# hanl2010/Binocular3DGS

Hardware: AMD Instinct MI355X
Metric: train iters/s (fwd+bwd), 1M Gaussians @ 800x600, 6 views/iter (higher is better)
Workload: dtype f32; 1 GPU; synth(P=1000000, seed=0) 800x600, 3 input + 3 binocular-shifted views per rank per iter, fwd+bwd+gradient sum+Adam; gaussians=1000000, width=800, height=600, views_per_rank=6, global_views=6, sh_degree=1, K=4, loss=synthetic, optimizer_in_step=True, densify_stats_in_step=True, optimizer=sharded, hip_graph=True, schedule=batched, binning_rounds=2, dp_tail_ranges=0

## Files before the change

binocular3dgs_amd/_lib.py:

```python
from __future__ import annotations

import ctypes as C
import os

_HERE = os.path.dirname(os.path.abspath(__file__))
LIB_PATH = os.environ.get("B3GS_LIB") or os.path.join(_HERE, "libb3gs_raster.so")

ABI_VERSION = 18
OK = 0
ERR_NAMES = {-1: "B3GS_ERR_ARG", -2: "B3GS_ERR_ALLOC", -3: "B3GS_ERR_HIP", -4: "B3GS_ERR_CAPACITY",
             -5: "B3GS_ERR_NO_DEVICE"}

c_float_p = C.c_void_p

ALLOC_FN = C.CFUNCTYPE(C.c_void_p, C.c_void_p, C.c_size_t)


class B3gsScene(C.Structure):
    _fields_ = [("P", C.c_int32), ("D", C.c_int32), ("M", C.c_int32), ("W", C.c_int32), ("H", C.c_int32),
                ("tan_fovx", C.c_float), ("tan_fovy", C.c_float), ("scale_modifier", C.c_float),
                ("prefiltered", C.c_int32), ("debug", C.c_int32),
                ("background", C.c_void_p), ("means3D", C.c_void_p), ("shs", C.c_void_p),
                ("colors_precomp", C.c_void_p), ("opacities", C.c_void_p), ("scales", C.c_void_p),
                ("rotations", C.c_void_p), ("cov3D_precomp", C.c_void_p), ("viewmatrix", C.c_void_p),
                ("projmatrix", C.c_void_p), ("campos", C.c_void_p)]


class B3gsRawParams(C.Structure):
    _fields_ = [("xyz", C.c_void_p), ("features_dc", C.c_void_p), ("features_rest", C.c_void_p),
                ("scaling", C.c_void_p), ("rotation", C.c_void_p), ("opacity", C.c_void_p)]


class B3gsRawGrads(C.Structure):
    _fields_ = B3gsRawParams._fields_ + [("touched_rows", C.c_void_p)]


class B3gsFusedView(C.Structure):
    _fields_ = [("view", C.POINTER(B3gsScene)), ("radii", C.c_void_p), ("geometry", C.c_void_p),
                ("scratch", C.c_void_p), ("dL_dmeans2D", C.c_void_p), ("densify_stats", C.c_int32)]


class B3gsBlendView(C.Structure):
    _fields_ = [("view", C.POINTER(B3gsScene)), ("geometry", C.c_void_p), ("binning", C.c_void_p),
                ("image", C.c_void_p), ("out_color", C.c_void_p), ("out_depth", C.c_void_p),
                ("out_alpha", C.c_void_p), ("dL_dcolor", C.c_void_p), ("dL_ddepth", C.c_void_p),
                ("dL_dalpha", C.c_void_p), ("scratch", C.c_void_p), ("binning_capacity", C.c_int64)]


class B3gsForwardView(C.Structure):
    _fields_ = [("view", C.POINTER(B3gsScene)), ("geometry", C.c_void_p), ("binning", C.c_void_p),
                ("binning_capacity", C.c_int64), ("image", C.c_void_p), ("out_color", C.c_void_p),
                ("out_depth", C.c_void_p), ("out_alpha", C.c_void_p), ("radii", C.c_void_p),
                ("device_num_rendered", C.c_void_p), ("depth_order_from", C.c_int32), ("seg1_fraction", C.c_float),
                ("high_water", C.c_void_p), ("overflow_flag", C.c_void_p), ("depth_key_bits", C.c_int32),
                ("fresh_image", C.c_int32), ("depth_order_hint", C.c_void_p), ("hint_mismatch", C.c_void_p),
                ("hint_trusted", C.c_int32), ("visible", C.c_void_p), ("reference_binning", C.c_int32)]


class B3gsLossIO(C.Structure):
    _fields_ = [("W", C.c_int32), ("H", C.c_int32), ("image", C.c_void_p), ("depth", C.c_void_p), ("alpha", C.c_void_p),
                ("gt_image", C.c_void_p), ("shifted_image", C.c_void_p), ("alpha_weight", C.c_void_p),
                ("focal_x", C.c_float), ("trans_dist", C.c_float), ("lambda_dssim", C.c_float),
                ("lambda_smooth", C.c_float), ("grad_scale", C.c_float), ("dL_dimage", C.c_void_p),
                ("dL_ddepth", C.c_void_p), ("dL_dalpha", C.c_void_p), ("dL_dshifted", C.c_void_p),
                ("parts", C.c_void_p), ("workspace", C.c_void_p), ("trans_dist_dev", C.c_void_p)]


class B3gsDensifyIO(C.Structure):
    _fields_ = [("P", C.c_int32), ("M", C.c_int32), ("param", C.c_void_p * 6), ("exp_avg", C.c_void_p * 6),
                ("exp_avg_sq", C.c_void_p * 6), ("xyz_gradient_accum", C.c_void_p), ("denom", C.c_void_p),
                ("grad_threshold", C.c_float), ("min_opacity", C.c_float), ("extent", C.c_float),
                ("percent_dense", C.c_float), ("max_screen_size", C.c_float)]


class B3gsAdamSegment(C.Structure):
    _fields_ = [("param", C.c_void_p), ("grad", C.c_void_p), ("exp_avg", C.c_void_p), ("exp_avg_sq", C.c_void_p),
                ("count", C.c_int64), ("lr", C.c_float), ("row_len", C.c_int32), ("first_row", C.c_int32),
                ("lr_dev", C.c_void_p)]


class B3gsDensifyStats(C.Structure):
    _fields_ = [("xyz_gradient_accum", C.c_void_p), ("denom", C.c_void_p), ("max_radii2D", C.c_void_p),
                ("skip_if_nonzero", C.c_void_p)]


class B3gsDebugViews(C.Structure):
    _fields_ = [("tiles_touched", C.c_void_p), ("depths", C.c_void_p), ("records", C.c_void_p),
                ("point_list", C.c_void_p), ("tile_ids", C.c_void_p), ("ranges", C.c_void_p),
                ("final_T", C.c_void_p), ("n_contrib", C.c_void_p), ("packed_idx_bits", C.c_int32),
                ("counts", C.c_void_p), ("point_list2", C.c_void_p), ("ranges2", C.c_void_p)]


class B3gsMetricView(C.Structure):
    _fields_ = [("image", C.c_void_p), ("gt", C.c_void_p), ("mask", C.c_void_p), ("mask_channels", C.c_int32),
                ("prepared_image", C.c_void_p), ("prepared_gt", C.c_void_p)]


class B3gsFrameView(C.Structure):
    _fields_ = [("rgb", C.c_void_p), ("depth", C.c_void_p), ("alpha", C.c_void_p), ("rgb_out", C.c_void_p),
                ("gray_out", C.c_void_p), ("cmap_out", C.c_void_p)]


class B3gsGtView(C.Structure):
    _fields_ = [("src", C.c_void_p), ("Hs", C.c_int32), ("Ws", C.c_int32), ("C", C.c_int32), ("tab_x", C.c_void_p),
                ("tab_y", C.c_void_p), ("ks_x", C.c_int32), ("ks_y", C.c_int32), ("image", C.c_void_p),
                ("alpha", C.c_void_p), ("bg_mask", C.c_void_p)]


class B3gsCloudGrow(C.Structure):
    _fields_ = ([(n, C.c_int32) for n in ("W", "H", "n_views", "ref", "src", "n_seeds", "n_samples", "n_start", "h_patch_size", "init")]
                + [(n, C.c_float) for n in ("fx", "fy", "cx", "cy", "alpha", "ssim_threshold")]
                + [(n, C.c_void_p) for n in ("images", "w2c", "window", "seed_idx", "noise", "points", "colors")]
                + [("capacity", C.c_int32)]
                + [(n, C.c_void_p) for n in ("length", "overflow", "grids", "workspace", "debug_ssim", "debug_mask")])


class B3gsSweepPair(C.Structure):
    _fields_ = ([(n, C.c_int32) for n in ("W", "H", "D", "stride", "radius")]
                + [(n, C.c_float) for n in ("near", "far", "inv_far", "step", "min_score", "margin", "min_var", "cyc_steps")]
                + [(n, C.c_void_p) for n in ("image_a", "image_b", "homographies", "proj", "kp_source", "kp_target", "score", "count",
                                             "node_invd", "node_score", "node_k", "workspace")])


class B3gsTsdfVolume(C.Structure):
    _fields_ = [("nx", C.c_int32), ("ny", C.c_int32), ("nz", C.c_int32), ("origin", C.c_float * 3), ("voxel", C.c_float),
                ("tsdf", C.c_void_p), ("weight", C.c_void_p), ("rgb", C.c_void_p)]


class B3gsTsdfView(C.Structure):
    _fields_ = [("depth", C.c_void_p), ("alpha", C.c_void_p), ("colour", C.c_void_p), ("rot", C.c_float * 9),
                ("trans", C.c_float * 3), ("fx", C.c_float), ("fy", C.c_float)]


class B3gsLpipsWeights(C.Structure):
    _fields_ = [("conv_w", C.c_void_p * 13), ("conv_b", C.c_void_p * 13), ("lin", C.c_void_p * 5), ("shift", C.c_float * 3),
                ("scale", C.c_float * 3)]


class B3gsKernelTimes(C.Structure):
    _fields_ = [("preprocess_ms", C.c_double), ("sort_ms", C.c_double), ("render_fwd_ms", C.c_double),
                ("render_bwd_ms", C.c_double), ("preprocess_bwd_ms", C.c_double), ("calls", C.c_int64)]


EXPORTS = ("b3gs_abi_version", "b3gs_last_error", "b3gs_set_timing", "b3gs_timing_collect", "b3gs_geometry_bytes", "b3gs_image_bytes",
           "b3gs_binning_bytes", "b3gs_forward", "b3gs_forward_capacity", "b3gs_backward", "b3gs_mark_visible",
           "b3gs_debug_views", "b3gs_forward_raw", "b3gs_backward_raw", "b3gs_backward_scratch_floats",
           "b3gs_backward_raw_accumulate", "b3gs_blend_forward_batch", "b3gs_blend_backward_batch",
           "b3gs_adam_step", "b3gs_forward_raw_batch", "b3gs_loss_workspace_floats", "b3gs_binocular_loss",
           "b3gs_densify_classify", "b3gs_densify_scatter", "b3gs_knn_workspace_bytes", "b3gs_knn_mean_dist2",
           "b3gs_backward_raw_accumulate_range", "b3gs_binocular_loss_batch",
           "b3gs_lossfn_workspace_floats", "b3gs_l1_loss_forward", "b3gs_l1_loss_backward", "b3gs_inverse_warp_forward",
           "b3gs_inverse_warp_backward", "b3gs_smooth_loss_forward", "b3gs_smooth_loss_backward", "b3gs_ssim_forward",
           "b3gs_ssim_backward", "b3gs_opacity_decay", "b3gs_add_densification_stats", "b3gs_adam_step_at", "b3gs_debug_activations",
           "b3gs_apply_staged_densify_stats",
           "b3gs_image_metrics_workspace_bytes", "b3gs_image_metrics_batch",
           "b3gs_frames_workspace_bytes", "b3gs_encode_frames_batch",
           "b3gs_gt_workspace_bytes", "b3gs_prepare_gt_batch",
           "b3gs_cloud_workspace_bytes", "b3gs_triangulate_matches", "b3gs_background_sheet", "b3gs_cloud_grow_round",
           "b3gs_sweep_workspace_bytes", "b3gs_sweep_match_pair",
           "b3gs_jpeg_workspace_bytes", "b3gs_jpeg_encode_batch",
           "b3gs_tsdf_integrate_batch", "b3gs_mesh_workspace_bytes", "b3gs_mesh_count", "b3gs_mesh_emit",
           "b3gs_mesh_components", "b3gs_mesh_clean_workspace_bytes", "b3gs_mesh_clean_count", "b3gs_mesh_clean_emit",
           "b3gs_mesh_sample_workspace_bytes", "b3gs_mesh_sample_count", "b3gs_mesh_sample_emit",
           "b3gs_nearest_workspace_bytes", "b3gs_nearest_grid", "b3gs_nearest_query",
           "b3gs_cloud_score_workspace_bytes", "b3gs_cloud_score",
           "b3gs_mesh_simplify_workspace_bytes", "b3gs_mesh_simplify_count", "b3gs_mesh_simplify_emit",
           "b3gs_mesh_raster_workspace_bytes", "b3gs_mesh_raster_batch", "b3gs_mesh_resolve_batch",
           "b3gs_mesh_texture_atlas_height", "b3gs_mesh_texture_accumulate_batch", "b3gs_mesh_texture_finalize",
           "b3gs_mesh_resolve_textured_batch",
           "b3gs_mesh_adjacency_workspace_bytes", "b3gs_mesh_adjacency_layout", "b3gs_mesh_adjacency_build", "b3gs_mesh_smooth",
           "b3gs_mesh_vertex_normals", "b3gs_mesh_resolve_shaded_batch",
           "b3gs_lpips_workspace_bytes", "b3gs_lpips_batch", "b3gs_lpips_features")

_lib = None


class B3gsError(RuntimeError):
    pass


def lib():
    global _lib
    if _lib is not None:
        return _lib
    if not os.path.exists(LIB_PATH):
        raise B3gsError(f"{LIB_PATH} not found: run `python -m binocular3dgs_amd.build` (hipcc, gfx950). "
                        "There is no CPU or PyTorch fallback for the rasterizer.")
    L = C.CDLL(LIB_PATH)
    L.b3gs_abi_version.restype = C.c_int
    L.b3gs_last_error.restype = C.c_char_p
    L.b3gs_set_timing.argtypes = [C.c_void_p]
    L.b3gs_set_timing.restype = None
    L.b3gs_timing_collect.restype = C.c_int
    L.b3gs_geometry_bytes.argtypes = [C.c_int32]
    L.b3gs_geometry_bytes.restype = C.c_size_t
    L.b3gs_image_bytes.argtypes = [C.c_int32, C.c_int32]
    L.b3gs_image_bytes.restype = C.c_size_t
    L.b3gs_binning_bytes.argtypes = [C.c_int32, C.c_int64]
    L.b3gs_binning_bytes.restype = C.c_size_t
    L.b3gs_forward.argtypes = [C.POINTER(B3gsScene), ALLOC_FN, C.c_void_p, ALLOC_FN, C.c_void_p, ALLOC_FN,
                               C.c_void_p, C.c_void_p, C.c_void_p, C.c_void_p, C.c_void_p,
                               C.POINTER(C.c_int32), C.c_void_p]
    L.b3gs_forward.restype = C.c_int
    L.b3gs_forward_capacity.argtypes = [C.POINTER(B3gsScene), C.c_void_p, C.c_void_p, C.c_int64, C.c_void_p,
                                        C.c_void_p, C.c_void_p, C.c_void_p, C.c_void_p, C.c_void_p, C.c_void_p]
    L.b3gs_forward_capacity.restype = C.c_int
    L.b3gs_backward.argtypes = [C.POINTER(B3gsScene), C.c_int32, C.c_void_p, C.c_void_p, C.c_void_p, C.c_void_p,
                                C.c_void_p, C.c_void_p, C.c_void_p] + [C.c_void_p] * 8 + [C.c_void_p]
    L.b3gs_backward.restype = C.c_int
    L.b3gs_forward_raw.argtypes = [C.POINTER(B3gsScene), C.POINTER(B3gsRawParams), C.c_void_p, C.c_void_p, C.c_int64,
                                   C.c_void_p, C.c_void_p, C.c_void_p, C.c_void_p, C.c_void_p, C.c_void_p, C.c_int,
                                   C.c_void_p]
    L.b3gs_forward_raw.restype = C.c_int
    for fn in (L.b3gs_blend_forward_batch, L.b3gs_blend_backward_batch):
        fn.argtypes = [C.c_int32, C.POINTER(B3gsBlendView), C.c_void_p]
        fn.restype = C.c_int
    L.b3gs_backward_scratch_floats.argtypes = [C.c_int32]
    L.b3gs_backward_scratch_floats.restype = C.c_size_t
    L.b3gs_backward_raw.argtypes = [C.POINTER(B3gsScene), C.POINTER(B3gsRawParams), C.c_void_p, C.c_void_p, C.c_void_p,
                                    C.c_void_p, C.c_void_p, C.c_void_p, C.c_void_p, C.c_void_p,
                                    C.POINTER(B3gsRawGrads), C.c_void_p, C.c_int, C.c_void_p]
    L.b3gs_backward_raw.restype = C.c_int
    L.b3gs_backward_raw_accumulate.argtypes = [C.c_int32, C.POINTER(B3gsFusedView), C.POINTER(B3gsRawParams),
                                               C.POINTER(B3gsRawGrads), C.c_int32, C.POINTER(B3gsDensifyStats),
                                               C.c_void_p]
    L.b3gs_backward_raw_accumulate.restype = C.c_int
    L.b3gs_backward_raw_accumulate_range.argtypes = [C.c_int32, C.POINTER(B3gsFusedView), C.POINTER(B3gsRawParams),
                                                     C.POINTER(B3gsRawGrads), C.c_int32, C.POINTER(B3gsDensifyStats),
                                                     C.c_int32, C.c_int32, C.c_void_p]
    L.b3gs_backward_raw_accumulate_range.restype = C.c_int
    L.b3gs_forward_raw_batch.argtypes = [C.c_int32, C.POINTER(B3gsForwardView), C.POINTER(B3gsRawParams), C.c_int,
                                         C.c_void_p]
    L.b3gs_forward_raw_batch.restype = C.c_int
    L.b3gs_loss_workspace_floats.argtypes = [C.c_int32, C.c_int32]
    L.b3gs_loss_workspace_floats.restype = C.c_size_t
    L.b3gs_binocular_loss.argtypes = [C.POINTER(B3gsLossIO), C.c_void_p]
    L.b3gs_binocular_loss.restype = C.c_int
    L.b3gs_binocular_loss_batch.argtypes = [C.c_int32, C.POINTER(B3gsLossIO), C.c_void_p]
    L.b3gs_binocular_loss_batch.restype = C.c_int
    L.b3gs_densify_classify.argtypes = [C.POINTER(B3gsDensifyIO), C.c_void_p, C.c_void_p]
    L.b3gs_densify_classify.restype = C.c_int
    L.b3gs_densify_scatter.argtypes = [C.POINTER(B3gsDensifyIO), C.c_void_p, C.c_void_p, C.c_void_p, C.c_void_p, C.c_int32,
                                       C.c_int32, C.c_int32, C.c_void_p, C.POINTER(C.c_void_p), C.POINTER(C.c_void_p),
                                       C.POINTER(C.c_void_p), C.c_void_p]
    L.b3gs_densify_scatter.restype = C.c_int
    L.b3gs_knn_workspace_bytes.argtypes = [C.c_int32]
    L.b3gs_knn_workspace_bytes.restype = C.c_size_t
    L.b3gs_knn_mean_dist2.argtypes = [C.c_int32, C.c_void_p, C.c_void_p, C.c_void_p, C.c_void_p]
    L.b3gs_knn_mean_dist2.restype = C.c_int
    L.b3gs_adam_step.argtypes = [C.c_int32, C.POINTER(B3gsAdamSegment), C.c_void_p, C.c_float, C.c_float, C.c_float,
                                 C.c_float, C.c_int32, C.c_int32, C.c_int32, C.c_void_p, C.c_void_p, C.c_void_p]
    L.b3gs_adam_step.restype = C.c_int
    V, I32, I64, F = C.c_void_p, C.c_int32, C.c_int64, C.c_float
    L.b3gs_lossfn_workspace_floats.argtypes = [I64, I32, I32]
    L.b3gs_lossfn_workspace_floats.restype = C.c_size_t
    L.b3gs_l1_loss_forward.argtypes = [V, V, V, I64, I32, I64, V, V, V]
    L.b3gs_l1_loss_backward.argtypes = [V, V, V, I64, I32, I64, V, V, V, V, V]
    L.b3gs_inverse_warp_forward.argtypes = [V, V, I32, I32, I32, I32, V, V, V]
    L.b3gs_inverse_warp_backward.argtypes = [V, V, V, I32, I32, I32, I32, V, V, V]
    L.b3gs_smooth_loss_forward.argtypes = [V, V, I32, I32, I32, I32, V, V, V]
    L.b3gs_smooth_loss_backward.argtypes = [V, V, I32, I32, I32, I32, V, V, V, V]
    L.b3gs_ssim_forward.argtypes = [V, V, I32, I32, I32, I32, I32, V, I32, V, V, V]
    L.b3gs_ssim_backward.argtypes = [V, V, V, I32, I32, I32, I32, I32, V, V, V, V]
    L.b3gs_opacity_decay.argtypes = [V, I64, F, V]
    L.b3gs_add_densification_stats.argtypes = [I64, V, I64, V, V, V, V]
    L.b3gs_adam_step_at.argtypes = [I32, C.POINTER(B3gsAdamSegment), I32, F, F, F, V]
    for fn in (L.b3gs_l1_loss_forward, L.b3gs_l1_loss_backward, L.b3gs_inverse_warp_forward, L.b3gs_inverse_warp_backward,
               L.b3gs_smooth_loss_forward, L.b3gs_smooth_loss_backward, L.b3gs_ssim_forward, L.b3gs_ssim_backward,
               L.b3gs_opacity_decay, L.b3gs_add_densification_stats, L.b3gs_adam_step_at):
        fn.restype = C.c_int
    L.b3gs_apply_staged_densify_stats.argtypes = [I64] + [V] * 9
    L.b3gs_apply_staged_densify_stats.restype = C.c_int
    L.b3gs_debug_activations.argtypes = [I32, C.POINTER(B3gsRawParams), V, V, V, V]
    L.b3gs_debug_activations.restype = C.c_int
    L.b3gs_image_metrics_workspace_bytes.argtypes = [I32, I32, I32, I32]
    L.b3gs_image_metrics_workspace_bytes.restype = C.c_size_t
    L.b3gs_image_metrics_batch.argtypes = [I32, C.POINTER(B3gsMetricView), I32, I32, I32, I32, V, V, V]
    L.b3gs_image_metrics_batch.restype = C.c_int
    L.b3gs_frames_workspace_bytes.argtypes = [I32, I32, I32]
    L.b3gs_frames_workspace_bytes.restype = C.c_size_t
    L.b3gs_encode_frames_batch.argtypes = [I32, C.POINTER(B3gsFrameView), I32, I32, C.c_double, V, V, V, V]
    L.b3gs_encode_frames_batch.restype = C.c_int
    L.b3gs_gt_workspace_bytes.argtypes = [I32, C.POINTER(B3gsGtView), I32, I32]
    L.b3gs_gt_workspace_bytes.restype = C.c_size_t
    L.b3gs_prepare_gt_batch.argtypes = [I32, C.POINTER(B3gsGtView), I32, I32, I32, C.c_float, V, V]
    L.b3gs_prepare_gt_batch.restype = C.c_int
    L.b3gs_cloud_workspace_bytes.argtypes = [I64]
    L.b3gs_cloud_workspace_bytes.restype = C.c_size_t
    L.b3gs_triangulate_matches.argtypes = [I32] + [V] * 8 + [I32, I32, F, V, V, V, V, V]
    L.b3gs_triangulate_matches.restype = C.c_int
    L.b3gs_background_sheet.argtypes = [V, I32, I32, V, V, F, V, V, V, V, V]
    L.b3gs_background_sheet.restype = C.c_int
    L.b3gs_cloud_grow_round.argtypes = [C.POINTER(B3gsCloudGrow), V]
    L.b3gs_cloud_grow_round.restype = C.c_int
    L.b3gs_sweep_workspace_bytes.argtypes = [I32, I32, I32, I32]
    L.b3gs_sweep_workspace_bytes.restype = C.c_size_t
    L.b3gs_sweep_match_pair.argtypes = [C.POINTER(B3gsSweepPair), V]
    L.b3gs_sweep_match_pair.restype = C.c_int
    L.b3gs_jpeg_workspace_bytes.argtypes = [I32, I32, I32]
    L.b3gs_jpeg_workspace_bytes.restype = C.c_size_t
    L.b3gs_jpeg_encode_batch.argtypes = [I32, C.POINTER(C.c_void_p), I32, I32, V, V, I64, V, V, V]
    L.b3gs_jpeg_encode_batch.restype = C.c_int
    L.b3gs_tsdf_integrate_batch.argtypes = [C.POINTER(B3gsTsdfVolume), I32, C.POINTER(B3gsTsdfView), I32, I32, F, F, F, V]
    L.b3gs_tsdf_integrate_batch.restype = C.c_int
    L.b3gs_mesh_workspace_bytes.argtypes = [I32, I32, I32]
    L.b3gs_mesh_workspace_bytes.restype = C.c_size_t
    L.b3gs_mesh_count.argtypes = [C.POINTER(B3gsTsdfVolume), F, V, V]
    L.b3gs_mesh_count.restype = C.c_int
    L.b3gs_mesh_emit.argtypes = [C.POINTER(B3gsTsdfVolume), V, I64, I64, V, V, V, V]
    L.b3gs_mesh_emit.restype = C.c_int
    L.b3gs_mesh_components.argtypes = [I32, I64, V, V, V, V]
    L.b3gs_mesh_components.restype = C.c_int
    L.b3gs_mesh_clean_workspace_bytes.argtypes = [I64, I64]
    L.b3gs_mesh_clean_workspace_bytes.restype = C.c_size_t
    L.b3gs_mesh_clean_count.argtypes = [I32, I64, V, V, V, V, V, V]
    L.b3gs_mesh_clean_count.restype = C.c_int
    L.b3gs_mesh_clean_emit.argtypes = [I32, I64, V, V, V, V, V, V, V, I64, I64, V, V, V, V]
    L.b3gs_mesh_clean_emit.restype = C.c_int
    L.b3gs_mesh_sample_workspace_bytes.argtypes = [I64]
    L.b3gs_mesh_sample_workspace_bytes.restype = C.c_size_t
    L.b3gs_mesh_sample_count.argtypes = [I32, I64, V, V, F, V, V]
    L.b3gs_mesh_sample_count.restype = C.c_int
    L.b3gs_mesh_sample_emit.argtypes = [I32, I64, V, V, F, V, I64, V, V]
    L.b3gs_mesh_sample_emit.restype = C.c_int
    L.b3gs_nearest_workspace_bytes.argtypes = [I64]
    L.b3gs_nearest_workspace_bytes.restype = C.c_size_t
    L.b3gs_nearest_grid.argtypes = [I64, V, F, V, V]
    L.b3gs_nearest_grid.restype = C.c_int
    L.b3gs_nearest_query.argtypes = [I64, V, I64, F, V, V, V]
    L.b3gs_nearest_query.restype = C.c_int
    L.b3gs_cloud_score_workspace_bytes.argtypes = [I64]
    L.b3gs_cloud_score_workspace_bytes.restype = C.c_size_t
    L.b3gs_cloud_score.argtypes = [I64, V, V, F, V, V, V]
    L.b3gs_cloud_score.restype = C.c_int
    L.b3gs_mesh_simplify_workspace_bytes.argtypes = [I64, I64]
    L.b3gs_mesh_simplify_workspace_bytes.restype = C.c_size_t
    L.b3gs_mesh_simplify_count.argtypes = [I32, I64, V, V, F, V, V]
    L.b3gs_mesh_simplify_count.restype = C.c_int
    L.b3gs_mesh_simplify_emit.argtypes = [I32, I64, V, V, V, F, I32, V, I64, I64, V, V, V, V]
    L.b3gs_mesh_simplify_emit.restype = C.c_int
    L.b3gs_mesh_raster_workspace_bytes.argtypes = [I32, I64, I64, I32, I32]
    L.b3gs_mesh_raster_workspace_bytes.restype = C.c_size_t
    L.b3gs_mesh_raster_batch.argtypes = [I32, V, I32, I32, I32, I64, V, V, I32, I32, I32, V, V, V]
    L.b3gs_mesh_raster_batch.restype = C.c_int
    L.b3gs_mesh_resolve_batch.argtypes = [I32, V, I32, I32, I32, I64, V, V, V, V, V, I32, V, V, V, V, V, V]
    L.b3gs_mesh_resolve_batch.restype = C.c_int
    L.b3gs_mesh_texture_atlas_height.argtypes = [I64, I32, I32]
    L.b3gs_mesh_texture_atlas_height.restype = I32
    L.b3gs_mesh_texture_accumulate_batch.argtypes = [I32, V, I32, I32, I32, I64, V, V, I32, I32, I32, V, V, V, C.c_float, I32, V, V, V]
    L.b3gs_mesh_texture_accumulate_batch.restype = C.c_int
    L.b3gs_mesh_texture_finalize.argtypes = [I32, I64, V, V, I32, I32, I32, V, V, V, V]
    L.b3gs_mesh_texture_finalize.restype = C.c_int
    L.b3gs_mesh_resolve_textured_batch.argtypes = [I32, V, I32, I32, I32, I64, V, V, V, V, V, I32, I32, I32, V, V, V, V, V, V]
    L.b3gs_mesh_resolve_textured_batch.restype = C.c_int
    L.b3gs_mesh_adjacency_workspace_bytes.argtypes = [I64, I64]
    L.b3gs_mesh_adjacency_workspace_bytes.restype = C.c_size_t
    L.b3gs_mesh_adjacency_layout.argtypes = [I64, I64, C.POINTER(C.c_size_t)]
    L.b3gs_mesh_adjacency_layout.restype = C.c_int
    L.b3gs_mesh_adjacency_build.argtypes = [I32, I64, V, V, V, V]
    L.b3gs_mesh_adjacency_build.restype = C.c_int
    L.b3gs_mesh_smooth.argtypes = [I32, I64, V, V, I32, C.c_double, C.c_double, I32, V, V]
    L.b3gs_mesh_smooth.restype = C.c_int
    L.b3gs_mesh_vertex_normals.argtypes = [I32, I64, V, V, V, V, V]
    L.b3gs_mesh_vertex_normals.restype = C.c_int
    L.b3gs_mesh_resolve_shaded_batch.argtypes = [I32, V, I32, I32, I32, I64, V, V, V, V, I32, V, V, V, V, V, V]
    L.b3gs_mesh_resolve_shaded_batch.restype = C.c_int
    L.b3gs_lpips_workspace_bytes.argtypes = [I32, I32, I32]
    L.b3gs_lpips_workspace_bytes.restype = C.c_size_t
    L.b3gs_lpips_batch.argtypes = [I32, V, V, I32, I32, C.POINTER(B3gsLpipsWeights), I32, V, V, V]
    L.b3gs_lpips_batch.restype = C.c_int
    L.b3gs_lpips_features.argtypes = [I32, V, I32, I32, C.POINTER(B3gsLpipsWeights), I32, C.POINTER(C.c_void_p), V, V]
    L.b3gs_lpips_features.restype = C.c_int
    L.b3gs_mark_visible.argtypes = [C.c_int32, C.c_void_p, C.c_void_p, C.c_void_p, C.c_void_p, C.c_void_p]
    L.b3gs_mark_visible.restype = C.c_int
    L.b3gs_debug_views.argtypes = [C.c_int32, C.c_int32, C.c_int32, C.c_int64, C.c_void_p, C.c_void_p, C.c_void_p,
                                   C.POINTER(B3gsDebugViews)]
    L.b3gs_debug_views.restype = C.c_int
    if L.b3gs_abi_version() != ABI_VERSION:
        raise B3gsError(f"libb3gs_raster.so ABI {L.b3gs_abi_version()} != binding {ABI_VERSION}: rebuild")
    _lib = L
    return L


# ... 5 lines not shown
```

binocular3dgs_amd/csrc/api.hip:

```cpp
#include "b3gs_internal.h"

#include <cstdio>
#include <cstdlib>
#include <cstring>
#include <mutex>

namespace {

thread_local char g_err[512] = "";
B3gsKernelTimes* g_timing = nullptr;
std::mutex g_timing_mu;

int fail(int code, const char* fmt, const char* detail) {
  snprintf(g_err, sizeof(g_err), fmt, detail);
  return code;
}

#define HIP_TRY(expr)                                                                   \
  do {                                                                                  \
    hipError_t e_ = (expr);                                                             \
    if (e_ != hipSuccess) return fail(B3GS_ERR_HIP, #expr ": %s", hipGetErrorString(e_)); \
  } while (0)

int check_scene(const B3gsScene* sc) {
  if (!sc) return fail(B3GS_ERR_ARG, "%s", "scene is NULL");
  if (sc->P < 0 || sc->W <= 0 || sc->H <= 0) return fail(B3GS_ERR_ARG, "%s", "bad P/W/H");
  if (sc->P >= (1 << 24)) return fail(B3GS_ERR_ARG, "%s", "P must be below 2^24 (24-bit row offsets in the blend backward)");
  if (sc->D < 0 || sc->D > 3) return fail(B3GS_ERR_ARG, "%s", "SH degree must be 0..3");
  if ((sc->shs == nullptr) == (sc->colors_precomp == nullptr))
    return fail(B3GS_ERR_ARG, "%s", "provide exactly one of shs / colors_precomp");
  const bool has_sr = sc->scales != nullptr && sc->rotations != nullptr;
  if (has_sr == (sc->cov3D_precomp != nullptr))
    return fail(B3GS_ERR_ARG, "%s", "provide exactly one of (scales, rotations) / cov3D_precomp");
  if (sc->shs && sc->M < (sc->D + 1) * (sc->D + 1)) return fail(B3GS_ERR_ARG, "%s", "M too small for SH degree");
  if (((sc->W + B3GS_TILE - 1) / B3GS_TILE) > 65535 || ((sc->H + B3GS_TILE - 1) / B3GS_TILE) > 65535)
    return fail(B3GS_ERR_ARG, "%s", "image too large for the packed tile rect");
  if (!sc->background || !sc->viewmatrix || !sc->projmatrix || !sc->campos || (sc->P > 0 && (!sc->means3D || !sc->opacities)))
    return fail(B3GS_ERR_ARG, "%s", "NULL required tensor");
  return B3GS_OK;
}

SceneX wrap(const B3gsScene* sc) {
  SceneX x;
  x.sc = *sc;
  x.raw = B3gsRawParams{nullptr, nullptr, nullptr, nullptr, nullptr, nullptr};
  x.raw_mode = 0;
  x.tight = 0;
  return x;
}

int check_raw(const B3gsScene* sc, const B3gsRawParams* rp) {
  if (!sc || !rp) return fail(B3GS_ERR_ARG, "%s", "scene / raw params NULL");
  if (sc->P < 0 || sc->W <= 0 || sc->H <= 0) return fail(B3GS_ERR_ARG, "%s", "bad P/W/H");
  if (sc->P >= (1 << 24)) return fail(B3GS_ERR_ARG, "%s", "P must be below 2^24 (24-bit row offsets in the blend backward)");
  if (sc->D < 0 || sc->D > 3 || sc->M < (sc->D + 1) * (sc->D + 1)) return fail(B3GS_ERR_ARG, "%s", "bad SH degree / M");
  if (((sc->W + B3GS_TILE - 1) / B3GS_TILE) > 65535 || ((sc->H + B3GS_TILE - 1) / B3GS_TILE) > 65535)
    return fail(B3GS_ERR_ARG, "%s", "image too large for the packed tile rect");
  if (!sc->background || !sc->viewmatrix || !sc->projmatrix || !sc->campos) return fail(B3GS_ERR_ARG, "%s", "NULL camera tensor");
  if (sc->P > 0 && (!rp->xyz || !rp->features_dc || (sc->M > 1 && !rp->features_rest) || !rp->scaling || !rp->rotation ||
                    !rp->opacity))
    return fail(B3GS_ERR_ARG, "%s", "NULL raw parameter tensor");
  return B3GS_OK;
}

void blend_forward_one(const B3gsScene& sc, const GeomView& g, const BinView& b, const ImgView& im, float* out_color,
                       float* out_depth, float* out_alpha, hipStream_t s) {
  BlendBatch batch;
  batch.n = 1;
  batch.order = nullptr;
  batch.order_buf = nullptr;
  batch.cls_size = 0;
  batch.v[0] = b3gs_blend_view(sc, g, b, im);
  batch.v[0].out_color = out_color;
  batch.v[0].out_depth = out_depth;
  batch.v[0].out_alpha = out_alpha;
  b3gs_launch_blend_forward(batch, s);
}

BlendView blend_backward_view(const B3gsScene& sc, const GeomView& g, const BinView& b, const ImgView& im,
                              const float* dL_dcolor, const float* dL_ddepth, const float* dL_dalpha, float* m2d,
                              float* col, float* op, float* cov, uint32_t m2d_stride, uint32_t col_stride,
                              uint32_t op_stride, uint32_t cov_stride) {
  BlendView v = b3gs_blend_view(sc, g, b, im);
  v.dL_dcolor = dL_dcolor;
  v.dL_ddepth = dL_ddepth;
  v.dL_dalpha = dL_dalpha;
  v.dL_dmeans2D = m2d;
  v.dL_dcolors = col;
  v.dL_dopacity = op;
  v.dL_dcov3D = cov;
  v.m2d_stride = m2d_stride;
  v.col_stride = col_stride;
  v.op_stride = op_stride;
  v.cov_stride = cov_stride;
  return v;
}

struct PendingStage {
  hipEvent_t a, b;
  int slot;
};
PendingStage g_pending[4096];
int g_npending = 0;

struct StageTimer {
  hipStream_t s;
  hipEvent_t prev = nullptr;
  bool on;
  explicit StageTimer(hipStream_t st) : s(st), on(g_timing != nullptr) {}
  void mark(int slot) {
    if (!on) return;
    hipEvent_t e;
    (void)hipEventCreate(&e);
    (void)hipEventRecord(e, s);
    std::lock_guard<std::mutex> lk(g_timing_mu);
    if (slot >= 0 && prev && g_npending < 4096) {
      g_pending[g_npending++] = PendingStage{prev, e, slot};
    }
    prev = e;
  }
};

int debug_sync(const B3gsScene* sc, hipStream_t s, const char* what) {
  if (!sc->debug) return B3GS_OK;
  hipError_t e = hipStreamSynchronize(s);
  if (e == hipSuccess) e = hipGetLastError();
  if (e != hipSuccess) {
    snprintf(g_err, sizeof(g_err), "after %s: %s", what, hipGetErrorString(e));
    return B3GS_ERR_HIP;
  }
  return B3GS_OK;
}

}

int b3gs_fail(int code, const char* what, const char* detail) {
  snprintf(g_err, sizeof(g_err), "%s%s%s", what ? what : "", (what && detail) ? ": " : "", detail ? detail : "");
  return code;
}

int b3gs_launch_status(const char* what) {
  const hipError_t e = hipGetLastError();
  return e == hipSuccess ? B3GS_OK : b3gs_fail(B3GS_ERR_HIP, what, hipGetErrorString(e));
}

extern "C" {

int b3gs_abi_version(void) { return B3GS_ABI_VERSION; }
const char* b3gs_last_error(void) { return g_err; }
void b3gs_set_timing(B3gsKernelTimes* sink) { g_timing = sink; }

int b3gs_timing_collect(void) {
  std::lock_guard<std::mutex> lk(g_timing_mu);
// ... 268 lines not shown
  if (phases & 2) {
    b3gs_launch_blend_forward(bb, s);
    tm.mark(2);
    if (K1) {
      b3gs_launch_round2_batch(P, nviews, jobs, s);
      tm.mark(1);
      for (int k = 0; k < nviews; k++) bb.v[k].round = 1;
      b3gs_launch_blend_forward(bb, s);
      tm.mark(2);
    }
  }
  HIP_TRY(hipGetLastError());
  return B3GS_OK;
}

size_t b3gs_backward_scratch_floats(int32_t P) { return (size_t)B3GS_SCRATCH_ROW * (size_t)(P > 0 ? P : 0); }

int b3gs_backward_raw(const B3gsScene* view, const B3gsRawParams* params, const int32_t* radii, const char* geometry,
                      const char* binning, const char* image, const float* dL_dcolor, const float* dL_ddepth,
                      const float* dL_dalpha, float* scratch, const B3gsRawGrads* grads, float* dL_dmeans2D,
                      int phases, b3gs_stream_t stream) {
  int rc = check_raw(view, params);
  if (rc) return rc;
  if (view->P == 0) return B3GS_OK;
  if (!radii || !geometry || !binning || !image || !dL_dcolor || !scratch || !grads || !grads->xyz ||
      !grads->features_dc || (view->M > 1 && !grads->features_rest) || !grads->scaling || !grads->rotation ||
      !grads->opacity)
    return fail(B3GS_ERR_ARG, "%s", "NULL required tensor in backward_raw");
  hipStream_t s = (hipStream_t)stream;
  SceneX sx;
  sx.sc = *view;
  sx.raw = *params;
  sx.raw_mode = 1;
  sx.tight = 0;
  GeomView g;
  ImgView im;
  BinView b;
  b3gs_geom_view(const_cast<char*>(geometry), view->P, &g);
  b3gs_img_view(const_cast<char*>(image), view->W, view->H, &im);
  b3gs_bin_view(const_cast<char*>(binning), view->P, 1, &b);
  const size_t P = (size_t)view->P;
  (void)P;
  StageTimer tm(s);
  tm.mark(-1);
  if (phases & 1) {
    BlendBatch batch;
    batch.n = 1;
    batch.order = nullptr;
    batch.order_buf = im.order;
    batch.v[0] = blend_backward_view(sx.sc, g, b, im, dL_dcolor, dL_ddepth, dL_dalpha, scratch + 4, scratch + 6,
                                     scratch + 9, scratch, B3GS_SCRATCH_ROW, B3GS_SCRATCH_ROW, B3GS_SCRATCH_ROW,
                                     B3GS_SCRATCH_ROW);
    b3gs_launch_blend_backward(batch, s);
    tm.mark(3);
  }
  if (phases & 2) {
    if (!(phases & 1)) tm.mark(-1);
    b3gs_launch_preprocess_backward(sx, g, radii, nullptr, nullptr, nullptr, nullptr, scratch, nullptr, nullptr, nullptr,
                                    grads, dL_dmeans2D, s);
    tm.mark(4);
  }
  HIP_TRY(hipGetLastError());
  return B3GS_OK;
}

int b3gs_backward(const B3gsScene* sc, int32_t num_rendered, const int32_t* radii, const char* geometry,
                  const char* binning, const char* image, const float* dL_dcolor, const float* dL_ddepth,
                  const float* dL_dalpha, float* dL_dmeans2D, float* dL_dcolors, float* dL_dopacity,
                  float* dL_dmeans3D, float* dL_dcov3D, float* dL_dsh, float* dL_dscales, float* dL_drotations,
                  b3gs_stream_t stream) {
  int rc = check_scene(sc);
  if (rc) return rc;
  if (sc->P == 0) return B3GS_OK;
  if (!radii || !geometry || !image || !dL_dcolor || !dL_dmeans2D || !dL_dcolors || !dL_dopacity || !dL_dmeans3D ||
      !dL_dcov3D)
    return fail(B3GS_ERR_ARG, "%s", "NULL required tensor in backward");
  if (sc->shs && !dL_dsh) return fail(B3GS_ERR_ARG, "%s", "dL_dsh required when shs given");
  if (sc->scales && (!dL_dscales || !dL_drotations)) return fail(B3GS_ERR_ARG, "%s", "dL_dscales/dL_drotations required");
  if (num_rendered != 0 && !binning) return fail(B3GS_ERR_ARG, "%s", "binning buffer is NULL");
  hipStream_t s = (hipStream_t)stream;
  GeomView g;
  ImgView im;
  BinView b;
  b3gs_geom_view(const_cast<char*>(geometry), sc->P, &g);
  b3gs_img_view(const_cast<char*>(image), sc->W, sc->H, &im);
  b3gs_bin_view(const_cast<char*>(binning), sc->P, num_rendered < 0 ? 1 : num_rendered, &b);

  const size_t P = (size_t)sc->P;
  StageTimer tm(s);
  tm.mark(-1);
  float* rows = g.bwd_rows;
  HIP_TRY(hipMemsetAsync(rows, 0, P * B3GS_SCRATCH_ROW * sizeof(float), s));
  if (num_rendered != 0) {
    BlendBatch batch;
    batch.n = 1;
    batch.order = nullptr;
    batch.order_buf = im.order;
    batch.v[0] = blend_backward_view(*sc, g, b, im, dL_dcolor, dL_ddepth, dL_dalpha, rows + 4, rows + 6, rows + 9, rows,
                                     B3GS_SCRATCH_ROW, B3GS_SCRATCH_ROW, B3GS_SCRATCH_ROW, B3GS_SCRATCH_ROW);
    b3gs_launch_blend_backward(batch, s);
  }
  if ((rc = debug_sync(sc, s, "render backward"))) return rc;
  tm.mark(3);
  b3gs_launch_preprocess_backward(wrap(sc), g, radii, dL_dmeans2D, dL_dcolors, dL_dopacity, dL_dmeans3D, dL_dcov3D,
                                  dL_dsh, dL_dscales, dL_drotations, nullptr, nullptr, s);
  if ((rc = debug_sync(sc, s, "preprocess backward"))) return rc;
  tm.mark(4);
  HIP_TRY(hipGetLastError());
  return B3GS_OK;
}

static int batch_views_ok(int32_t nviews, const B3gsBlendView* views) {
  if (nviews <= 0 || nviews > B3GS_MAX_FUSED_VIEWS || !views)
    return fail(B3GS_ERR_ARG, "%s", "bad view count (1..8) or NULL view table");
  for (int k = 0; k < nviews; k++)
    if (!views[k].view || !views[k].geometry || !views[k].binning || !views[k].image || views[k].view->W <= 0 ||
        views[k].view->H <= 0 || !views[k].view->background)
      return fail(B3GS_ERR_ARG, "%s", "NULL state buffer in a batched view");
  return B3GS_OK;
}

int b3gs_blend_forward_batch(int32_t nviews, const B3gsBlendView* views, b3gs_stream_t stream) {
  int rc = batch_views_ok(nviews, views);
  if (rc) return rc;
  hipStream_t s = (hipStream_t)stream;
  BlendBatch batch;
  batch.n = nviews;
  batch.order = nullptr;
  batch.order_buf = nullptr;
  batch.cls_size = 0;
  for (int k = 0; k < nviews; k++) {
    const B3gsBlendView& bv = views[k];
    if (!bv.out_color || !bv.out_depth || !bv.out_alpha) return fail(B3GS_ERR_ARG, "%s", "NULL output image");
    GeomView g;
    ImgView im;
    BinView b;
    b3gs_geom_view(const_cast<char*>(bv.geometry), bv.view->P, &g);
    b3gs_img_view(const_cast<char*>(bv.image), bv.view->W, bv.view->H, &im);
    b3gs_bin_view(const_cast<char*>(bv.binning), bv.view->P, bv.binning_capacity > 0 ? bv.binning_capacity : 1, &b);
    batch.v[k] = b3gs_blend_view(*bv.view, g, b, im);
    batch.v[k].round = 2;
    batch.v[k].out_color = bv.out_color;
    batch.v[k].out_depth = bv.out_depth;
    batch.v[k].out_alpha = bv.out_alpha;
  }
  StageTimer tm(s);
  tm.mark(-1);
  b3gs_launch_blend_forward(batch, s);
  tm.mark(2);
  HIP_TRY(hipGetLastError());
  return B3GS_OK;
}

int b3gs_blend_backward_batch(int32_t nviews, const B3gsBlendView* views, b3gs_stream_t stream) {
  int rc = batch_views_ok(nviews, views);
  if (rc) return rc;
  hipStream_t s = (hipStream_t)stream;
  BlendBatch batch;
  batch.n = nviews;
  batch.order = nullptr;
  batch.order_buf = nullptr;
  batch.cls_size = 0;
  for (int k = 0; k < nviews; k++) {
    const B3gsBlendView& bv = views[k];
    if (!bv.dL_dcolor || !bv.scratch) return fail(B3GS_ERR_ARG, "%s", "NULL dL_dcolor / scratch");
    GeomView g;
    ImgView im;
    BinView b;
    b3gs_geom_view(const_cast<char*>(bv.geometry), bv.view->P, &g);
    b3gs_img_view(const_cast<char*>(bv.image), bv.view->W, bv.view->H, &im);
    if (k == 0) batch.order_buf = im.order;
    b3gs_bin_view(const_cast<char*>(bv.binning), bv.view->P, bv.binning_capacity > 0 ? bv.binning_capacity : 1, &b);
    batch.v[k] = blend_backward_view(*bv.view, g, b, im, bv.dL_dcolor, bv.dL_ddepth, bv.dL_dalpha, bv.scratch + 4,
                                     bv.scratch + 6, bv.scratch + 9, bv.scratch, B3GS_SCRATCH_ROW, B3GS_SCRATCH_ROW,
                                     B3GS_SCRATCH_ROW, B3GS_SCRATCH_ROW);
  }
  StageTimer tm(s);
  tm.mark(-1);
  b3gs_launch_blend_backward(batch, s);
  tm.mark(3);
  HIP_TRY(hipGetLastError());
  return B3GS_OK;
}

int b3gs_backward_raw_accumulate(int32_t nviews, const B3gsFusedView* views, const B3gsRawParams* params,
                                 const B3gsRawGrads* grads, int32_t overwrite, const B3gsDensifyStats* stats,
                                 b3gs_stream_t stream) {
  const int32_t P = (nviews > 0 && views && views[0].view) ? views[0].view->P : 0;
  return b3gs_backward_raw_accumulate_range(nviews, views, params, grads, overwrite, stats, 0, P, stream);
}

int b3gs_backward_raw_accumulate_range(int32_t nviews, const B3gsFusedView* views, const B3gsRawParams* params,
                                       const B3gsRawGrads* grads, int32_t overwrite, const B3gsDensifyStats* stats,
                                       int32_t first, int32_t count, b3gs_stream_t stream) {
  if (nviews <= 0 || nviews > B3GS_MAX_FUSED_VIEWS || !views || !params || !grads)
    return fail(B3GS_ERR_ARG, "%s", "bad view count / NULL argument (at most 8 views per call)");
  const B3gsScene* v0 = views[0].view;
  int rc = check_raw(v0, params);
  if (rc) return rc;
  if (v0->P == 0 || count == 0) return B3GS_OK;
  if (first < 0 || count < 0 || (int64_t)first + count > v0->P) return fail(B3GS_ERR_ARG, "%s", "bad Gaussian range");
  if (grads->touched_rows && overwrite && (first & 63))
    return fail(B3GS_ERR_ARG, "%s", "sparse-row gradients (touched_rows) need a range that starts at a multiple of 64");
  if (!grads->xyz || !grads->features_dc || (v0->M > 1 && !grads->features_rest) || !grads->scaling ||
      !grads->rotation || !grads->opacity)
    return fail(B3GS_ERR_ARG, "%s", "NULL gradient buffer");
  B3gsViewRef refs[B3GS_MAX_FUSED_VIEWS];
  uint32_t *list = nullptr, *counts = nullptr;
  static const bool no_staged = getenv("B3GS_NO_STAGED") != nullptr;
  for (int k = 0; k < nviews; k++) {
    const B3gsFusedView& fv = views[k];
    if (!fv.view || !fv.radii || !fv.geometry || !fv.scratch) return fail(B3GS_ERR_ARG, "%s", "NULL view state");
    if (fv.view->P != v0->P || fv.view->M != v0->M || fv.view->D != v0->D || fv.view->scale_modifier != v0->scale_modifier)
      return fail(B3GS_ERR_ARG, "%s", "views of one call must share P, M, D and scale_modifier");
    GeomView g;
    b3gs_geom_view(const_cast<char*>(fv.geometry), v0->P, &g);
    if (k == 0) { list = g.skey[1]; counts = g.skey[0]; }
    refs[k] = B3gsViewRef{fv.view->W, fv.view->H, fv.view->tan_fovx, fv.view->tan_fovy, fv.view->viewmatrix,
                          fv.view->projmatrix, fv.view->campos, fv.radii, reinterpret_cast<const float*>(g.rec), fv.scratch, fv.dL_dmeans2D,
                          fv.densify_stats, no_staged ? nullptr : g.staged, g.header + B3GS_GEOM_EPOCH};
  }
  if (stats && (!stats->xyz_gradient_accum || !stats->denom || !stats->max_radii2D))
    return fail(B3GS_ERR_ARG, "%s", "densify stats need all three arrays");
  hipStream_t s = (hipStream_t)stream;
  StageTimer tm(s);
  tm.mark(-1);
  b3gs_launch_accumulate_views(*v0, *params, nviews, refs, *grads, overwrite, stats, first, count, list, counts, s);
  tm.mark(4);
  HIP_TRY(hipGetLastError());
  return B3GS_OK;
}

int b3gs_mark_visible(int32_t P, const float* means3D, const float* viewmatrix, const float* projmatrix,
                      uint8_t* present, b3gs_stream_t stream) {
  (void)projmatrix;
  if (P < 0 || (P > 0 && (!means3D || !viewmatrix || !present))) return fail(B3GS_ERR_ARG, "%s", "bad arguments");
  b3gs_launch_mark_visible(P, means3D, viewmatrix, present, (hipStream_t)stream);
  HIP_TRY(hipGetLastError());
  return B3GS_OK;
}

int b3gs_debug_views(int32_t P, int32_t W, int32_t H, int64_t num_rendered, const char* geometry, const char* binning,
                     const char* image, B3gsDebugViews* out) {
  if (!out || !geometry || !image) return fail(B3GS_ERR_ARG, "%s", "NULL argument");
  GeomView g;
  ImgView im;
  BinView b;
  b3gs_geom_view(const_cast<char*>(geometry), P, &g);
  b3gs_img_view(const_cast<char*>(image), W, H, &im);
  memset(out, 0, sizeof(*out));
  out->tiles_touched = g.tiles_touched;
  out->depths = reinterpret_cast<const float*>(g.depth_key);
  out->records = reinterpret_cast<const float*>(g.rec);
  if (binning) {
    b3gs_bin_view(const_cast<char*>(binning), P, num_rendered, &b);
    out->point_list = b.val[0];
    out->packed_idx_bits = b3gs_packed_idx_bits(P, W, H);
    out->tile_ids = out->packed_idx_bits >= 0 ? nullptr : b.key[0];
  }
  out->ranges = reinterpret_cast<const uint32_t*>(im.ranges);
  out->ranges2 = reinterpret_cast<const uint32_t*>(im.ranges2);
  out->counts = g.header;
  if (binning) out->point_list2 = b.val[0];
  out->final_T = im.final_T;
  out->n_contrib = im.n_contrib;
  return B3GS_OK;
}

}
```

binocular3dgs_amd/csrc/preprocess.hip:

```cpp
#include "b3gs_internal.h"

namespace {

constexpr float SH_C0 = 0.28209479177387814f;
constexpr float SH_C1 = 0.4886025119029199f;
__constant__ float SH_C2[5] = {1.0925484305920792f, -1.0925484305920792f, 0.31539156525252005f,
                               -1.0925484305920792f, 0.5462742152960396f};
__constant__ float SH_C3[7] = {-0.5900435899266435f, 2.890611442640554f, -0.4570457994644658f,
                               0.3731763325901154f,  -0.4570457994644658f, 1.445305721320277f,
                               -0.5900435899266435f};

struct Mat16 {
  float m[16];
};

__device__ __forceinline__ Mat16 load_mat(const float* __restrict__ p) {
  Mat16 r;
#pragma unroll
  for (int i = 0; i < 16; i++) r.m[i] = p[i];
  return r;
}
typedef const float __attribute__((address_space(4))) cfloat_k;
__device__ __forceinline__ cfloat_k* uniform_ptr(const float* p) { return (cfloat_k*)(uintptr_t)p; }
__device__ __forceinline__ Mat16 load_mat_uniform(const float* p) {
  cfloat_k* q = uniform_ptr(p);
  Mat16 r;
#pragma unroll
  for (int i = 0; i < 16; i++) r.m[i] = q[i];
  return r;
}

__device__ __forceinline__ void quat_to_R(float r, float x, float y, float z, float R[9]) {
  R[0] = 1.f - 2.f * (y * y + z * z);
  R[1] = 2.f * (x * y - r * z);
  R[2] = 2.f * (x * z + r * y);
  R[3] = 2.f * (x * y + r * z);
  R[4] = 1.f - 2.f * (x * x + z * z);
  R[5] = 2.f * (y * z - r * x);
  R[6] = 2.f * (x * z - r * y);
  R[7] = 2.f * (y * z + r * x);
  R[8] = 1.f - 2.f * (x * x + y * y);
}

template <bool RAW>
__device__ __forceinline__ void load_scale_rot(const SceneX& sx_, int i, float s[3], float q[4], float* inv_norm) {
  if (RAW) {
    const float* ls = sx_.raw.scaling + 3 * (size_t)i;
    s[0] = expf(ls[0]); s[1] = expf(ls[1]); s[2] = expf(ls[2]);
    const float4 r = reinterpret_cast<const float4*>(sx_.raw.rotation)[i];
    const float n = sqrtf((r.x * r.x + r.y * r.y) + (r.z * r.z + r.w * r.w));
    const float den = fmaxf(n, 1e-12f);
    q[0] = r.x / den; q[1] = r.y / den; q[2] = r.z / den; q[3] = r.w / den;
    *inv_norm = 1.0f / den;
  } else {
    const float* ps = sx_.sc.scales + 3 * (size_t)i;
    s[0] = ps[0]; s[1] = ps[1]; s[2] = ps[2];
    const float4 r = reinterpret_cast<const float4*>(sx_.sc.rotations)[i];
    q[0] = r.x; q[1] = r.y; q[2] = r.z; q[3] = r.w;
    *inv_norm = 1.0f;
  }
}
template <bool RAW>
__device__ __forceinline__ float load_opacity(const SceneX& sx_, int i) {
  if (RAW) return 1.0f / (1.0f + expf(-sx_.raw.opacity[i]));
  return sx_.sc.opacities[i];
}
struct ShView {
  const float* dc;
  const float* rest;
  __device__ __forceinline__ float operator()(int k, int ch) const { return k == 0 ? dc[ch] : rest[3 * (k - 1) + ch]; }
};
struct ShLds {
  const float* lo;
  const float* rest;
  __device__ __forceinline__ float operator()(int k, int ch) const { return k < 4 ? lo[(3 * k + ch) * 256] : rest[3 * (k - 1) + ch]; }
};
template <bool RAW>
__device__ __forceinline__ ShView sh_view(const SceneX& sx_, int i) {
  ShView v;
  if (RAW) {
    v.dc = sx_.raw.features_dc + 3 * (size_t)i;
    v.rest = sx_.raw.features_rest + (size_t)3 * (sx_.sc.M - 1) * i;
  } else {
    v.dc = sx_.sc.shs + (size_t)3 * sx_.sc.M * i;
    v.rest = v.dc + 3;
  }
  return v;
}

template <bool RAW>
__device__ __forceinline__ void cov3d_of(const SceneX& sx_, int i, float c6[6]) {
  const B3gsScene& sc = sx_.sc;
  if (!RAW && sc.cov3D_precomp) {
#pragma unroll
    for (int k = 0; k < 6; k++) c6[k] = sc.cov3D_precomp[6 * (size_t)i + k];
    return;
  }
  float s[3], q[4], inv_norm;
  load_scale_rot<RAW>(sx_, i, s, q, &inv_norm);
  float R[9], L[9];
  quat_to_R(q[0], q[1], q[2], q[3], R);
  float sx = sc.scale_modifier * s[0], sy = sc.scale_modifier * s[1], sz = sc.scale_modifier * s[2];
#pragma unroll
  for (int r = 0; r < 3; r++) {
    L[3 * r + 0] = R[3 * r + 0] * sx;
    L[3 * r + 1] = R[3 * r + 1] * sy;
    L[3 * r + 2] = R[3 * r + 2] * sz;
  }
#define LL(a, b) ((L[3 * a] * L[3 * b] + L[3 * a + 1] * L[3 * b + 1]) + L[3 * a + 2] * L[3 * b + 2])
  c6[0] = LL(0, 0);
  c6[1] = LL(0, 1);
  c6[2] = LL(0, 2);
  c6[3] = LL(1, 1);
  c6[4] = LL(1, 2);
  c6[5] = LL(2, 2);
#undef LL
}

struct Ewa {
  float T0[3], T1[3];
  float a, b, c;
  float tx, ty, tz;
  float xmul, ymul;
};

__device__ __forceinline__ Ewa ewa_project(const float pv[3], float fx, float fy, float tanfovx, float tanfovy,
                                           const float c6[6], const Mat16& vm) {
  Ewa e;
  float limx = 1.3f * tanfovx, limy = 1.3f * tanfovy;
  float txtz = pv[0] / pv[2], tytz = pv[1] / pv[2];
  e.xmul = (txtz < -limx || txtz > limx) ? 0.f : 1.f;
  e.ymul = (tytz < -limy || tytz > limy) ? 0.f : 1.f;
  e.tx = fminf(limx, fmaxf(-limx, txtz)) * pv[2];
  e.ty = fminf(limy, fmaxf(-limy, tytz)) * pv[2];
  e.tz = pv[2];
  float J00 = fx / e.tz, J02 = -(fx * e.tx) / (e.tz * e.tz);
  float J11 = fy / e.tz, J12 = -(fy * e.ty) / (e.tz * e.tz);
#pragma unroll
  for (int j = 0; j < 3; j++) {
    e.T0[j] = J00 * vm.m[4 * j + 0] + J02 * vm.m[4 * j + 2];
    e.T1[j] = J11 * vm.m[4 * j + 1] + J12 * vm.m[4 * j + 2];
  }
  float S00 = c6[0], S01 = c6[1], S02 = c6[2], S11 = c6[3], S12 = c6[4], S22 = c6[5];
  float v0x = (S00 * e.T0[0] + S01 * e.T0[1]) + S02 * e.T0[2];
  float v0y = (S01 * e.T0[0] + S11 * e.T0[1]) + S12 * e.T0[2];
  float v0z = (S02 * e.T0[0] + S12 * e.T0[1]) + S22 * e.T0[2];
  float v1x = (S00 * e.T1[0] + S01 * e.T1[1]) + S02 * e.T1[2];
  float v1y = (S01 * e.T1[0] + S11 * e.T1[1]) + S12 * e.T1[2];
  float v1z = (S02 * e.T1[0] + S12 * e.T1[1]) + S22 * e.T1[2];
  e.a = (e.T0[0] * v0x + e.T0[1] * v0y) + e.T0[2] * v0z;
  e.b = (e.T0[0] * v1x + e.T0[1] * v1y) + e.T0[2] * v1z;
  e.c = (e.T1[0] * v1x + e.T1[1] * v1y) + e.T1[2] * v1z;
  return e;
// ... 408 lines not shown
      gdir[0] += rx * gl;
      gdir[1] += ry * gl;
      gdir[2] += rz * gl;
    }
    float dot = gdir[0] * x + gdir[1] * y + gdir[2] * z;
    dmean[0] += (gdir[0] - x * dot) * inv;
    dmean[1] += (gdir[1] - y * dot) * inv;
    dmean[2] += (gdir[2] - z * dot) * inv;
  }

  if (do_sr) {
    load_scale_rot<RAW>(sx_, i, o.sraw, o.q, &o.inv_norm);
    const float r = o.q[0], x = o.q[1], y = o.q[2], z = o.q[3];
    float R[9];
    quat_to_R(r, x, y, z, R);
    const float sv[3] = {sc.scale_modifier * o.sraw[0], sc.scale_modifier * o.sraw[1], sc.scale_modifier * o.sraw[2]};
    const float G[9] = {dS[0], 0.5f * dS[1], 0.5f * dS[2], 0.5f * dS[1], dS[3], 0.5f * dS[4], 0.5f * dS[2], 0.5f * dS[4], dS[5]};
    float dR[9];
#pragma unroll
    for (int bcol = 0; bcol < 3; bcol++) {
      float ds = 0.f;
#pragma unroll
      for (int arow = 0; arow < 3; arow++) {
        float dLab = 2.f * sv[bcol] * (G[3 * arow] * R[bcol] + G[3 * arow + 1] * R[3 + bcol] + G[3 * arow + 2] * R[6 + bcol]);
        ds += dLab * R[3 * arow + bcol];
        dR[3 * arow + bcol] = dLab * sv[bcol];
      }
      o.dscale[bcol] = ds * sc.scale_modifier;
    }
    o.dq.x = 2.f * (-z * dR[1] + y * dR[2] + z * dR[3] - x * dR[5] - y * dR[6] + x * dR[7]);
    o.dq.y = 2.f * (y * dR[1] + z * dR[2] + y * dR[3] - 2.f * x * dR[4] - r * dR[5] + z * dR[6] + r * dR[7] - 2.f * x * dR[8]);
    o.dq.z = 2.f * (-2.f * y * dR[0] + x * dR[1] + r * dR[2] + x * dR[3] + z * dR[5] - r * dR[6] + z * dR[7] - 2.f * y * dR[8]);
    o.dq.w = 2.f * (-2.f * z * dR[0] - r * dR[1] + x * dR[2] + r * dR[3] - 2.f * z * dR[4] + y * dR[5] + x * dR[6] + y * dR[7]);
  }
}

__device__ __forceinline__ void raw_chain(const GaussGrad& gg, float dscaling[3], float4& drot) {
  dscaling[0] = gg.dscale[0] * gg.sraw[0];
  dscaling[1] = gg.dscale[1] * gg.sraw[1];
  dscaling[2] = gg.dscale[2] * gg.sraw[2];
  const float qd = ((gg.q[0] * gg.dq.x + gg.q[1] * gg.dq.y) + gg.q[2] * gg.dq.z) + gg.q[3] * gg.dq.w;
  drot.x = (gg.dq.x - gg.q[0] * qd) * gg.inv_norm;
  drot.y = (gg.dq.y - gg.q[1] * qd) * gg.inv_norm;
  drot.z = (gg.dq.z - gg.q[2] * qd) * gg.inv_norm;
  drot.w = (gg.dq.w - gg.q[3] * qd) * gg.inv_norm;
}

template <bool RAW>
__global__ void __launch_bounds__(256)
    preprocess_bwd_kernel(SceneX sx_, GeomView g, const int32_t* __restrict__ radii, float* __restrict__ dL_dmeans2D,
                          float* __restrict__ dL_dcolors, float* __restrict__ dL_dopacity,
                          float* __restrict__ dL_dmeans3D, float* __restrict__ dL_dcov3D, float* __restrict__ dL_dsh,
                          float* __restrict__ dL_dscales, float* __restrict__ dL_drots, B3gsRawGrads rg,
                          float* __restrict__ m2d_out) {
  const B3gsScene& sc = sx_.sc;
  const int i = blockIdx.x * blockDim.x + threadIdx.x;
  if (i >= sc.P) return;
  const size_t i3 = 3 * (size_t)i;
  if (radii[i] <= 0) {
    if (RAW) {
      if (m2d_out) { m2d_out[i3] = 0.f; m2d_out[i3 + 1] = 0.f; m2d_out[i3 + 2] = 0.f; }
      return;
    }
#pragma unroll
    for (int k = 0; k < 3; k++) { dL_dmeans2D[i3 + k] = 0.f; dL_dcolors[i3 + k] = 0.f; dL_dmeans3D[i3 + k] = 0.f; }
#pragma unroll
    for (int k = 0; k < 6; k++) dL_dcov3D[6 * (size_t)i + k] = 0.f;
    dL_dopacity[i] = 0.f;
    if (dL_dsh) for (int k = 0; k < 3 * sc.M; k++) dL_dsh[(size_t)3 * sc.M * i + k] = 0.f;
    if (dL_dscales) { dL_dscales[i3] = 0.f; dL_dscales[i3 + 1] = 0.f; dL_dscales[i3 + 2] = 0.f; }
    if (dL_drots) reinterpret_cast<float4*>(dL_drots)[i] = make_float4(0.f, 0.f, 0.f, 0.f);
    return;
  }
  const Mat16 vm = load_mat_uniform(sc.viewmatrix);
  const Mat16 pm = load_mat_uniform(sc.projmatrix);

  PixSums in;
  if (RAW) {
    bool touched;
    in = load_scratch_row(dL_dcov3D, i, &touched);
    if (m2d_out) { m2d_out[i3] = in.g2x; m2d_out[i3 + 1] = in.g2y; m2d_out[i3 + 2] = 0.f; }
  } else {
    const float2* row = reinterpret_cast<const float2*>(g.bwd_rows) + 5 * (size_t)i;
    const float2 r0 = row[0], r1 = row[1], r2 = row[2], r3 = row[3], r4 = row[4];
    in.gxx = r0.x; in.gxy = r0.y; in.gyy = r1.x; in.gdepth = r1.y;
    in.g2x = r2.x; in.g2y = r2.y;
    in.gcol[0] = r3.x; in.gcol[1] = r3.y; in.gcol[2] = r4.x;
    in.gop = r4.y;
    dL_dmeans2D[i3] = in.g2x; dL_dmeans2D[i3 + 1] = in.g2y; dL_dmeans2D[i3 + 2] = 0.f;
    dL_dcolors[i3] = in.gcol[0]; dL_dcolors[i3 + 1] = in.gcol[1]; dL_dcolors[i3 + 2] = in.gcol[2];
    dL_dopacity[i] = in.gop;
  }
  {
    const uint32_t any = ((__float_as_uint(in.gxx) | __float_as_uint(in.gxy)) | (__float_as_uint(in.gyy) | __float_as_uint(in.gdepth))) |
                         ((__float_as_uint(in.g2x) | __float_as_uint(in.g2y)) | (__float_as_uint(in.gcol[0]) | __float_as_uint(in.gcol[1]))) |
                         (__float_as_uint(in.gcol[2]) | __float_as_uint(in.gop));
    if (any == 0u) {
      if (RAW) return;
#pragma unroll
      for (int k = 0; k < 3; k++) dL_dmeans3D[i3 + k] = 0.f;
#pragma unroll
      for (int k = 0; k < 6; k++) dL_dcov3D[6 * (size_t)i + k] = 0.f;
      if (dL_dsh) for (int k = 0; k < 3 * sc.M; k++) dL_dsh[(size_t)3 * sc.M * i + k] = 0.f;
      if (dL_dscales) { dL_dscales[i3] = 0.f; dL_dscales[i3 + 1] = 0.f; dL_dscales[i3 + 2] = 0.f; }
      if (dL_drots) reinterpret_cast<float4*>(dL_drots)[i] = make_float4(0.f, 0.f, 0.f, 0.f);
      return;
    }
  }

  GaussGrad gg;
  const uint32_t cb = __float_as_uint(reinterpret_cast<const float*>(g.rec + 4 * (size_t)i + 3)[0]);
  if (RAW) {
    ShAddMem sink{rg.features_dc + i3, rg.features_rest + (size_t)3 * (sc.M - 1) * i};
    gaussian_backward<true>(sx_, vm, pm, i, cb, in, true, true, gg, sink);
    rg.xyz[i3] += gg.dmean[0];
    rg.xyz[i3 + 1] += gg.dmean[1];
    rg.xyz[i3 + 2] += gg.dmean[2];
    const float op = load_opacity<true>(sx_, i);
    rg.opacity[i] += in.gop * op * (1.0f - op);
    float dsc[3];
    float4 drot;
    raw_chain(gg, dsc, drot);
    rg.scaling[i3] += dsc[0];
    rg.scaling[i3 + 1] += dsc[1];
    rg.scaling[i3 + 2] += dsc[2];
    float4* dst = reinterpret_cast<float4*>(rg.rotation) + i;
    float4 cur = *dst;
    cur.x += drot.x; cur.y += drot.y; cur.z += drot.z; cur.w += drot.w;
    *dst = cur;
  } else {
    const bool do_sh = !sc.colors_precomp && dL_dsh;
    const bool do_sr = !sc.cov3D_precomp && dL_dscales && dL_drots;
    float* dsh = do_sh ? dL_dsh + (size_t)3 * sc.M * i : nullptr;
    if (do_sh) {
      const int nb = (sc.D + 1) * (sc.D + 1);
      for (int k = nb; k < sc.M; k++) { dsh[3 * k] = 0.f; dsh[3 * k + 1] = 0.f; dsh[3 * k + 2] = 0.f; }
    }
    ShStore sink{dsh, dsh ? dsh + 3 : nullptr};
    gaussian_backward<false>(sx_, vm, pm, i, cb, in, do_sh, do_sr, gg, sink);
#pragma unroll
    for (int k = 0; k < 6; k++) dL_dcov3D[6 * (size_t)i + k] = gg.dS[k];
    dL_dmeans3D[i3] = gg.dmean[0];
    dL_dmeans3D[i3 + 1] = gg.dmean[1];
    dL_dmeans3D[i3 + 2] = gg.dmean[2];
    if (do_sr) {
      dL_dscales[i3] = gg.dscale[0];
      dL_dscales[i3 + 1] = gg.dscale[1];
      dL_dscales[i3 + 2] = gg.dscale[2];
      reinterpret_cast<float4*>(dL_drots)[i] = gg.dq;
    }
  }
}

struct MultiViews {
  int n;
  B3gsViewRef v[B3GS_MAX_FUSED_VIEWS];
};

#ifndef B3GS_ACC_WAVES
#define B3GS_ACC_WAVES 3
#endif
template <int ACC_PER_THREAD>
__global__ void __launch_bounds__(256, ACC_PER_THREAD >= 4 ? 4 : 8)
    accumulate_scan_kernel(B3gsScene base, MultiViews mv, B3gsRawGrads rg, int overwrite, int first, int count,
                           B3gsDensifyStats ds, uint32_t* __restrict__ g_list, uint32_t* __restrict__ g_count) {
  constexpr int ACC_BLOCK = 256 * ACC_PER_THREAD;
  __shared__ uint32_t s_list[ACC_BLOCK];
  __shared__ uint32_t s_count;
  if (threadIdx.x == 0) s_count = 0;
  __syncthreads();
  const int blk_first = first + (int)blockIdx.x * ACC_BLOCK;
  const int end = first + count;
  const unsigned lane = threadIdx.x & 63u;
  const unsigned long long lt = lane == 0 ? 0ull : (~0ull >> (64 - lane));
  const int nrest = 3 * (base.M - 1);
  const bool skip_stats = ds.skip_if_nonzero && *ds.skip_if_nonzero != 0;
  unsigned long long epochs = 0ull;
#pragma unroll
  for (int v = 0; v < B3GS_MAX_FUSED_VIEWS; v++)
    if (v < mv.n && mv.v[v].staged) epochs |= (unsigned long long)(*mv.v[v].epoch & 0xFFu) << (8 * v);

  uint32_t vis_j[ACC_PER_THREAD], stg_j[ACC_PER_THREAD];
  int rad_j[ACC_PER_THREAD];
  float cnt_j[ACC_PER_THREAD], acc_j[ACC_PER_THREAD], den_j[ACC_PER_THREAD], mxr_j[ACC_PER_THREAD];
  const bool do_stats = ds.denom && !skip_stats;
#pragma unroll
  for (int j = 0; j < ACC_PER_THREAD; j++) {
    const int i = blk_first + j * 256 + (int)threadIdx.x;
    const bool valid = i < end;
    const int ic = valid ? i : end - 1;
    uint32_t vis = 0u, stg = 0u;
    int st_rad = 0;
    float st_cnt = 0.f;
#pragma unroll
    for (int v = 0; v < B3GS_MAX_FUSED_VIEWS; v++) {
      if (v < mv.n) {
        const B3gsViewRef& vr = mv.v[v];
        const int rad = vr.radii[ic];
        const uint8_t ep = (uint8_t)(epochs >> (8 * v));
        const uint8_t mk = vr.staged ? vr.staged[ic] : ep;
        if (rad > 0) {
          vis |= 1u << v;
          if (vr.densify_stats) {
            st_cnt += 1.0f;
            st_rad = max(st_rad, rad);
          }
        }
        if (mk == ep) stg |= 1u << v;
      }
    }
    vis_j[j] = valid ? vis : 0u, stg_j[j] = stg, rad_j[j] = st_rad, cnt_j[j] = valid ? st_cnt : 0.f;
    acc_j[j] = do_stats ? ds.xyz_gradient_accum[ic] : 0.f;
    den_j[j] = do_stats ? ds.denom[ic] : 0.f;
    mxr_j[j] = do_stats ? ds.max_radii2D[ic] : 0.f;
  }
#pragma unroll
  for (int j = 0; j < ACC_PER_THREAD; j++) {
    const int li = j * 256 + (int)threadIdx.x;
    const int i = blk_first + li;
    uint32_t mask = 0;
    if (i < end) {
      const size_t i3 = 3 * (size_t)i;
      float st_norm = 0.f;
      const float st_cnt = cnt_j[j];
      const int st_rad = rad_j[j];
      const uint32_t vis = vis_j[j], stg = stg_j[j];
      for (int v = 0; v < mv.n; v++) {
        const B3gsViewRef& vr = mv.v[v];
        float* m2d = vr.dL_dmeans2D;
        if (!((vis >> v) & 1u)) {
          if (m2d) { m2d[i3] = 0.f; m2d[i3 + 1] = 0.f; m2d[i3 + 2] = 0.f; }
          continue;
        }
        float2 r0 = make_float2(0.f, 0.f), r1 = r0, r2 = r0, r3 = r0, r4 = r0;
        if ((stg >> v) & 1u) {
          const float2* row = reinterpret_cast<const float2*>(vr.scratch) + 5 * (size_t)i;
          r0 = row[0], r1 = row[1], r2 = row[2], r3 = row[3], r4 = row[4];
        }
        const uint32_t any = ((__float_as_uint(r0.x) | __float_as_uint(r0.y)) | (__float_as_uint(r1.x) | __float_as_uint(r1.y))) |
                             ((__float_as_uint(r2.x) | __float_as_uint(r2.y)) | (__float_as_uint(r3.x) | __float_as_uint(r3.y))) |
                             (__float_as_uint(r4.x) | __float_as_uint(r4.y));
        if (any) mask |= 1u << v;
        if (m2d) { m2d[i3] = r2.x; m2d[i3 + 1] = r2.y; m2d[i3 + 2] = 0.f; }
        if (vr.densify_stats) st_norm += sqrtf(r2.x * r2.x + r2.y * r2.y);
      }
      if (do_stats && st_cnt > 0.f) {
        ds.xyz_gradient_accum[i] = acc_j[j] + st_norm;
        ds.denom[i] = den_j[j] + st_cnt;
        ds.max_radii2D[i] = fmaxf(mxr_j[j], (float)st_rad);
      }
      if (mask == 0u && overwrite && !rg.touched_rows) {
        rg.xyz[i3] = 0.f; rg.xyz[i3 + 1] = 0.f; rg.xyz[i3 + 2] = 0.f;
        rg.scaling[i3] = 0.f; rg.scaling[i3 + 1] = 0.f; rg.scaling[i3 + 2] = 0.f;
        reinterpret_cast<float4*>(rg.rotation)[i] = make_float4(0.f, 0.f, 0.f, 0.f);
        rg.opacity[i] = 0.f;
        rg.features_dc[i3] = 0.f; rg.features_dc[i3 + 1] = 0.f; rg.features_dc[i3 + 2] = 0.f;
        float* rest = rg.features_rest + (size_t)nrest * i;
        for (int k = 0; k < nrest; k++) rest[k] = 0.f;
      }
    }
    const unsigned long long b = __ballot(mask != 0u);
    if (overwrite && rg.touched_rows && lane == 0 && blk_first + j * 256 + (int)(threadIdx.x & ~63u) < end)
      rg.touched_rows[(size_t)(blk_first + j * 256 + (int)(threadIdx.x & ~63u)) >> 6] = b;
    if (b) {
      const int leader = __builtin_ctzll(b);
      uint32_t at = 0;
      if ((int)lane == leader) at = atomicAdd(&s_count, (uint32_t)__builtin_popcountll(b));
      at = (uint32_t)__shfl((int)at, leader, 64);
      if (mask != 0u) s_list[at + (uint32_t)__builtin_popcountll(b & lt)] = (uint32_t)li | (mask << 16);
    }
  }
  __syncthreads();
  const uint32_t n_list = s_count;
  for (uint32_t e = threadIdx.x; e < n_list; e += 256) g_list[(size_t)blockIdx.x * ACC_BLOCK + e] = s_list[e];
  if (threadIdx.x == 0) g_count[blockIdx.x] = n_list;
}

template <int REG>
struct ShPairReg {
  float acc[3 * REG];
  float* rest;
  __device__ __forceinline__ void put(int k, int ch, float v) {
    if (k < REG) acc[3 * k + ch] += v;
    else unsafeAtomicAdd(rest + 3 * (k - 1) + ch, v);
  }
};

constexpr int CH_GROUP = 256;
constexpr int CH_ROW = 25;
template <int ACC_PER_THREAD>
__global__ void __launch_bounds__(256, B3GS_ACC_WAVES)
    accumulate_chain_kernel(B3gsScene base, B3gsRawParams raw, MultiViews mv, B3gsRawGrads rg, int overwrite, int first,
                            const uint32_t* __restrict__ g_list, const uint32_t* __restrict__ g_count) {
  constexpr int ACC_BLOCK = 256 * ACC_PER_THREAD;
  __shared__ float s_acc[CH_GROUP][CH_ROW];
  __shared__ uint8_t s_idx[B3GS_MAX_FUSED_VIEWS][CH_GROUP];
  __shared__ uint32_t s_wcnt[B3GS_MAX_FUSED_VIEWS][4];
  __shared__ uint32_t s_chunk[B3GS_MAX_FUSED_VIEWS * 4];
  __shared__ uint32_t s_nchunk;
  const uint32_t nblk = gridDim.x / (uint32_t)ACC_PER_THREAD;
  const uint32_t blk = blockIdx.x % nblk, part = blockIdx.x / nblk;
  const int blk_first = first + (int)blk * ACC_BLOCK;
  const int nrest = 3 * (base.M - 1);
  const uint32_t* __restrict__ s_list = g_list + (size_t)blk * ACC_BLOCK;
  const uint32_t n_list = min(g_count[blk], (part + 1u) * (uint32_t)CH_GROUP);
  const unsigned lane = threadIdx.x & 63u, w = threadIdx.x >> 6;
  const unsigned long long lt = lane == 0 ? 0ull : (~0ull >> (64 - lane));
  SceneX sx_;
  sx_.sc = base;
  sx_.raw = raw;
  sx_.raw_mode = 1;
  sx_.tight = 0;
#pragma unroll 1
  for (uint32_t e0 = part * (uint32_t)CH_GROUP; e0 < n_list; e0 += CH_GROUP) {
    const uint32_t e = e0 + threadIdx.x;
    const uint32_t ent = e < n_list ? s_list[e] : 0u;
    const uint32_t mask = ent >> 16;
    const int i = blk_first + (int)(ent & 0xFFFFu);
    const size_t i3 = 3 * (size_t)i;
#pragma unroll
    for (int k = 0; k < 23; k++) s_acc[threadIdx.x][k] = 0.f;
    if (mask != 0u && overwrite && base.M > 4) {
      float* rest = rg.features_rest + (size_t)nrest * i;
      for (int k = 9; k < nrest; k++) rest[k] = 0.f;
    }
    uint32_t rank[B3GS_MAX_FUSED_VIEWS];
#pragma unroll
    for (int v = 0; v < B3GS_MAX_FUSED_VIEWS; v++) {
      rank[v] = 0;
      if (v < mv.n) {
        const unsigned long long b = __ballot((mask >> v) & 1u);
        rank[v] = (uint32_t)__builtin_popcountll(b & lt);
        if (lane == 0) s_wcnt[v][w] = (uint32_t)__builtin_popcountll(b);
      }
    }
    __syncthreads();
#pragma unroll
    for (int v = 0; v < B3GS_MAX_FUSED_VIEWS; v++)
      if (v < mv.n && ((mask >> v) & 1u)) {
        uint32_t base_w = 0;
        for (unsigned k = 0; k < w; k++) base_w += s_wcnt[v][k];
        s_idx[v][base_w + rank[v]] = (uint8_t)threadIdx.x;
      }
    if (threadIdx.x == 0) {
      uint32_t nc = 0;
      for (int v = 0; v < mv.n; v++) {
        const uint32_t tot = (s_wcnt[v][0] + s_wcnt[v][1]) + (s_wcnt[v][2] + s_wcnt[v][3]);
        for (uint32_t p0 = 0; p0 < tot; p0 += 64u) s_chunk[nc++] = (uint32_t)v | (p0 << 8) | (min(64u, tot - p0) << 20);
      }
      s_nchunk = nc;
    }
    __syncthreads();
    const uint32_t nchunk = s_nchunk;
#pragma unroll 1
    for (uint32_t c = w; c < nchunk; c += 4u) {
      const uint32_t cd = __builtin_amdgcn_readfirstlane(s_chunk[c]);
      const int v = (int)(cd & 0xFFu);
      const uint32_t p0 = (cd >> 8) & 0xFFFu, np = cd >> 20;
      if (lane >= np) continue;
      const uint32_t t2 = s_idx[v][p0 + lane];
      const int i2 = blk_first + (int)(s_list[e0 + t2] & 0xFFFFu);
      const B3gsViewRef& vr = mv.v[v];
      sx_.sc.W = vr.W; sx_.sc.H = vr.H;
      sx_.sc.tan_fovx = vr.tan_fovx; sx_.sc.tan_fovy = vr.tan_fovy;
      sx_.sc.viewmatrix = vr.viewmatrix; sx_.sc.projmatrix = vr.projmatrix; sx_.sc.campos = vr.campos;
      const Mat16 vm = load_mat_uniform(vr.viewmatrix);
      const Mat16 pm = load_mat_uniform(vr.projmatrix);
      const PixSums in = load_scratch_row(vr.scratch, i2);
      ShPairReg<4> sink;
#pragma unroll
      for (int k = 0; k < 12; k++) sink.acc[k] = 0.f;
      sink.rest = rg.features_rest + (size_t)nrest * i2;
      GaussGrad gg;
      gaussian_backward<true>(sx_, vm, pm, i2, __float_as_uint(vr.rec_words[16 * (size_t)i2 + 12]), in, true, true, gg, sink);
      float dsc[3];
      float4 dr;
      raw_chain(gg, dsc, dr);
      float* row = s_acc[t2];
      atomicAdd(row + 0, gg.dmean[0]); atomicAdd(row + 1, gg.dmean[1]); atomicAdd(row + 2, gg.dmean[2]);
      atomicAdd(row + 3, dsc[0]); atomicAdd(row + 4, dsc[1]); atomicAdd(row + 5, dsc[2]);
      atomicAdd(row + 6, dr.x); atomicAdd(row + 7, dr.y); atomicAdd(row + 8, dr.z); atomicAdd(row + 9, dr.w);
      atomicAdd(row + 10, in.gop);
#pragma unroll
      for (int k = 0; k < 12; k++) atomicAdd(row + 11 + k, sink.acc[k]);
    }
    __syncthreads();
    if (mask != 0u) {
      const float* row = s_acc[threadIdx.x];
      const float op = load_opacity<true>(sx_, i);
      const float dop = row[10] * op * (1.0f - op);
      const int nreg = base.M < 4 ? base.M : 4;
      float4* rot_dst = reinterpret_cast<float4*>(rg.rotation) + i;
      float* dc = rg.features_dc + i3;
      float* rest = rg.features_rest + (size_t)nrest * i;
      if (overwrite) {
        rg.xyz[i3] = row[0]; rg.xyz[i3 + 1] = row[1]; rg.xyz[i3 + 2] = row[2];
        rg.scaling[i3] = row[3]; rg.scaling[i3 + 1] = row[4]; rg.scaling[i3 + 2] = row[5];
        *rot_dst = make_float4(row[6], row[7], row[8], row[9]);
        rg.opacity[i] = dop;
#pragma unroll
        for (int ch = 0; ch < 3; ch++) dc[ch] = row[11 + ch];
#pragma unroll
        for (int k = 1; k < 4; k++)
          if (k < nreg) { rest[3 * (k - 1)] = row[11 + 3 * k]; rest[3 * (k - 1) + 1] = row[12 + 3 * k]; rest[3 * (k - 1) + 2] = row[13 + 3 * k]; }
      } else {
        rg.xyz[i3] += row[0]; rg.xyz[i3 + 1] += row[1]; rg.xyz[i3 + 2] += row[2];
        rg.scaling[i3] += row[3]; rg.scaling[i3 + 1] += row[4]; rg.scaling[i3 + 2] += row[5];
        float4 cur = *rot_dst;
        cur.x += row[6]; cur.y += row[7]; cur.z += row[8]; cur.w += row[9];
        *rot_dst = cur;
        rg.opacity[i] += dop;
#pragma unroll
        for (int ch = 0; ch < 3; ch++) dc[ch] += row[11 + ch];
#pragma unroll
        for (int k = 1; k < 4; k++)
          if (k < nreg) { rest[3 * (k - 1)] += row[11 + 3 * k]; rest[3 * (k - 1) + 1] += row[12 + 3 * k]; rest[3 * (k - 1) + 2] += row[13 + 3 * k]; }
      }
    }
  }
}

__global__ void mark_visible_kernel(int P, const float* __restrict__ means3D, const float* __restrict__ viewmatrix,
                                    uint8_t* __restrict__ present) {
  const int i = blockIdx.x * blockDim.x + threadIdx.x;
  if (i >= P) return;
  const float x = means3D[3 * (size_t)i], y = means3D[3 * (size_t)i + 1], z = means3D[3 * (size_t)i + 2];
  float vz = ((viewmatrix[2] * x + viewmatrix[6] * y) + viewmatrix[10] * z) + viewmatrix[14];
  present[i] = vz > B3GS_NEAR ? 1 : 0;
}

}

PreOut b3gs_pre_out(const B3gsScene& sc, const GeomView& g, const ImgView& im, int32_t* radii) {
  PreOut o;
  o.rec = g.rec;
  o.depth_key = g.depth_key;
  o.tiles_touched = g.tiles_touched;
  o.rect = g.rect;
  o.rect_stride = 1;
  o.rect_role = 0;
  o.radii = radii;
  o.ranges = im.ranges;
  o.ranges2 = im.ranges2;
  o.open_rows = im.open_rows;
  o.span_flag = nullptr;
  o.pred_rows = nullptr;
  o.pflag = g.pflag;
  o.nrowwords = ((sc.H + B3GS_TILE - 1) / B3GS_TILE) * (((sc.W + B3GS_TILE - 1) / B3GS_TILE + 63) / 64);
  o.ntiles = ((sc.W + B3GS_TILE - 1) / B3GS_TILE) * ((sc.H + B3GS_TILE - 1) / B3GS_TILE);
  return o;
}

void b3gs_launch_preprocess(const PreBatch& pb, hipStream_t s) {
  int work = pb.sc[0].P;
  for (int v = 0; v < pb.n; v++) work = pb.out[v].ntiles > work ? pb.out[v].ntiles : work;
  if (pb.n <= 0 || work <= 0) return;
  const dim3 grid((work + 255) / 256);
  if (pb.raw_mode) hipLaunchKernelGGL(preprocess_fwd_kernel<true>, grid, dim3(256), 0, s, pb);
  else hipLaunchKernelGGL(preprocess_fwd_kernel<false>, grid, dim3(256), 0, s, pb);
}

void b3gs_launch_preprocess_backward(const SceneX& sx, const GeomView& g, const int32_t* radii, float* dL_dmeans2D,
                                     float* dL_dcolors, float* dL_dopacity, float* dL_dmeans3D, float* dL_dcov3D,
                                     float* dL_dsh, float* dL_dscales, float* dL_drotations, const B3gsRawGrads* rg,
                                     float* m2d_out, hipStream_t s) {
  if (sx.sc.P <= 0) return;
  const dim3 grid((sx.sc.P + 255) / 256);
  B3gsRawGrads none = {nullptr, nullptr, nullptr, nullptr, nullptr, nullptr};
  if (sx.raw_mode)
    hipLaunchKernelGGL(preprocess_bwd_kernel<true>, grid, dim3(256), 0, s, sx, g, radii, dL_dmeans2D, dL_dcolors,
                       dL_dopacity, dL_dmeans3D, dL_dcov3D, dL_dsh, dL_dscales, dL_drotations, *rg, m2d_out);
  else
    hipLaunchKernelGGL(preprocess_bwd_kernel<false>, grid, dim3(256), 0, s, sx, g, radii, dL_dmeans2D, dL_dcolors,
                       dL_dopacity, dL_dmeans3D, dL_dcov3D, dL_dsh, dL_dscales, dL_drotations, none, m2d_out);
}

void b3gs_launch_accumulate_views(const B3gsScene& base, const B3gsRawParams& raw, int nviews, const B3gsViewRef* views,
                                  const B3gsRawGrads& rg, int overwrite, const B3gsDensifyStats* stats, int first, int count,
                                  uint32_t* list, uint32_t* counts, hipStream_t s) {
  if (base.P <= 0 || nviews <= 0 || count <= 0) return;
  MultiViews mv;
  mv.n = nviews;
  for (int v = 0; v < nviews; v++) mv.v[v] = views[v];
  const B3gsDensifyStats ds = stats ? *stats : B3gsDensifyStats{nullptr, nullptr, nullptr, nullptr};
  static const int force = getenv("B3GS_ACC_PER_THREAD") ? atoi(getenv("B3GS_ACC_PER_THREAD")) : 0;
  const bool big = force ? force >= 4 : count >= (1 << 18) + (1 << 17);
  if (force == 2) {
    const dim3 grid((count + 511) / 512);
    hipLaunchKernelGGL(accumulate_scan_kernel<2>, grid, dim3(256), 0, s, base, mv, rg, overwrite, first, count, ds, list, counts);
    hipLaunchKernelGGL(accumulate_chain_kernel<2>, dim3(grid.x * 2), dim3(256), 0, s, base, raw, mv, rg, overwrite, first, list, counts);
  } else if (big) {
    const dim3 grid((count + 1023) / 1024);
    hipLaunchKernelGGL(accumulate_scan_kernel<4>, grid, dim3(256), 0, s, base, mv, rg, overwrite, first, count, ds, list, counts);
    hipLaunchKernelGGL(accumulate_chain_kernel<4>, dim3(grid.x * 4), dim3(256), 0, s, base, raw, mv, rg, overwrite, first, list, counts);
  } else {
    const dim3 grid((count + 255) / 256);
    hipLaunchKernelGGL(accumulate_scan_kernel<1>, grid, dim3(256), 0, s, base, mv, rg, overwrite, first, count, ds, list, counts);
    hipLaunchKernelGGL(accumulate_chain_kernel<1>, grid, dim3(256), 0, s, base, raw, mv, rg, overwrite, first, list, counts);
  }
}

void b3gs_launch_mark_visible(int32_t P, const float* means3D, const float* viewmatrix, uint8_t* present,
                              hipStream_t s) {
  if (P <= 0) return;
  hipLaunchKernelGGL(mark_visible_kernel, dim3((P + 255) / 256), dim3(256), 0, s, P, means3D, viewmatrix, present);
}


namespace {
__global__ void __launch_bounds__(256) debug_activations_kernel(SceneX sx_, float* __restrict__ scales, float* __restrict__ rot,
                                                                float* __restrict__ opacity) {
  const int i = blockIdx.x * 256 + threadIdx.x;
  if (i >= sx_.sc.P) return;
  float s[3], q[4], inv;
  load_scale_rot<true>(sx_, i, s, q, &inv);
  for (int k = 0; k < 3; k++) scales[3 * (size_t)i + k] = s[k];
  for (int k = 0; k < 4; k++) rot[4 * (size_t)i + k] = q[k];
  opacity[i] = load_opacity<true>(sx_, i);
}
}

extern "C" int b3gs_debug_activations(int32_t P, const B3gsRawParams* raw, float* scales, float* rotations, float* opacity,
                                      b3gs_stream_t stream) {
  if (P < 0 || !raw || (P > 0 && (!raw->scaling || !raw->rotation || !raw->opacity || !scales || !rotations || !opacity)))
    return b3gs_fail(B3GS_ERR_ARG, "b3gs_debug_activations", "NULL pointer or negative count");
  if (P == 0) return B3GS_OK;
  SceneX sx_{};
  sx_.sc.P = P;
  sx_.raw = *raw;
  sx_.raw_mode = 1;
  hipLaunchKernelGGL(debug_activations_kernel, dim3((P + 255) / 256), dim3(256), 0, (hipStream_t)stream, sx_, scales, rotations, opacity);
  return b3gs_launch_status("b3gs_debug_activations");
}
```

binocular3dgs_amd/csrc/render.hip:

```cpp
#include "b3gs_internal.h"
#include <cstdlib>
#include <cstring>

namespace {

typedef unsigned long long u64;

__device__ __forceinline__ unsigned lane_id() {
  return __builtin_amdgcn_mbcnt_hi(~0u, __builtin_amdgcn_mbcnt_lo(~0u, 0u));
}
__device__ __forceinline__ void clear_bit(u64& m, int j) {
#ifdef B3GS_NO_BITSET0
  m &= ~(1ull << j);
#else
  asm("s_bitset0_b64 %0, %1" : "+s"(m) : "s"(j));
#endif
}
__device__ __forceinline__ u64 uniform_u64(u64 v) {
  uint32_t lo = __builtin_amdgcn_readfirstlane((uint32_t)v);
  uint32_t hi = __builtin_amdgcn_readfirstlane((uint32_t)(v >> 32));
  return ((u64)hi << 32) | lo;
}

constexpr uint32_t B3GS_ORDER_MAGIC = 0xB365A0D1u;
__device__ __forceinline__ int tile_of_block(int bid, int ntiles) {
  const int per = (ntiles + 7) >> 3;
  return (bid & 7) * per + (bid >> 3);
}

__device__ __forceinline__ BlendView select_view(const BlendBatch& batch, int bid) {
  BlendView v = batch.v[0];
#pragma unroll
  for (int k = 1; k < B3GS_MAX_FUSED_VIEWS; k++)
    if (k < batch.n && bid >= batch.v[k].block_base) v = batch.v[k];
  return v;
}

template <int CTRL, int ROW_MASK>
__device__ __forceinline__ float dpp_add(float v) {
  int t = __builtin_amdgcn_update_dpp(0, __float_as_int(v), CTRL, ROW_MASK, 0xF, false);
  return v + __int_as_float(t);
}
template <int CHUNK>
struct TileShared {
  float4 A[CHUNK];
  float4 B[CHUNK];
  float4 C[CHUNK];
  u64 mask[4][CHUNK / 64];
};

struct TileList {
  const uint32_t* list1;
  const uint32_t* list2;
  uint32_t first1, first2, len1, total;
};
__device__ __forceinline__ TileList tile_list(const BlendView& bv, int tile, bool with_segment2) {
  uint2 r1 = bv.ranges[tile];
  if (r1.y <= r1.x) r1 = make_uint2(0u, 0u);
  uint2 r2 = with_segment2 ? bv.ranges2[tile] : make_uint2(0u, 0u);
  if (r2.y <= r2.x) r2 = make_uint2(0u, 0u);
  TileList t;
  t.list1 = bv.point_list;
  t.list2 = bv.point_list2;
  t.first1 = r1.x;
  t.first2 = r2.x;
  t.len1 = r1.y - r1.x;
  t.total = t.len1 + (r2.y - r2.x);
  return t;
}

template <int CHUNK>
__device__ __forceinline__ int stage_chunk(TileShared<CHUNK>& sh, const TileList& tl, uint32_t idx_mask,
                                           const float4* __restrict__ rec, uint32_t q0, float tile_px, float tile_py) {
  const unsigned tid = threadIdx.x;
  const uint32_t q = q0 + tid;
  int id = -1;
  uint32_t hits = 0u;
  if (CHUNK < 256 && tid >= (unsigned)CHUNK) return id;
  if (q < tl.total) {
    const uint32_t word = q < tl.len1 ? tl.list1[tl.first1 + q] : tl.list2[tl.first2 + (q - tl.len1)];
    id = (int)(word & idx_mask);
    const float4* r = rec + 4 * (size_t)id;
    const float4 r0 = r[0], r1 = r[1], r2 = r[2];
    sh.A[tid] = r0;
    sh.B[tid] = r1;
    sh.C[tid] = make_float4(r2.x, r2.y, __int_as_float(id), 0.f);
    const float lx = r0.x - r2.z - tile_px, hx = r0.x + r2.z - tile_px;
    const float ly = r0.y - r2.w - tile_py, hy = r0.y + r2.w - tile_py;
    const bool xl = (lx <= 7.0f) && (hx >= 0.0f), xr = (lx <= 15.0f) && (hx >= 8.0f);
    const bool yt = (ly <= 7.0f) && (hy >= 0.0f), yb = (ly <= 15.0f) && (hy >= 8.0f);
    hits = (uint32_t)(xl && yt) | ((uint32_t)(xr && yt) << 1) | ((uint32_t)(xl && yb) << 2) | ((uint32_t)(xr && yb) << 3);
    if (hits) {
      const float cxx = r0.z, cxy = r0.w, cyy = r1.x;
      const float tau = __logf(255.0f * r1.y) * 1.0005f + 2e-3f;
      const float icx = __builtin_amdgcn_rcpf(cxx), icy = __builtin_amdgcn_rcpf(cyy);
      const float ox = tile_px - r0.x, oy = tile_py - r0.y;
#pragma unroll 1
      for (int qd = 0; qd < 4; qd++) {
        if (!((hits >> qd) & 1u)) continue;
        const float ax = ox + (float)((qd & 1) * 8), bx = ax + 7.0f;
        const float ay = oy + (float)((qd >> 1) * 8), by = ay + 7.0f;
        const bool inside = (ax <= 0.0f) && (bx >= 0.0f) && (ay <= 0.0f) && (by >= 0.0f);
        float fmin = 3.0e38f;
#pragma unroll
        for (int e = 0; e < 2; e++) {
          const float dx = e ? bx : ax;
          const float dy = fminf(fmaxf(-cxy * dx * icy, ay), by);
          fmin = fminf(fmin, 0.5f * (cxx * dx * dx + cyy * dy * dy) + cxy * dx * dy);
          const float ey = e ? by : ay;
          const float ex = fminf(fmaxf(-cxy * ey * icx, ax), bx);
          fmin = fminf(fmin, 0.5f * (cxx * ex * ex + cyy * ey * ey) + cxy * ex * ey);
        }
        if (!(inside || !(fmin > tau))) hits &= ~(1u << qd);
      }
    }
  }
  const unsigned w = tid >> 6;
#pragma unroll
  for (int qd = 0; qd < 4; qd++) {
    const u64 m = __ballot((hits >> qd) & 1u);
    if ((tid & 63) == 0) sh.mask[qd][w] = m;
  }
  return id;
}

__device__ __forceinline__ float blend_power(const float4& A, float cyy, float dx, float dy) {
  const float q = __builtin_fmaf(cyy * dy, dy, (A.z * dx) * dx);
  return __builtin_fmaf(-A.w * dx, dy, -0.5f * q);
}

#if defined(B3GS_FWD_SENS_SALU)
#define B3GS_FWD_SENS asm volatile("s_add_u32 s2, s2, 1\n s_add_u32 s2, s2, 1\n s_add_u32 s2, s2, 1\n s_add_u32 s2, s2, 1" ::: "s2", "scc")
#elif defined(B3GS_FWD_SENS_VALU)
#define B3GS_FWD_SENS asm volatile("v_add_u32 v60, v60, 1\n v_add_u32 v61, v61, 1\n v_add_u32 v62, v62, 1\n v_add_u32 v63, v63, 1" ::: "v60", "v61", "v62", "v63")
#else
#define B3GS_FWD_SENS do { } while (0)
#endif
#ifndef B3GS_FWD_CHECK_EVERY
#define B3GS_FWD_CHECK_EVERY 4
#endif
template <int CHUNK, bool TRACE>
__device__ __forceinline__ void render_fwd_tile(const BlendView bv, int bid, unsigned slot, TileShared<CHUNK>& sh,
                                                uint32_t (&s_work)[4], unsigned long long* __restrict__ trace) {
  const unsigned long long t_start = TRACE ? __builtin_readcyclecounter() : 0ull;
  const unsigned long long r_start = TRACE ? __builtin_amdgcn_s_memrealtime() : 0ull;
  unsigned n_iter = 0, n_chunks = 0;
  const int W = bv.W, H = bv.H, grid_x = bv.grid_x, ntiles = bv.ntiles;
  const float4* __restrict__ rec = bv.rec;
  const float* __restrict__ bg = bv.bg;
  float* __restrict__ final_T = bv.final_T;
  uint32_t* __restrict__ n_contrib = bv.n_contrib;
  float* __restrict__ out_color = bv.out_color;
  float* __restrict__ out_depth = bv.out_depth;
// ... 307 lines not shown
      "ds_write_addtid_b32 %9 offset:2448"                                                       \
      :                                                                                          \
      : "v"(p[0]), "v"(p[1]), "v"(p[2]), "v"(p[3]), "v"(p[4]), "v"(p[5]), "v"(p[6]), "v"(p[7]),  \
        "v"(p[8]), "v"(p[9]), "s"(red_m0)                                                        \
      : "memory")


template <int CHUNK, bool TRACE>
__global__ void __launch_bounds__(256, B3GS_BWD_WAVES)
    render_bwd_tile_kernel(BlendBatch batch, unsigned long long* __restrict__ trace) {
  __shared__ TileSharedBwd<CHUNK> sh;
  __shared__ uint32_t s_max_last[4];
  const unsigned long long t_start = TRACE ? __builtin_readcyclecounter() : 0ull;
  const unsigned long long r_start = TRACE ? __builtin_amdgcn_s_memrealtime() : 0ull;
  unsigned n_iter = 0, n_live = 0, n_lanes = 0, n_half = 0, n_pair = 0, prev_half = 0, n_pair_last_ = 0;
  const int bid = batch.order ? 8 * (int)batch.order[(blockIdx.x & 7u) * (unsigned)batch.cls_size + (blockIdx.x >> 3)] + (int)(blockIdx.x & 7u)
                              : (int)blockIdx.x;
  const BlendView bv = select_view(batch, bid);
  const int W = bv.W, H = bv.H, grid_x = bv.grid_x, ntiles = bv.ntiles;
  const float4* __restrict__ rec = bv.rec;
  const float* __restrict__ bg = bv.bg;
  const float* __restrict__ final_T = bv.final_T;
  const uint32_t* __restrict__ n_contrib = bv.n_contrib;
  const float* __restrict__ dL_dcolor = bv.dL_dcolor;
  const float* __restrict__ dL_ddepth = bv.dL_ddepth;
  const float* __restrict__ dL_dalpha_img = bv.dL_dalpha;
  float* __restrict__ dL_dmeans2D = bv.dL_dmeans2D;
  float* __restrict__ dL_dcolors = bv.dL_dcolors;
  float* __restrict__ dL_dopacity = bv.dL_dopacity;
  float* __restrict__ dL_dcov3D = bv.dL_dcov3D;
  const unsigned cov_stride = bv.cov_stride;
  const int tile = tile_of_block(bid - bv.block_base, ntiles);
  if (tile >= ntiles) return;
  const int tile_x = tile % grid_x, tile_y = tile / grid_x;
  const unsigned tid = threadIdx.x, lane = tid & 63, w = tid >> 6;
  const int ipx = tile_x * B3GS_TILE + (int)((w & 1) * 8 + (lane & 7));
  const int ipy = tile_y * B3GS_TILE + (int)((w >> 1) * 8 + (lane >> 3));
  const bool inside = ipx < W && ipy < H;
  const TileList tl = tile_list(bv, tile, true);

  BwdPixel px;
  px.fpx = (float)ipx;
  px.fpy = (float)ipy;
  px.half_w = 0.5f * (float)W;
  px.half_h = 0.5f * (float)H;
  px.last = 0;
  px.T_final = 0.f;
  px.dCr = px.dCg = px.dCb = px.dD = px.dA = 0.f;
  if (inside) {
    const size_t pix = (size_t)ipy * W + ipx, hw = (size_t)H * W;
    px.last = n_contrib[pix];
    px.T_final = final_T[pix];
    px.dCr = dL_dcolor[pix];
    px.dCg = dL_dcolor[hw + pix];
    px.dCb = dL_dcolor[2 * hw + pix];
    if (dL_ddepth) px.dD = dL_ddepth[pix];
    if (dL_dalpha_img) px.dA = dL_dalpha_img[pix];
  }
  px.bg_dot = (bg[0] * px.dCr + bg[1] * px.dCg) + bg[2] * px.dCb;
  px.T = px.T_final;
  px.Bw = 0.f;

  {
    uint32_t m = px.last;
#pragma unroll
    for (int d = 32; d >= 1; d >>= 1) m = max(m, (uint32_t)__shfl_xor((int)m, d, 64));
    if (lane == 0) s_max_last[w] = m;
  }
  __syncthreads();
  const uint32_t max_last = max(max(s_max_last[0], s_max_last[1]), max(s_max_last[2], s_max_last[3]));
  if (max_last == 0) return;
  const uint32_t wave_last = __builtin_amdgcn_readfirstlane(s_max_last[w]);
  if (wave_last > 400) __builtin_amdgcn_s_setprio(3);
  else if (wave_last > 330) __builtin_amdgcn_s_setprio(2);
  else if (wave_last > 260) __builtin_amdgcn_s_setprio(1);

  const unsigned rk = lane >> 2, rpart = lane & 3;
  float* red_base;
  unsigned red_stride;
  if (rk < 2) { red_base = dL_dmeans2D + rk; red_stride = bv.m2d_stride; }
  else if (rk < 5) { red_base = dL_dcov3D + (rk - 2); red_stride = cov_stride; }
  else if (rk == 5) { red_base = dL_dopacity; red_stride = bv.op_stride; }
  else if (rk < 9) { red_base = dL_dcolors + (rk - 6); red_stride = bv.col_stride; }
  else { red_base = dL_dcov3D + 3; red_stride = cov_stride; }
  const bool red_writer = (rk < 10u) && (rpart == 0);
  float* const red = sh.red[w];
  static_assert(RED_STRIDE * 4 == 272, "row offsets of the ds_write_addtid_b32 block");
  const uint32_t red_m0 = __builtin_amdgcn_readfirstlane((uint32_t)(uintptr_t)(__attribute__((address_space(3))) float*)red);
  const float4* const red_rd = reinterpret_cast<const float4*>(red + (rk < 10 ? rk : 0) * RED_STRIDE + rpart * 16);

  float4 q0, q1, q2, q3;
  uint32_t pend_g = 0;
  bool pending = false;
  for (int c = (int)((max_last - 1) / CHUNK); c >= 0; c--) {
    stage_chunk(sh.f, tl, bv.idx_mask, rec, (uint32_t)(c * CHUNK), (float)(tile_x * B3GS_TILE), (float)(tile_y * B3GS_TILE));
    __syncthreads();
#pragma unroll 1
    for (int pw = CHUNK / 64 - 1; pw >= 0; pw--) {
      const uint32_t base = (uint32_t)(c * CHUNK + pw * 64);
      if (base >= wave_last) continue;
      u64 m = uniform_u64(sh.f.mask[w][pw]);
      const uint32_t lim = wave_last - base;
      if (lim < 64) m &= (1ull << lim) - 1ull;
      if (m == 0) continue;
      const float4* const sA = sh.f.A + pw * 64;
      const float4* const sB = sh.f.B + pw * 64;
      const float4* const sC = sh.f.C + pw * 64;
#if B3GS_BWD_PREFETCH
      int j = 63 - __builtin_clzll(m);
      clear_bit(m, j);
      float4 A0 = sA[j], B0 = sB[j], C0 = sC[j], A1, B1, C1;
      while (true) {
        bool more = m != 0;
        int jn = more ? 63 - __builtin_clzll(m) : j;
        clear_bit(m, jn);
        A1 = sA[jn]; B1 = sB[jn]; C1 = sC[jn];
        B3GS_BWD_CANDIDATE(A0, B0, C0, j);
        if (!more) break;
        j = jn;
        more = m != 0;
        jn = more ? 63 - __builtin_clzll(m) : j;
        clear_bit(m, jn);
        A0 = sA[jn]; B0 = sB[jn]; C0 = sC[jn];
        B3GS_BWD_CANDIDATE(A1, B1, C1, j);
        if (!more) break;
        j = jn;
      }
#else
      while (m) {
        const int j = 63 - __builtin_clzll(m);
        clear_bit(m, j);
        const float4 A0 = sA[j], B0 = sB[j], C0 = sC[j];
        B3GS_BWD_CANDIDATE(A0, B0, C0, j);
      }
#endif
    }
    __syncthreads();
  }
  if (pending) B3GS_RETIRE_PENDING();
  if (TRACE && lane == 0) {
    unsigned long long* t = trace + 4 * ((size_t)blockIdx.x * 4 + w);
    t[0] = __builtin_readcyclecounter() - t_start;
    t[1] = (r_start << 32) | (__builtin_amdgcn_s_memrealtime() & 0xFFFFFFFFull);
    t[2] = (unsigned long long)n_iter | ((unsigned long long)(n_half & 0xFFFFu) << 32) | ((unsigned long long)(n_pair & 0xFFFFu) << 48);
    t[3] = (unsigned long long)n_live | ((unsigned long long)n_lanes << 32);
  }
}

template <int SC>
struct WaveSharedBwd {
  float4 A[SC], B[SC], C[SC];
  float red[10 * RED_STRIDE];
};
template <bool TRACE, int SC, bool REGS, bool ROWS>
__global__ void __launch_bounds__(64, REGS ? B3GS_BWD_QWAVES : B3GS_BWD_WAVES)
    render_bwd_kernel(BlendBatch batch, unsigned long long* __restrict__ trace) {
  __shared__ WaveSharedBwd<REGS ? 1 : SC> sh;
  const unsigned long long t_start = TRACE ? __builtin_readcyclecounter() : 0ull;
  const unsigned long long r_start = TRACE ? __builtin_amdgcn_s_memrealtime() : 0ull;
  unsigned n_iter = 0, n_live = 0, n_lanes = 0, n_half = 0, n_pair = 0, prev_half = 0, n_pair_last_ = 0;
#ifdef B3GS_BWD_QUAD_LINEAR
  const unsigned w = blockIdx.x & 3u, blk = blockIdx.x >> 2;
#else
  const unsigned w = (blockIdx.x >> 3) & 3u, blk = ((blockIdx.x >> 5) << 3) | (blockIdx.x & 7u);
#endif
  const int bid = batch.order ? 8 * (int)batch.order[(blk & 7u) * (unsigned)batch.cls_size + (blk >> 3)] + (int)(blk & 7u) : (int)blk;
  const BlendView bv = select_view(batch, bid);
  const int W = bv.W, H = bv.H, grid_x = bv.grid_x, ntiles = bv.ntiles;
  const float4* __restrict__ rec = bv.rec;
  const float* __restrict__ bg = bv.bg;
  float* __restrict__ dL_dmeans2D = bv.dL_dmeans2D;
  float* __restrict__ dL_dcolors = bv.dL_dcolors;
  float* __restrict__ dL_dopacity = bv.dL_dopacity;
  float* __restrict__ dL_dcov3D = bv.dL_dcov3D;
  const unsigned cov_stride = bv.cov_stride;
  const int tile = tile_of_block(bid - bv.block_base, ntiles);
  if (tile >= ntiles) return;
  const int tile_x = tile % grid_x, tile_y = tile / grid_x;
  const unsigned lane = threadIdx.x;
  const int ipx = tile_x * B3GS_TILE + (int)((w & 1) * 8 + (lane & 7));
  const int ipy = tile_y * B3GS_TILE + (int)((w >> 1) * 8 + (lane >> 3));
  const bool inside = ipx < W && ipy < H;
  const TileList tl = tile_list(bv, tile, true);

  BwdPixel px;
  px.fpx = (float)ipx;
  px.fpy = (float)ipy;
  px.half_w = 0.5f * (float)W;
  px.half_h = 0.5f * (float)H;
  px.last = 0;
  px.T_final = 0.f;
  px.dCr = px.dCg = px.dCb = px.dD = px.dA = 0.f;
  if (inside) {
    const size_t pix = (size_t)ipy * W + ipx, hw = (size_t)H * W;
    px.last = bv.n_contrib[pix];
    px.T_final = bv.final_T[pix];
    px.dCr = bv.dL_dcolor[pix];
    px.dCg = bv.dL_dcolor[hw + pix];
    px.dCb = bv.dL_dcolor[2 * hw + pix];
    if (bv.dL_ddepth) px.dD = bv.dL_ddepth[pix];
    if (bv.dL_dalpha) px.dA = bv.dL_dalpha[pix];
  }
  px.bg_dot = (bg[0] * px.dCr + bg[1] * px.dCg) + bg[2] * px.dCb;
  px.T = px.T_final;
  px.Bw = 0.f;
  uint32_t wave_last = px.last;
#pragma unroll
  for (int d = 32; d >= 1; d >>= 1) wave_last = max(wave_last, (uint32_t)__shfl_xor((int)wave_last, d, 64));
  wave_last = __builtin_amdgcn_readfirstlane(wave_last);
  if (wave_last == 0) {
    if (TRACE && lane == 0) {
      unsigned long long* t = trace + 4 * ((size_t)blk * 4 + w);
      t[0] = 0ull;
      t[1] = (r_start << 32) | (r_start & 0xFFFFFFFFull);
      t[2] = 0ull;
      t[3] = 0ull;
    }
    return;
  }
  if (wave_last > 400) __builtin_amdgcn_s_setprio(3);
  else if (wave_last > 330) __builtin_amdgcn_s_setprio(2);
  else if (wave_last > 260) __builtin_amdgcn_s_setprio(1);

  const unsigned rk = lane >> 2, rpart = lane & 3;
  float* red_base;
  unsigned red_stride;
  if (rk < 2) { red_base = dL_dmeans2D + rk; red_stride = bv.m2d_stride; }
  else if (rk < 5) { red_base = dL_dcov3D + (rk - 2); red_stride = cov_stride; }
  else if (rk == 5) { red_base = dL_dopacity; red_stride = bv.op_stride; }
  else if (rk < 9) { red_base = dL_dcolors + (rk - 6); red_stride = bv.col_stride; }
  else { red_base = dL_dcov3D + 3; red_stride = cov_stride; }
  const bool red_writer = (rk < 10u) && (rpart == 0);
  const uint32_t red_col4 = 4u * (rk < 2 ? 4u + rk : (rk < 5 ? rk - 2u : (rk == 5 ? 9u : (rk < 9 ? rk : 3u))));
  const uint32_t row_bytes = 4u * cov_stride;
  char* const row0 = reinterpret_cast<char*>(dL_dcov3D);
#undef B3GS_RED_ADDR
#define B3GS_RED_ADDR(g) (ROWS ? reinterpret_cast<float*>(row0 + ((g) * row_bytes + red_col4)) : red_base + __umul24((g), red_stride))
  float* const red = sh.red;
  const uint32_t red_m0 = __builtin_amdgcn_readfirstlane((uint32_t)(uintptr_t)(__attribute__((address_space(3))) float*)red);
  const float4* const red_rd = reinterpret_cast<const float4*>(red + (rk < 10 ? rk : 0) * RED_STRIDE + rpart * 16);
  float4 q0, q1, q2, q3;
  uint32_t pend_g = 0;
  bool pending = false;

  const float qx0 = (float)((w & 1) * 8), qy0 = (float)((w >> 1) * 8);
  const float tile_px = (float)(tile_x * B3GS_TILE), tile_py = (float)(tile_y * B3GS_TILE);
  for (int c = (int)((wave_last - 1) / (uint32_t)SC); c >= 0; c--) {
    const uint32_t base = (uint32_t)c * (uint32_t)SC;
    const uint32_t q = base + lane;
    bool hit = false;
    float4 r0 = make_float4(0.f, 0.f, 0.f, 0.f), r1 = r0, r2 = r0;
    int id = 0;
    if ((SC == 64 || lane < (unsigned)SC) && q < tl.total && q < wave_last) {
      const uint32_t word = q < tl.len1 ? tl.list1[tl.first1 + q] : tl.list2[tl.first2 + (q - tl.len1)];
      id = (int)(word & bv.idx_mask);
      const float4* r = rec + 4 * (size_t)id;
      r0 = r[0]; r1 = r[1]; r2 = r[2];
      if (!REGS) {
        sh.A[lane] = r0;
        sh.B[lane] = r1;
        sh.C[lane] = make_float4(r2.x, r2.y, __int_as_float(id), 0.f);
      }
      const float ax = (tile_px + qx0) - r0.x, bx = ax + 7.0f;
      const float ay = (tile_py + qy0) - r0.y, by = ay + 7.0f;
      hit = (ax <= r2.z) && (bx >= -r2.z) && (ay <= r2.w) && (by >= -r2.w);
      if (hit) {
        const float cxx = r0.z, cxy = r0.w, cyy = r1.x;
        const float tau = __logf(255.0f * r1.y) * 1.0005f + 2e-3f;
        const float icx = __builtin_amdgcn_rcpf(cxx), icy = __builtin_amdgcn_rcpf(cyy);
        const bool in_rect = (ax <= 0.0f) && (bx >= 0.0f) && (ay <= 0.0f) && (by >= 0.0f);
        float fmin = 3.0e38f;
#pragma unroll
        for (int e = 0; e < 2; e++) {
          const float dx = e ? bx : ax;
          const float dy = fminf(fmaxf(-cxy * dx * icy, ay), by);
          fmin = fminf(fmin, 0.5f * (cxx * dx * dx + cyy * dy * dy) + cxy * dx * dy);
          const float ey = e ? by : ay;
          const float ex = fminf(fmaxf(-cxy * ey * icx, ax), bx);
          fmin = fminf(fmin, 0.5f * (cxx * ex * ex + cyy * ey * ey) + cxy * ex * ey);
        }
        hit = in_rect || !(fmin > tau);
      }
    }
    u64 m = __ballot(hit);
    __builtin_amdgcn_fence(__ATOMIC_RELEASE, "wavefront");
    __builtin_amdgcn_wave_barrier();
    __builtin_amdgcn_fence(__ATOMIC_ACQUIRE, "wavefront");
    if (REGS) {
      typedef const float __attribute__((address_space(4))) cfloat_k;
      while (m) {
        const int j = 63 - __builtin_clzll(m);
        clear_bit(m, j);
        const int idj = __builtin_amdgcn_readlane(id, j);
        cfloat_k* rs = (cfloat_k*)(uintptr_t)(rec + 4 * (size_t)idj);
        const float4 A0 = make_float4(rs[0], rs[1], rs[2], rs[3]);
        const float4 B0 = make_float4(rs[4], rs[5], rs[6], rs[7]);
        const float4 C0 = make_float4(rs[8], rs[9], __int_as_float(idj), 0.f);
        B3GS_BWD_CANDIDATE(A0, B0, C0, j);
      }
    } else if (m != 0) {
      const float4* const sA = sh.A;
      const float4* const sB = sh.B;
      const float4* const sC = sh.C;
      int j = 63 - __builtin_clzll(m);
      clear_bit(m, j);
      float4 A0 = sA[j], B0 = sB[j], C0 = sC[j], A1, B1, C1;
      while (true) {
        bool more = m != 0;
        int jn = more ? 63 - __builtin_clzll(m) : j;
        clear_bit(m, jn);
        A1 = sA[jn]; B1 = sB[jn]; C1 = sC[jn];
        B3GS_BWD_CANDIDATE(A0, B0, C0, j);
        if (!more) break;
        j = jn;
        more = m != 0;
        jn = more ? 63 - __builtin_clzll(m) : j;
        clear_bit(m, jn);
        A0 = sA[jn]; B0 = sB[jn]; C0 = sC[jn];
        B3GS_BWD_CANDIDATE(A1, B1, C1, j);
        if (!more) break;
        j = jn;
      }
    }
    __builtin_amdgcn_fence(__ATOMIC_RELEASE, "wavefront");
    __builtin_amdgcn_wave_barrier();
  }
  if (pending) B3GS_RETIRE_PENDING();
  if (TRACE && lane == 0) {
    unsigned long long* t = trace + 4 * ((size_t)blk * 4 + w);
    t[0] = __builtin_readcyclecounter() - t_start;
    t[1] = (r_start << 32) | (__builtin_amdgcn_s_memrealtime() & 0xFFFFFFFFull);
    t[2] = (unsigned long long)n_iter | ((unsigned long long)(n_half & 0xFFFFu) << 32) | ((unsigned long long)(n_pair & 0xFFFFu) << 48);
    t[3] = (unsigned long long)n_live | ((unsigned long long)n_lanes << 32);
  }
}
#undef B3GS_BWD_CANDIDATE
#undef B3GS_ROW_WRITES
#undef B3GS_RETIRE_PENDING
#undef B3GS_RED_ADDR

#ifndef B3GS_FWD_CHUNK
#define B3GS_FWD_CHUNK 256
#endif
constexpr int FWD_CHUNK = B3GS_FWD_CHUNK;
unsigned long long* g_bwd_trace = nullptr;
size_t g_bwd_trace_words = 0;
unsigned long long* trace_buffer(int nblocks) {
  if (g_bwd_trace && g_bwd_trace_words < (size_t)nblocks * 16) {
    (void)hipFree(g_bwd_trace);
    g_bwd_trace = nullptr;
  }
  if (!g_bwd_trace) {
    (void)hipMalloc((void**)&g_bwd_trace, (size_t)nblocks * 16 * sizeof(unsigned long long));
    g_bwd_trace_words = (size_t)nblocks * 16;
  }
  return g_bwd_trace;
}
constexpr int BWD_CHUNK = 64;

}

namespace {
int blocks_of(const BlendView& v) { return ((v.ntiles + 7) / 8) * 8; }
}

namespace {
bool order_fits(const BlendBatch& batch, int total, uint32_t* sig_off, uint32_t* sig) {
  const size_t words = (size_t)B3GS_MAX_FUSED_VIEWS * (size_t)(batch.v[0].ntiles + 8);
  *sig_off = (uint32_t)(words - 2);
  *sig = (uint32_t)total * 16u + (uint32_t)batch.n;
  return (size_t)total <= words - 2;
}
}

void b3gs_launch_blend_forward(BlendBatch batch, hipStream_t s) {
  int total = 0;
  for (int k = 0; k < batch.n; k++) {
    batch.v[k].block_base = total;
    total += blocks_of(batch.v[k]);
  }
  if (total <= 0) return;
  static const bool lpt = getenv("B3GS_NO_LPT") == nullptr && getenv("B3GS_NO_FWD_LPT") == nullptr;
  batch.order = nullptr;
  batch.cls_size = total / 8;
  if (lpt && batch.order_buf && order_fits(batch, total, &batch.sig_off, &batch.sig)) batch.order = batch.order_buf;
  if (batch.v[0].round == 1) {
    batch.order = nullptr;
    hipLaunchKernelGGL((render_fwd_repair_kernel<FWD_CHUNK>), dim3(total < REBLEND_GRID ? total : REBLEND_GRID), dim3(256), 0, s,
                       batch, total);
    return;
  }
  static const bool fwd_trace = getenv("B3GS_FWD_TRACE") != nullptr;
  if (fwd_trace)
    hipLaunchKernelGGL((render_fwd_kernel<FWD_CHUNK, true>), dim3(total), dim3(256), 0, s, batch, trace_buffer(total));
  else
    hipLaunchKernelGGL((render_fwd_kernel<FWD_CHUNK, false>), dim3(total), dim3(256), 0, s, batch, nullptr);
}

namespace {
constexpr int ORDER_CACHE = 4096;
__global__ void __launch_bounds__(256) blend_order_kernel(BlendBatch batch, uint32_t* __restrict__ order, int cls_size,
                                                          int view_groups) {
  __shared__ uint32_t hist[256], cursor[256], s_max[4], tmp[8];
  const int c = (int)blockIdx.x;
  const unsigned lane = threadIdx.x & 63u, w = threadIdx.x >> 6;
  const uint32_t levels = 256u / (uint32_t)view_groups;
  auto work_of = [&](int q) -> uint32_t {
    const int bid = 8 * q + c;
    int k = 0;
    for (int j = 1; j < batch.n; j++) k = bid >= batch.v[j].block_base ? j : k;
    const BlendView bv = select_view(batch, bid);
    const int tile = tile_of_block(bid - bv.block_base, bv.ntiles);
    const uint32_t wk = tile < bv.ntiles ? min(bv.tile_work[tile], 0xFFFFFFu) : 0u;
    return wk | ((uint32_t)(k * view_groups / batch.n) << 24);
  };
  __shared__ uint32_t s_work[ORDER_CACHE];
  for (int q = (int)threadIdx.x; q < cls_size && q < ORDER_CACHE; q += 256) s_work[q] = work_of(q);
  __syncthreads();
  auto work_at = [&](int q) -> uint32_t { return q < ORDER_CACHE ? s_work[q] : work_of(q); };
  uint32_t m = 0;
  for (int q = (int)threadIdx.x; q < cls_size; q += 256) m = max(m, work_at(q) & 0xFFFFFFu);
#pragma unroll
  for (int d = 32; d >= 1; d >>= 1) m = max(m, (uint32_t)__shfl_xor((int)m, d, 64));
  if (lane == 0) s_max[w] = m;
  hist[threadIdx.x] = 0;
  __syncthreads();
  const float scale = (float)(levels - 1u) / (float)max(max(max(s_max[0], s_max[1]), max(s_max[2], s_max[3])), 1u);
  auto bucket_of = [&](uint32_t wk) -> uint32_t {
    return (wk >> 24) * levels + (levels - 1u) - (uint32_t)((float)(wk & 0xFFFFFFu) * scale);
  };
  for (int q = (int)threadIdx.x; q < cls_size; q += 256) atomicAdd(&hist[bucket_of(work_at(q))], 1u);
  __syncthreads();
  {
    const uint32_t v = hist[threadIdx.x];
    uint32_t inc = v;
#pragma unroll
    for (int d = 1; d < 64; d <<= 1) {
      const uint32_t o = (uint32_t)__shfl_up((int)inc, d, 64);
      if (lane >= (unsigned)d) inc += o;
    }
    if (lane == 63) tmp[w] = inc;
    __syncthreads();
    uint32_t base = 0;
    for (unsigned k = 0; k < w; k++) base += tmp[k];
    cursor[threadIdx.x] = base + inc - v;
  }
  __syncthreads();
  for (int q = (int)threadIdx.x; q < cls_size; q += 256) {
    const uint32_t b = bucket_of(work_at(q));
    order[(size_t)c * cls_size + atomicAdd(&cursor[b], 1u)] = (uint32_t)q;
  }
  if (c == 0 && threadIdx.x == 0) {
    order[batch.sig_off] = B3GS_ORDER_MAGIC;
    order[batch.sig_off + 1] = batch.sig;
  }
}
}

void b3gs_launch_blend_backward(BlendBatch batch, hipStream_t s) {
  int total = 0;
  for (int k = 0; k < batch.n; k++) {
    batch.v[k].block_base = total;
    total += blocks_of(batch.v[k]);
  }
  if (total <= 0) return;
  static const bool lpt = getenv("B3GS_NO_LPT") == nullptr;
  uint32_t* order = batch.order_buf;
  batch.order = nullptr;
  batch.cls_size = total / 8;
  if (lpt && order && order_fits(batch, total, &batch.sig_off, &batch.sig)) {
    static const int groups_env = getenv("B3GS_BWD_VIEW_GROUPS") ? atoi(getenv("B3GS_BWD_VIEW_GROUPS")) : 0;
    const int want = groups_env > 0 ? groups_env : (batch.n + 2) / 3;
    const int groups = want < 1 ? 1 : (want > batch.n ? batch.n : want);
    hipLaunchKernelGGL(blend_order_kernel, dim3(8), dim3(256), 0, s, batch, order, batch.cls_size, groups);
    batch.order = order;
  }
  static const bool bwd_trace = getenv("B3GS_BWD_TRACE") != nullptr;
  unsigned long long* trace = bwd_trace ? trace_buffer(total) : nullptr;
  static const int bwd_chunk = getenv("B3GS_BWD_CHUNK") ? atoi(getenv("B3GS_BWD_CHUNK")) : BWD_CHUNK;
  static const char* which = getenv("B3GS_BWD_KERNEL");
  const bool tile_wg = which && !strcmp(which, "tile"), wave_lds = which && !strcmp(which, "wave");
  if (!tile_wg) {
    bool rows = true;
    for (int k = 0; k < batch.n; k++) {
      const BlendView& v = batch.v[k];
      rows = rows && v.m2d_stride == v.cov_stride && v.col_stride == v.cov_stride && v.op_stride == v.cov_stride &&
             v.dL_dmeans2D == v.dL_dcov3D + 4 && v.dL_dcolors == v.dL_dcov3D + 6 && v.dL_dopacity == v.dL_dcov3D + 9 &&
             (uint64_t)v.cov_stride * 4u * (uint64_t)(v.idx_mask == 0xFFFFFFFFu ? 0x7FFFFFFFu : v.idx_mask) < 0xFFFFFFFFull;
    }
    if (trace) hipLaunchKernelGGL((render_bwd_kernel<true, 64, true, false>), dim3(total * 4), dim3(64), 0, s, batch, trace);
    else if (wave_lds) hipLaunchKernelGGL((render_bwd_kernel<false, 64, false, false>), dim3(total * 4), dim3(64), 0, s, batch, trace);
    else if (rows) hipLaunchKernelGGL((render_bwd_kernel<false, 64, true, true>), dim3(total * 4), dim3(64), 0, s, batch, trace);
    else hipLaunchKernelGGL((render_bwd_kernel<false, 64, true, false>), dim3(total * 4), dim3(64), 0, s, batch, trace);
    return;
  }
  if (trace) hipLaunchKernelGGL((render_bwd_tile_kernel<64, true>), dim3(total), dim3(256), 0, s, batch, trace);
  else if (bwd_chunk == 256) hipLaunchKernelGGL((render_bwd_tile_kernel<256, false>), dim3(total), dim3(256), 0, s, batch, trace);
  else if (bwd_chunk == 128) hipLaunchKernelGGL((render_bwd_tile_kernel<128, false>), dim3(total), dim3(256), 0, s, batch, trace);
  else hipLaunchKernelGGL((render_bwd_tile_kernel<64, false>), dim3(total), dim3(256), 0, s, batch, trace);
}

BlendView b3gs_blend_view(const B3gsScene& sc, const GeomView& g, const BinView& b, const ImgView& im) {
  BlendView v;
  memset(&v, 0, sizeof(v));
  v.W = sc.W;
  v.H = sc.H;
  v.grid_x = (sc.W + B3GS_TILE - 1) / B3GS_TILE;
  v.ntiles = v.grid_x * ((sc.H + B3GS_TILE - 1) / B3GS_TILE);
  v.ranges = im.ranges;
  v.point_list = b.val[0];
  v.ranges2 = im.ranges2;
  v.point_list2 = b.val[0];
  v.tile_work = im.tile_work;
  v.open_rows = nullptr;
  v.pred_rows = nullptr;
  v.pred_next = nullptr;
  v.z_clear = nullptr;
  v.z_base = 0u;
  v.open_count = im.header + 3;
  v.row_words = (v.grid_x + 63) / 64;
  v.round = 0;
  const int idx_bits = b3gs_packed_idx_bits(sc.P, sc.W, sc.H);
  v.idx_mask = (idx_bits < 0 || idx_bits >= 32) ? 0xFFFFFFFFu : ((1u << idx_bits) - 1u);
  v.rec = g.rec;
  static const bool no_staged = getenv("B3GS_NO_STAGED") != nullptr;
  v.staged = no_staged ? nullptr : g.staged;
  v.epoch = g.header + B3GS_GEOM_EPOCH;
  v.bg = sc.background;
  v.final_T = im.final_T;
  v.n_contrib = im.n_contrib;
  return v;
}

extern "C" size_t b3gs_debug_bwd_trace(unsigned long long* host, size_t max_words) {
  if (!g_bwd_trace) return 0;
  (void)hipDeviceSynchronize();
  size_t n = g_bwd_trace_words < max_words ? g_bwd_trace_words : max_words;
  (void)hipMemcpy(host, g_bwd_trace, n * sizeof(unsigned long long), hipMemcpyDeviceToHost);
  return n;
}
```

binocular3dgs_amd/fused.py:

```python
from __future__ import annotations

import ctypes as C
import math
from typing import List, Optional, Sequence

import torch

from . import _lib

MAX_BATCH = 8


class _Slot:
    def __init__(self, P, W, H, capacity, dev, want_means2D, scratch_floats, stream, n_dev):
        L = _lib.lib()
        u8 = dict(dtype=torch.uint8, device=dev)
        self.geom = torch.empty(L.b3gs_geometry_bytes(P), **u8)
        self.binning = torch.empty(L.b3gs_binning_bytes(P, capacity), **u8)
        self.img = torch.zeros(L.b3gs_image_bytes(W, H), **u8)
        self.capacity = capacity
        f = dict(dtype=torch.float32, device=dev)
        self.color = torch.empty((3, H, W), **f)
        self.depth = torch.empty((1, H, W), **f)
        self.alpha = torch.empty((1, H, W), **f)
        self.radii = torch.zeros((P,), dtype=torch.int32, device=dev)
        self.n_dev = n_dev
        self.means2D_grad = torch.zeros((P, 3), **f) if want_means2D else None
        self.scratch = torch.zeros(max(scratch_floats, 1), **f)
        self.stream = stream


class _ViewOutputs(dict):

    def __missing__(self, key):
        if key == "visibility_filter":
            self[key] = self["radii"] > 0
            return self[key]
        raise KeyError(key)


class _RasterizeBatch(torch.autograd.Function):

    @staticmethod
    def forward(ctx, xyz, f_dc, f_rest, scaling, rotation, opacity, owner, specs):
        owner._forward_batch(specs)
        ctx.owner, ctx.specs = owner, specs
        ctx.set_materialize_grads(False)
        outs = []
        for sp in specs:
            s = owner.slots[sp["slot"]]
            ctx.mark_non_differentiable(s.radii)
            outs += [s.color, s.radii, s.depth, s.alpha]
        return tuple(outs)

    @staticmethod
    def backward(ctx, *grads):
        per_view = [(grads[4 * k], grads[4 * k + 2], grads[4 * k + 3]) for k in range(len(ctx.specs))]
        ctx.owner._backward_batch(ctx.specs, per_view)
        return (None,) * 8


class FusedRasterizer:
    def __init__(self, model, width: int, height: int, num_slots: int = 2, binning_capacity: Optional[int] = None,
                 want_means2D: bool = True, concurrent: bool = True, schedule: Optional[str] = None,
                 seg1_fraction="auto", reference_binning: bool = False):
        self.model = model
        self.reference_binning = bool(reference_binning)
        self.W, self.H = int(width), int(height)
        p = model.get_xyz
        if not p.is_cuda:
            raise _lib.B3gsError("FusedRasterizer needs the model on an MI355X (HIP) device")
        self.dev = p.device
        self.P = p.shape[0]
        self.K = model._features_dc.shape[1] + model._features_rest.shape[1]
        self.capacity = int(binning_capacity) if binning_capacity else max(4_000_000, 12 * self.P)
        self.schedule = schedule or ("batched" if concurrent else "serial")
        assert self.schedule in ("batched", "groups", "streams", "serial")
        self.concurrent = self.schedule == "streams"
        self._want_m2d = want_means2D
        self.two_round_min_instances = 2_000_000
        self.two_round_max_miss_rate = 0.3
        self.two_round_disabled = None
        self._seg1_auto = seg1_fraction == "auto"
        self.seg1_fraction = 0.0 if self._seg1_auto else float(seg1_fraction)
        self._n_all = torch.zeros((num_slots,), dtype=torch.int32, device=self.dev)
        self.high_water = torch.zeros((num_slots,), dtype=torch.int32, device=self.dev)
        self.overflow_flag = torch.zeros((1,), dtype=torch.int32, device=self.dev)
        self.depth_key_bits = 27
        self.slots: List[_Slot] = [self._new_slot(torch.cuda.Stream(self.dev), k) for k in range(num_slots)]
        self._deferred = None
        self._params = _lib.B3gsRawParams()
        self._grads = _lib.B3gsRawGrads()

    def _new_slot(self, stream, index):
        L = _lib.lib()
        return _Slot(self.P, self.W, self.H, self.capacity, self.dev, self._want_m2d,
                     L.b3gs_backward_scratch_floats(self.P), stream, self._n_all[index:index + 1])

    def _scene(self, sp) -> _lib.B3gsScene:
        cam, m = sp["cam"], self.model
        return _lib.B3gsScene(self.P, int(m.active_sh_degree), int(self.K), self.W, self.H,
                              math.tan(cam.FoVx * 0.5), math.tan(cam.FoVy * 0.5), float(sp["scaling_modifier"]), 0,
                              int(bool(sp["debug"])), sp["bg"].data_ptr(), None, None, None, None, None, None, None,
                              cam.world_view_transform.data_ptr(), cam.full_proj_transform.data_ptr(),
                              cam.camera_center.data_ptr())

    def _bind_params(self):
        m, rp = self.model, self._params
        rp.xyz, rp.features_dc = m._xyz.data_ptr(), m._features_dc.data_ptr()
        rp.features_rest = m._features_rest.data_ptr() if m._features_rest.numel() else None
        rp.scaling, rp.rotation, rp.opacity = m._scaling.data_ptr(), m._rotation.data_ptr(), m._opacity.data_ptr()
        return rp

    def _bind_grads(self):
        m, gr = self.model, self._grads
        for name, p in (("xyz", m._xyz), ("features_dc", m._features_dc), ("features_rest", m._features_rest),
                        ("scaling", m._scaling), ("rotation", m._rotation), ("opacity", m._opacity)):
            if p.grad is None:
                p.grad = torch.zeros_like(p)
            setattr(gr, name, p.grad.data_ptr() if p.numel() else None)
        return gr

    def _blend_table(self, specs, scenes, grads=None):
        arr = (_lib.B3gsBlendView * len(specs))()
        keep = []
        for k, (sp, sc) in enumerate(zip(specs, scenes)):
            s = self.slots[sp["slot"]]
            arr[k].view = C.pointer(sc)
            arr[k].geometry, arr[k].binning, arr[k].image = s.geom.data_ptr(), s.binning.data_ptr(), s.img.data_ptr()
            arr[k].out_color, arr[k].out_depth, arr[k].out_alpha = s.color.data_ptr(), s.depth.data_ptr(), s.alpha.data_ptr()
            arr[k].binning_capacity = s.capacity
            if grads is not None:
                gc, gd, ga = grads[k]
                if gc is None:
                    gc = torch.zeros((3, self.H, self.W), dtype=torch.float32, device=self.dev)
                gc = gc.contiguous()
                gd = None if gd is None else gd.contiguous()
                ga = None if ga is None else ga.contiguous()
                keep += [gc, gd, ga]
                arr[k].dL_dcolor = gc.data_ptr()
                arr[k].dL_ddepth = None if gd is None else gd.data_ptr()
                arr[k].dL_dalpha = None if ga is None else ga.data_ptr()
                arr[k].scratch = s.scratch.data_ptr()
        return arr, keep

    def _forward_batch(self, specs):
        self._forward_batch_launch(specs)
        if self.schedule not in ("batched", "groups"):
            torch.maximum(self.high_water, self._n_all, out=self.high_water)
            self.overflow_flag.bitwise_or_((self._n_all > self.capacity).any().to(torch.int32))

    def _forward_batch_launch(self, specs):
        L = _lib.lib()
        main = torch.cuda.current_stream(self.dev)
        scenes = [self._scene(sp) for sp in specs]
        rp = self._bind_params()
        if self.schedule in ("batched", "groups"):
            if self.schedule == "groups" and len(specs) > 2:
                per = min(MAX_BATCH - MAX_BATCH % 2, max(2, 2 * (-(-len(specs) // (2 * getattr(self, "groups", 2))))))
                bounds = list(range(0, len(specs), per))
            else:
                per, bounds = MAX_BATCH, list(range(0, len(specs), MAX_BATCH))
            streams = [main] + [self.slots[k].stream for k in range(1, len(bounds))] if len(bounds) > 1 and self.schedule == "groups" else None
            for gi, c0 in enumerate(bounds):
                chunk = specs[c0:c0 + per]
                st = main
                if streams is not None:
                    st = streams[gi]
                    if st is not main:
                        st.wait_stream(main)
                arr = (_lib.B3gsForwardView * len(chunk))()
                for k, sp in enumerate(chunk):
                    s = self.slots[sp["slot"]]
                    arr[k].view = C.pointer(scenes[c0 + k])
                    arr[k].geometry, arr[k].binning, arr[k].image = s.geom.data_ptr(), s.binning.data_ptr(), s.img.data_ptr()
                    arr[k].binning_capacity = s.capacity
                    arr[k].out_color, arr[k].out_depth, arr[k].out_alpha = (s.color.data_ptr(), s.depth.data_ptr(),
                                                                            s.alpha.data_ptr())
                    arr[k].radii, arr[k].device_num_rendered = s.radii.data_ptr(), s.n_dev.data_ptr()
                    donor = getattr(sp["cam"], "same_depth_as", None)
                    arr[k].depth_order_from = -1
                    arr[k].seg1_fraction = self.seg1_fraction
                    arr[k].reference_binning = int(self.reference_binning)
                    arr[k].high_water = self.high_water[sp["slot"]:sp["slot"] + 1].data_ptr()
                    arr[k].overflow_flag = self.overflow_flag.data_ptr()
                    arr[k].depth_key_bits = sp.get("key_bits", self.depth_key_bits)
                    for j in range(k):
                        if donor is not None and chunk[j]["cam"] is donor and arr[j].depth_order_from == -1:
                            arr[k].depth_order_from = j
                            arr[k].hint_trusted = 1 if j == k - 1 else 0
                rc = L.b3gs_forward_raw_batch(len(chunk), arr, C.byref(rp), 3, st.cuda_stream)
                _lib.check(rc, "b3gs_forward_raw_batch")
            if streams is not None:
                for st in streams[1:]:
                    main.wait_stream(st)
            return
        if self.concurrent:
            for sp, sc in zip(specs, scenes):
                s = self.slots[sp["slot"]]
                s.stream.wait_stream(main)
                rc = L.b3gs_forward_raw(C.byref(sc), C.byref(rp), s.geom.data_ptr(), s.binning.data_ptr(), s.capacity,
                                        s.img.data_ptr(), s.color.data_ptr(), s.depth.data_ptr(), s.alpha.data_ptr(),
                                        s.radii.data_ptr(), s.n_dev.data_ptr(), 3, s.stream.cuda_stream)
                _lib.check(rc, "b3gs_forward_raw")
            for sp in specs:
                main.wait_stream(self.slots[sp["slot"]].stream)
            return
        for sp, sc in zip(specs, scenes):
            s = self.slots[sp["slot"]]
            rc = L.b3gs_forward_raw(C.byref(sc), C.byref(rp), s.geom.data_ptr(), s.binning.data_ptr(), s.capacity,
                                    s.img.data_ptr(), None, None, None, s.radii.data_ptr(), s.n_dev.data_ptr(), 1,
                                    main.cuda_stream)
            _lib.check(rc, "b3gs_forward_raw(phase 1)")
        for c0 in range(0, len(specs), MAX_BATCH):
            arr, _ = self._blend_table(specs[c0:c0 + MAX_BATCH], scenes[c0:c0 + MAX_BATCH])
            _lib.check(L.b3gs_blend_forward_batch(len(arr), arr, main.cuda_stream), "b3gs_blend_forward_batch")

    def _backward_batch(self, specs, grads):
        L = _lib.lib()
        stream = torch.cuda.current_stream(self.dev)
        scenes = [self._scene(sp) for sp in specs]
        for c0 in range(0, len(specs), MAX_BATCH):
            arr, keep = self._blend_table(specs[c0:c0 + MAX_BATCH], scenes[c0:c0 + MAX_BATCH], grads[c0:c0 + MAX_BATCH])
            _lib.check(L.b3gs_blend_backward_batch(len(arr), arr, stream.cuda_stream), "b3gs_blend_backward_batch")
            del keep
        pend = list(zip(specs, scenes))
        if self._deferred is not None:
            self._deferred += pend
        else:
            self._accumulate(pend, overwrite=False)

    def _accumulate(self, pend, overwrite: bool, grads=None, first: int = 0, count: Optional[int] = None,
                    touched_rows: Optional[torch.Tensor] = None, stats_target=None):
        L, m = _lib.lib(), self.model
        gr = grads if grads is not None else self._bind_grads()
        if touched_rows is not None:
            if not overwrite or len(pend) > MAX_BATCH:
                raise _lib.B3gsError("sparse gradient rows need overwrite mode and at most 8 views (one accumulate call)")
            assert touched_rows.dtype == torch.int64 and touched_rows.numel() >= (self.P + 63) // 64
        if grads is None or touched_rows is not None:
            gr.touched_rows = None if touched_rows is None else touched_rows.data_ptr()
        count = self.P - first if count is None else count
        stats = None
        if getattr(m, "denom", None) is not None and m.denom.numel() == self.P:
            ta, td, tr = stats_target if stats_target is not None else (m.xyz_gradient_accum, m.denom, m.max_radii2D)
            stats = _lib.B3gsDensifyStats(ta.data_ptr(), td.data_ptr(), tr.data_ptr(), self.overflow_flag.data_ptr())
        stream = torch.cuda.current_stream(self.dev).cuda_stream
        for c0 in range(0, len(pend), MAX_BATCH):
            chunk = pend[c0:c0 + MAX_BATCH]
            arr = (_lib.B3gsFusedView * len(chunk))()
            for k, (sp, sc) in enumerate(chunk):
                sl = self.slots[sp["slot"]]
                arr[k].view = C.pointer(sc)
                arr[k].radii, arr[k].geometry = sl.radii.data_ptr(), sl.geom.data_ptr()
                arr[k].scratch = sl.scratch.data_ptr()
                arr[k].dL_dmeans2D = None if sl.means2D_grad is None else sl.means2D_grad.data_ptr()
                arr[k].densify_stats = int(bool(sp["densify_stats"]) and stats is not None)
            rc = L.b3gs_backward_raw_accumulate_range(len(chunk), arr, C.byref(self._bind_params()), C.byref(gr),
                                                      int(bool(overwrite) and c0 == 0),
                                                      None if stats is None else C.byref(stats), first, count, stream)
            _lib.check(rc, "b3gs_backward_raw_accumulate_range")

    def render(self, viewpoint_camera, bg_color: torch.Tensor, slot: int = 0, scaling_modifier: float = 1.0,
               debug: bool = False) -> dict:
        return self.render_batch([(viewpoint_camera, slot)], bg_color, scaling_modifier, debug)[0]

    def render_batch(self, views: Sequence, bg_color: torch.Tensor, scaling_modifier: float = 1.0,
                     debug: bool = False, _span_checked: bool = False) -> List[dict]:
        m = self.model
        key_bits = self.depth_key_bits if (torch.is_grad_enabled() or _span_checked) else 0
        specs = tuple({"cam": v[0], "slot": int(v[1]), "densify_stats": bool(v[2]) if len(v) > 2 else False,
                       "bg": bg_color, "scaling_modifier": scaling_modifier, "debug": debug, "key_bits": key_bits}
                      for v in views)
        assert len({sp["slot"] for sp in specs}) == len(specs), "each view of a batch needs its own slot"
        flat = _RasterizeBatch.apply(m._xyz, m._features_dc, m._features_rest, m._scaling, m._rotation, m._opacity,
                                     self, specs)
        out = []
        for k, sp in enumerate(specs):
            color, radii, depth, alpha = flat[4 * k:4 * k + 4]
            out.append(_ViewOutputs({"render": color, "viewspace_points_grad": self.slots[sp["slot"]].means2D_grad,
                                     "radii": radii, "rendered_depth": depth, "rendered_alpha": alpha}))
        return out

    def begin_deferred(self):
        self._deferred = []

    def take_deferred(self):
        pend, self._deferred = self._deferred, None
        return pend

    def accumulate_range(self, pend, grads, first: int, count: int, overwrite: bool = True, stats_target=None):
        self._accumulate(pend, overwrite, grads, first, count, stats_target=stats_target)

    def finish_views(self, pend, overwrite: bool = True):
        if not pend:
            if overwrite:
                for p in self.model.parameters():
                    if p.grad is not None:
                        p.grad.zero_()
            return
        self._accumulate(pend, overwrite)

    def finish_deferred(self, overwrite: bool = True, touched_rows: Optional[torch.Tensor] = None):
        pend, self._deferred = self._deferred, None
        if not pend:
            if overwrite:
                for p in self.model.parameters():
                    if p.grad is not None:
                        p.grad.zero_()
                if touched_rows is not None:
                    touched_rows.fill_(-1)
            return
        self._accumulate(pend, overwrite, touched_rows=touched_rows)

    def resize(self):
        self.P = self.model.get_xyz.shape[0]
        self.capacity = max(self.capacity, 12 * self.P)
        for i in range(len(self.slots)):
            self.slots[i] = self._new_slot(self.slots[i].stream, i)
        self.high_water.zero_()
        self.overflow_flag.zero_()

    def num_rendered(self):
        torch.cuda.synchronize(self.dev)
        return [int(s.n_dev.item()) for s in self.slots]

    def overflowed(self) -> bool:
        return any(n > self.capacity for n in self.num_rendered())

    def grow(self, factor: float = 1.5, need: Optional[int] = None):
        need = max(self.num_rendered() + [self.capacity, int(need or 0)])
        self.capacity = int(need * factor)
        for i in range(len(self.slots)):
            self.slots[i] = self._new_slot(self.slots[i].stream, i)
        self.high_water.zero_()

    def check_overflow(self) -> int:
        hw = int(self.high_water.max().item())
        flag = int(self.overflow_flag.item())
        self.high_water.zero_()
        timed_out = self._check_repair_status()
        if hw <= self.capacity and not flag and not timed_out:
            return 0
        self.overflow_flag.zero_()
        if flag & 8:
            raise _lib.B3gsError("B3GS_ERR_ARG: a view was rendered from the depth order of the camera it names as "
                                 "`same_depth_as`, but its depth keys differ (the z rows of the two view matrices are not the "
                                 "same bits); the steps since the last check were dropped on the device")
        if flag & 2:
            self.depth_key_bits = 0
        if (flag & 4) or timed_out:
            self.seg1_fraction = 0.0
            self._seg1_auto = False
            self.two_round_disabled = "grid-barrier time-out of the second binning round"
        if hw > self.capacity or (flag & 1):
            self.grow(need=hw)
        return max(hw, 1)

    def repair_rate(self, reset: bool = False):
        w = self.slots[0].img[:48].view(torch.int32)
        missed, total = int(w[10].item()), int(w[11].item())
        if reset:
            w[10:12] = 0
        return missed, total

    def _check_repair_status(self):
        if self.seg1_fraction <= 0.0 or not self.slots:
            return False
        if self._seg1_auto and not torch.cuda.is_current_stream_capturing():
            missed, total = self.repair_rate(reset=True)
            if total >= 8 and missed > self.two_round_max_miss_rate * total:
                self.seg1_fraction = 0.0
                self.two_round_disabled = (missed, total)
        st = int(self.slots[0].img[:48].view(torch.int32)[9].item())
        if st:
            self.slots[0].img[:48].view(torch.int32)[9] = 0
        return bool(st)

    def fit_capacity(self, views: Sequence, bg_color: torch.Tensor, margin: float = 1.3) -> int:
        frac, self.seg1_fraction = self.seg1_fraction, 0.0
        with torch.no_grad():
            self.render_batch([(v[0], v[1]) for v in views], bg_color, _span_checked=True)
        need = max(self.num_rendered())
        self.high_water.zero_()
        if int(self.overflow_flag.item()) & 2:
            self.depth_key_bits = 0
        self.overflow_flag.zero_()
        if need * margin > self.capacity:
            self.grow(factor=margin, need=need)
        self.seg1_fraction = (0.0 if (need < self.two_round_min_instances or self.two_round_disabled)
                              else min(0.125, max(0.02, 0.75e6 / need))) if self._seg1_auto else frac
        if self.seg1_fraction > 0.0:
            with torch.no_grad():
                self.render_batch([(v[0], v[1]) for v in views], bg_color, _span_checked=True)
            self.high_water.zero_()
        return self.capacity
```

binocular3dgs_amd/step.py:

```python
from __future__ import annotations

from typing import Callable, List, Optional, Sequence, Tuple

import torch
import torch.distributed as dist

from .render import PipelineParams, render


def _dist_on(group=None) -> bool:
    return dist.is_available() and dist.is_initialized()


class FlatGradSlab:

    def __init__(self, params: Sequence[torch.nn.Parameter], padded_numel: int = 0):
        self.params = list(params)
        self.force_collective = False
        total = sum(p.numel() for p in self.params)
        self.numel = total
        dev = self.params[0].device
        self.flat = torch.zeros(max(total, int(padded_numel)), dtype=torch.float32, device=dev)
        off = 0
        self.views: List[torch.Tensor] = []
# ... 421 lines not shown
            return self._reduce_and_update_pipelined()
        self._agree_on_overflow()
        if self._pending_views is not None:
            self.slab.rebind()
            self.fused.finish_views(self._pending_views, overwrite=True)
        mask, self._row_mask = self._row_mask, None
        if isinstance(self.optimizer, ShardedAdam):
            self.slab.rebind()
            return self.optimizer.step(self.slab, average=self.average, row_mask=mask)
        assert mask is None or isinstance(self.optimizer, FusedAdam)
        self.slab.all_reduce(self.average, self.group)
        if self.optimizer is not None:
            self.slab.rebind()
            if mask is not None:
                self.optimizer.step(row_mask=mask)
            else:
                self.optimizer.step()

    def _agree_on_overflow(self, group=None):
        group = group if group is not None else self.group
        if self.fused is not None and _dist_on() and dist.get_world_size(group) > 1:
            dist.all_reduce(self.fused.overflow_flag, op=dist.ReduceOp.MAX, group=group)

    def densify_and_prune(self, max_grad: float, min_opacity: float, extent: float, max_screen_size=None,
                          percent_dense: float = 0.01, noise=None, generator=None, group=None) -> int:
        from .densify import densify_and_prune
        group = group if group is not None else self.group
        self.check_capacity()
        self.sync_densify_stats(group)
        if noise is None and generator is None and _dist_on() and dist.get_world_size(group) > 1:
            P, dev = self.model.get_xyz.shape[0], self.model.get_xyz.device
            noise = torch.randn((2, P, 3), device=dev) if dist.get_rank(group) == 0 else torch.empty((2, P, 3), device=dev)
            dist.broadcast(noise, src=dist.get_global_rank(group, 0) if group is not None else 0, group=group)
        newP = densify_and_prune(self.model, self.optimizer, max_grad, min_opacity, extent, max_screen_size,
                                 percent_dense, noise, generator)
        self.slab = FlatGradSlab(self.model.parameters(), getattr(self.optimizer, "padded_numel", 0))
        if self.range_slab is not None:
            self.range_slab = RangeGradSlab(self.model.parameters(), self.pipeline_ranges)
        if self.fused is not None:
            self.fused.resize()
            if self.views:
                self.fused.fit_capacity([(v.cam, v.slot) for v in self.views], self.bg)
        return newP

    def _reduce_and_update_pipelined(self, group=None):
        from . import _lib
        rs, fr, opt = self.range_slab, self.fused, self.optimizer
        group = group if group is not None else self.group
        collective = self._collective(group)
        m = self.model
        staged = None
        if fr is not None and getattr(m, "denom", None) is not None and m.denom.numel() == rs.P:
            if self._staged_stats is None or self._staged_stats[0].numel() != rs.P:
                self._staged_stats = tuple(torch.zeros(rs.P, dtype=torch.float32, device=rs.flat.device) for _ in range(3))
            staged = self._staged_stats
        if fr is not None:
            rs.flag.copy_(fr.overflow_flag)
        else:
            rs.flag.zero_()
        skip_keep = getattr(opt, "skip_flag", None)
        if fr is not None and hasattr(opt, "skip_flag"):
            opt.skip_flag = rs.flag_word
        ev = None
        if self.tail_events is not None:
            mk = lambda: torch.cuda.Event(enable_timing=True)
            ev = {"start": mk(), "issued": [mk() for _ in range(rs.K)], "reduced": [mk() for _ in range(rs.K)], "end": mk()}
            ev["start"].record()
        works = []
        for r in range(rs.K):
            first, count = rs.rows(r)
            gr = _lib.B3gsRawGrads()
            for name, ptr, w in zip(("xyz", "features_dc", "features_rest", "scaling", "rotation", "opacity"),
                                    rs.grad_ptrs(r), rs.widths):
                setattr(gr, name, (ptr - 4 * w * first) if w else None)
            if self._pending_views:
                fr.accumulate_range(self._pending_views, gr, first, count, overwrite=True, stats_target=staged)
            if ev:
                ev["issued"][r].record()
            works.append(dist.all_reduce(rs.chunk(r), op=dist.ReduceOp.SUM, group=group, async_op=True) if collective else None)
        for r in range(rs.K):
            if works[r] is not None:
                works[r].wait()
            if r == 0 and staged is not None:
                rc = _lib.lib().b3gs_apply_staged_densify_stats(
                    rs.P, staged[0].data_ptr(), staged[1].data_ptr(), staged[2].data_ptr(), m.xyz_gradient_accum.data_ptr(),
                    m.denom.data_ptr(), m.max_radii2D.data_ptr(), rs.flag_word.data_ptr(), fr.overflow_flag.data_ptr(),
                    torch.cuda.current_stream(rs.flat.device).cuda_stream)
                _lib.check(rc, "b3gs_apply_staged_densify_stats")
            elif r == 0 and fr is not None:
                fr.overflow_flag.bitwise_or_((rs.flag_word != 0).to(torch.int32))
            if ev:
                ev["reduced"][r].record()
            if self.average and collective:
                rs.chunk(r).div_(dist.get_world_size(group))
            first, count = rs.rows(r)
            opt.step_rows(first, count, rs.grad_ptrs(r), last=(r == rs.K - 1))
        if fr is not None and hasattr(opt, "skip_flag"):
            opt.skip_flag = skip_keep
        if ev:
            ev["end"].record()
            self.tail_events.append(ev)

    def sync_densify_stats(self, group=None):
        m = self.model
        if not _dist_on() or getattr(m, "denom", None) is None:
            return
        group = group if group is not None else self.group
        dist.all_reduce(m.xyz_gradient_accum, op=dist.ReduceOp.SUM, group=group)
        dist.all_reduce(m.denom, op=dist.ReduceOp.SUM, group=group)
        dist.all_reduce(m.max_radii2D, op=dist.ReduceOp.MAX, group=group)

    def _exchange(self, sends, recvs):
        if not sends and not recvs:
            return
        ops = [dist.P2POp(dist.isend, t, p, self.group) for t, p in sends] + \
              [dist.P2POp(dist.irecv, t, p, self.group) for t, p in recvs]
        for w in dist.batch_isend_irecv(ops):
            w.wait()

    def _render_views(self):
        if self.fused is not None:
            return self.fused.render_batch([(v.cam, v.slot, v.role == 0 and self.densify_stats) for v in self.views], self.bg)
        return [self.render(v.cam, self.model, self.pipe, self.bg) for v in self.views]

    def compute_grads(self, pair_grad_fn=None, loss_fn=None, batch_loss_fn=None):
        assert sum(f is not None for f in (pair_grad_fn, loss_fn, batch_loss_fn)) == 1
        assert batch_loss_fn is None or self.fused is not None
        if not self.views:
            self.slab.zero()
            self._pending_views = None
            if self.range_slab is not None:
                self.range_slab.flat.zero_()
                self._pending_views = []
            self.last_stats = {"views": 0}
            return 0
        if self.fused is not None:
            self.slab.rebind()
            self.fused.begin_deferred()
        else:
            self.slab.zero()
        pkgs = self._render_views()
        outs, grads = [], []
        if pair_grad_fn is not None:
            for k, v in enumerate(self.views):
                if v.role == 1 and v.mate is not None:
                    continue
                prim = pkgs[k] if v.role == 0 else None
                shif = pkgs[v.mate] if (v.role == 0 and v.mate is not None) else (pkgs[k] if v.role == 1 else None)
                for o, g in pair_grad_fn(v.key, prim, shif):
                    outs.append(o)
                    grads.append(g)
        else:
            outs, grads = self._loss_pixel_grads(pkgs, loss_fn, batch_loss_fn)
        if outs:
            torch.autograd.backward(outs, grads)
        if self.fused is None:
            self._update_densify_stats(pkgs)
        if self.fused is not None:
            if not self._chain_rule_after_agreement():
                self._pending_views = None
                self._row_mask = self._sparse_rows()
                self.fused.finish_deferred(overwrite=True, touched_rows=self._row_mask)
            else:
                self._pending_views = self.fused.take_deferred()
        self.last_stats = {"views": len(self.views)}
        return len(self.views)

    def _update_densify_stats(self, pkgs):
        m = self.model
        if getattr(m, "denom", None) is None or m.denom.shape[0] != m.get_xyz.shape[0]:
            return
        with torch.no_grad():
            for v, pkg in zip(self.views, pkgs):
                g = pkg["viewspace_points"].grad if v.role == 0 else None
                if g is None:
                    continue
                vis = pkg["visibility_filter"]
                m.update_max_radii(pkg["radii"], vis)
                m._accumulate_stats(g, vis)

    def _loss_pixel_grads(self, pkgs, loss_fn, batch_loss_fn):
        def leaf(t):
            return t.detach().requires_grad_(True)

        dev = self.bg.device
        H, W = pkgs[0]["render"].shape[-2:]
        sends, recvs = [], []
        for k, v in enumerate(self.views):
            if v.peer is None:
                continue
            if v.role == 1:
                sends.append((pkgs[k]["render"].detach(), v.peer))
            else:
                if k not in self._recv_img:
                    self._recv_img[k] = torch.empty((3, H, W), dtype=torch.float32, device=dev)
                recvs.append((self._recv_img[k], v.peer))
        self._exchange(sends, recvs)
        leaves, items = {}, []
        for k, v in enumerate(self.views):
            if v.role != 0:
                continue
            lp = dict(pkgs[k])
            for name in ("render", "rendered_depth", "rendered_alpha"):
                lp[name] = leaf(pkgs[k][name])
            leaves[k] = lp
            sp = None
            if v.mate is not None:
                sp = dict(pkgs[v.mate])
                sp["render"] = leaf(pkgs[v.mate]["render"])
                leaves[v.mate] = sp
            elif v.peer is not None:
                sp = {"render": leaf(self._recv_img[k])}
                leaves[("remote", k)] = sp
            items.append((v.key, v.cam, lp, sp, v.t))
        if items:
            if batch_loss_fn is not None:
                total = batch_loss_fn(items)
            else:
                losses = [loss_fn(*it) for it in items]
                total = losses[0]
                for extra in losses[1:]:
                    total = total + extra
            one = self._one if getattr(self, "_one", None) is not None and self._one.device == total.device and \
                self._one.dtype == total.dtype and self._one.shape == total.shape else None
            if one is None:
                one = self._one = torch.ones_like(total)
            torch.autograd.backward([total], [one])
        sends, recvs = [], []
        for k, v in enumerate(self.views):
            if v.peer is None:
                continue
            if v.role == 0:
                g = leaves[("remote", k)]["render"].grad
                sends.append((g if g is not None else torch.zeros((3, H, W), dtype=torch.float32, device=dev), v.peer))
            else:
                if k not in self._recv_grad:
                    self._recv_grad[k] = torch.empty((3, H, W), dtype=torch.float32, device=dev)
                recvs.append((self._recv_grad[k], v.peer))
        self._exchange(sends, recvs)
        outs, grads = [], []
        for k, v in enumerate(self.views):
            if v.role == 1 and v.peer is not None:
                outs.append(pkgs[k]["render"])
                grads.append(self._recv_grad[k])
                continue
            lp = leaves.get(k)
            if lp is None:
                continue
            for name in (("render", "rendered_depth", "rendered_alpha") if v.role == 0 else ("render",)):
                if lp[name].grad is not None:
                    outs.append(pkgs[k][name])
                    grads.append(lp[name].grad)
        return outs, grads
```

include/b3gs_raster.h:

```cpp
#ifndef B3GS_RASTER_H
#define B3GS_RASTER_H

#include <stddef.h>
#include <stdint.h>

#ifdef __cplusplus
extern "C" {
#endif

#define B3GS_ABI_VERSION 18
#define B3GS_TILE 16

typedef enum B3gsStatus {
  B3GS_OK = 0,
  B3GS_ERR_ARG = -1,
  B3GS_ERR_ALLOC = -2,
  B3GS_ERR_HIP = -3,
  B3GS_ERR_CAPACITY = -4,
  B3GS_ERR_NO_DEVICE = -5
} B3gsStatus;

typedef void* b3gs_stream_t;

typedef char* (*b3gs_alloc_fn)(void* user, size_t bytes);

typedef struct B3gsScene {
  int32_t P;
  int32_t D;
  int32_t M;
  int32_t W, H;
  float tan_fovx, tan_fovy;
  float scale_modifier;
  int32_t prefiltered;
  int32_t debug;
  const float* background;
  const float* means3D;
  const float* shs;
  const float* colors_precomp;
  const float* opacities;
  const float* scales;
  const float* rotations;
  const float* cov3D_precomp;
  const float* viewmatrix;
  const float* projmatrix;
  const float* campos;
} B3gsScene;

size_t b3gs_geometry_bytes(int32_t P);
size_t b3gs_image_bytes(int32_t W, int32_t H);
size_t b3gs_binning_bytes(int32_t P, int64_t num_rendered);

int b3gs_forward(const B3gsScene* scene,
                 b3gs_alloc_fn geometry_alloc, void* geometry_user,
                 b3gs_alloc_fn binning_alloc, void* binning_user,
                 b3gs_alloc_fn image_alloc, void* image_user,
                 float* out_color, float* out_depth, float* out_alpha, int32_t* radii,
                 int32_t* host_num_rendered, b3gs_stream_t stream);

int b3gs_forward_capacity(const B3gsScene* scene, char* geometry, char* binning, int64_t binning_capacity,
                          char* image, float* out_color, float* out_depth, float* out_alpha, int32_t* radii,
                          int32_t* device_num_rendered, b3gs_stream_t stream);

int b3gs_backward(const B3gsScene* scene, int32_t num_rendered, const int32_t* radii,
                  const char* geometry, const char* binning, const char* image,
                  const float* dL_dcolor, const float* dL_ddepth, const float* dL_dalpha,
                  float* dL_dmeans2D, float* dL_dcolors, float* dL_dopacity, float* dL_dmeans3D,
                  float* dL_dcov3D, float* dL_dsh, float* dL_dscales, float* dL_drotations,
                  b3gs_stream_t stream);

typedef struct B3gsRawParams {
  const float* xyz;
  const float* features_dc;
  const float* features_rest;
  const float* scaling;
  const float* rotation;
  const float* opacity;
} B3gsRawParams;
typedef struct B3gsRawGrads {
  float* xyz; float* features_dc; float* features_rest; float* scaling; float* rotation; float* opacity;
  uint64_t* touched_rows;
} B3gsRawGrads;

int b3gs_forward_raw(const B3gsScene* view, const B3gsRawParams* params, char* geometry, char* binning,
                     int64_t binning_capacity, char* image, float* out_color, float* out_depth, float* out_alpha,
                     int32_t* radii, int32_t* device_num_rendered, int phases, b3gs_stream_t stream);

typedef struct B3gsForwardView {
  const B3gsScene* view;
  char* geometry;
  char* binning;
  int64_t binning_capacity;
  char* image;
  float* out_color;
  float* out_depth;
  float* out_alpha;
  int32_t* radii;
  int32_t* device_num_rendered;
  int32_t depth_order_from;
  float seg1_fraction;
  int32_t* high_water;
  int32_t* overflow_flag;
  int32_t depth_key_bits;
  int32_t fresh_image;
  const char* depth_order_hint;
  int32_t* hint_mismatch;
  int32_t hint_trusted;
  uint8_t* visible;
  int32_t reference_binning;
} B3gsForwardView;
int b3gs_forward_raw_batch(int32_t nviews, const B3gsForwardView* views, const B3gsRawParams* params, int phases,
                           b3gs_stream_t stream);

typedef struct B3gsBlendView {
  const B3gsScene* view;
  const char* geometry;
  const char* binning;
  const char* image;
  float* out_color;
  float* out_depth;
  float* out_alpha;
  const float* dL_dcolor;
  const float* dL_ddepth;
  const float* dL_dalpha;
  float* scratch;
  int64_t binning_capacity;
} B3gsBlendView;
int b3gs_blend_forward_batch(int32_t nviews, const B3gsBlendView* views, b3gs_stream_t stream);
int b3gs_blend_backward_batch(int32_t nviews, const B3gsBlendView* views, b3gs_stream_t stream);

size_t b3gs_backward_scratch_floats(int32_t P);
int b3gs_backward_raw(const B3gsScene* view, const B3gsRawParams* params, const int32_t* radii, const char* geometry,
                      const char* binning, const char* image, const float* dL_dcolor, const float* dL_ddepth,
                      const float* dL_dalpha, float* scratch, const B3gsRawGrads* grads, float* dL_dmeans2D,
                      int phases, b3gs_stream_t stream);

typedef struct B3gsFusedView {
  const B3gsScene* view;
  const int32_t* radii;
  const char* geometry;
  float* scratch;
  float* dL_dmeans2D;
  int32_t densify_stats;
} B3gsFusedView;
typedef struct B3gsDensifyStats {
  float* xyz_gradient_accum;
  float* denom;
  float* max_radii2D;
  const int32_t* skip_if_nonzero;
} B3gsDensifyStats;
int b3gs_backward_raw_accumulate(int32_t nviews, const B3gsFusedView* views, const B3gsRawParams* params,
                                 const B3gsRawGrads* grads, int32_t overwrite, const B3gsDensifyStats* stats,
                                 b3gs_stream_t stream);
int b3gs_backward_raw_accumulate_range(int32_t nviews, const B3gsFusedView* views, const B3gsRawParams* params,
                                       const B3gsRawGrads* grads, int32_t overwrite, const B3gsDensifyStats* stats,
                                       int32_t first, int32_t count, b3gs_stream_t stream);

typedef struct B3gsAdamSegment {
  float* param;
  const float* grad;
  float* exp_avg;
  float* exp_avg_sq;
  int64_t count;
  float lr;
  int32_t row_len;
  int32_t first_row;
  const float* lr_dev;
} B3gsAdamSegment;
#define B3GS_ADAM_STEP_WORDS (2 + 64 * 32)
int b3gs_adam_step(int32_t nseg, const B3gsAdamSegment* segs, int32_t* device_step, float beta1, float beta2,
                   float eps, float opacity_decay, int32_t opacity_segment, int32_t opacity_decay_first,
                   int32_t bump_step_after, const uint64_t* row_mask, const int32_t* skip_if_nonzero,
                   b3gs_stream_t stream);

typedef struct B3gsLossIO {
  int32_t W, H;
  const float* image;
  const float* depth;
  const float* alpha;
  const float* gt_image;
  const float* shifted_image;
  const float* alpha_weight;
  float focal_x, trans_dist, lambda_dssim, lambda_smooth, grad_scale;
  float* dL_dimage;
  float* dL_ddepth;
  float* dL_dalpha;
  float* dL_dshifted;
  float* parts;
  float* workspace;
  const float* trans_dist_dev;
} B3gsLossIO;
size_t b3gs_loss_workspace_floats(int32_t W, int32_t H);
int b3gs_binocular_loss(const B3gsLossIO* io, b3gs_stream_t stream);
int b3gs_binocular_loss_batch(int32_t npairs, const B3gsLossIO* ios, b3gs_stream_t stream);

typedef struct B3gsDensifyIO {
  int32_t P, M;
  const float* param[6];
  const float* exp_avg[6];
  const float* exp_avg_sq[6];
  const float* xyz_gradient_accum;
  const float* denom;
  float grad_threshold, min_opacity, extent, percent_dense, max_screen_size;
} B3gsDensifyIO;
int b3gs_densify_classify(const B3gsDensifyIO* io, int32_t* flags, b3gs_stream_t stream);
int b3gs_densify_scatter(const B3gsDensifyIO* io, const int32_t* flags, const int32_t* off_keep,
                         const int32_t* off_clone, const int32_t* off_split, int32_t n_keep, int32_t n_clone,
                         int32_t n_split, const float* noise, float* const* out_param, float* const* out_exp_avg,
                         float* const* out_exp_avg_sq, b3gs_stream_t stream);

size_t b3gs_lossfn_workspace_floats(int64_t planes, int32_t H, int32_t W);

int b3gs_l1_loss_forward(const float* x, const float* y, const float* mask, int64_t batch, int32_t channels, int64_t hw,
                         float* out, float* workspace, b3gs_stream_t stream);
int b3gs_l1_loss_backward(const float* x, const float* y, const float* mask, int64_t batch, int32_t channels, int64_t hw,
                          const float* grad_out, float* grad_x, float* grad_y, float* grad_mask, b3gs_stream_t stream);

int b3gs_inverse_warp_forward(const float* image, const float* disparity, int32_t B, int32_t C, int32_t H, int32_t W,
                              float* out, float* zero_fill, b3gs_stream_t stream);
int b3gs_inverse_warp_backward(const float* image, const float* disparity, const float* grad_out, int32_t B, int32_t C,
                               int32_t H, int32_t W, float* grad_image, float* grad_disparity, b3gs_stream_t stream);

int b3gs_smooth_loss_forward(const float* disparity, const float* image, int32_t B, int32_t C, int32_t H, int32_t W,
                             float* out, float* workspace, b3gs_stream_t stream);
int b3gs_smooth_loss_backward(const float* disparity, const float* image, int32_t B, int32_t C, int32_t H, int32_t W,
                              const float* grad_out, float* grad_disparity, float* grad_image, b3gs_stream_t stream);

int b3gs_ssim_forward(const float* img1, const float* img2, int32_t batch, int32_t channels, int32_t H, int32_t W,
                      int32_t size_average, float* maps, int32_t maps_for_img2, float* out, float* workspace,
                      b3gs_stream_t stream);
int b3gs_ssim_backward(const float* img1, const float* img2, const float* maps, int32_t batch, int32_t channels, int32_t H,
                       int32_t W, int32_t size_average, const float* grad_out, float* grad_img1, float* grad_img2,
                       b3gs_stream_t stream);

int b3gs_opacity_decay(float* opacity, int64_t count, float factor, b3gs_stream_t stream);
int b3gs_add_densification_stats(int64_t P, const float* viewspace_grad, int64_t row_stride, const uint8_t* update_filter,
                                 float* xyz_gradient_accum, float* denom, b3gs_stream_t stream);
int b3gs_apply_staged_densify_stats(int64_t P, float* staged_accum, float* staged_denom, float* staged_max_radii,
                                    float* xyz_gradient_accum, float* denom, float* max_radii2D, const int32_t* agreed_word,
                                    int32_t* local_overflow_flag, b3gs_stream_t stream);
int b3gs_adam_step_at(int32_t nseg, const B3gsAdamSegment* segs, int32_t step, float beta1, float beta2, float eps,
                      b3gs_stream_t stream);

#define B3GS_METRIC_CLAMP 1
#define B3GS_METRIC_QUANTIZE 2
typedef struct B3gsMetricView {
  const float* image;
  const float* gt;
  const float* mask;
  int32_t mask_channels;
  float* prepared_image;
  float* prepared_gt;
} B3gsMetricView;
size_t b3gs_image_metrics_workspace_bytes(int32_t nviews, int32_t C, int32_t H, int32_t W);
int b3gs_image_metrics_batch(int32_t nviews, const B3gsMetricView* views, int32_t C, int32_t H, int32_t W, int32_t mode,
                             double* out, void* workspace, b3gs_stream_t stream);

#define B3GS_MAX_FRAME_VIEWS 8
typedef struct B3gsFrameView {
  const float* rgb;
  const float* depth;
  const float* alpha;
  uint8_t* rgb_out;
  uint8_t* gray_out;
  uint8_t* cmap_out;
} B3gsFrameView;
size_t b3gs_frames_workspace_bytes(int32_t nviews, int32_t H, int32_t W);
int b3gs_encode_frames_batch(int32_t nviews, const B3gsFrameView* views, int32_t H, int32_t W, double percentile,
                             const uint8_t* lut, void* workspace, double* bounds_out, b3gs_stream_t stream);

#define B3GS_MAX_GT_VIEWS 8
typedef struct B3gsGtView {
  const uint8_t* src;
  int32_t Hs, Ws, C;
  const int32_t* tab_x;
  const int32_t* tab_y;
  int32_t ks_x, ks_y;
  float* image;
  float* alpha;
  float* bg_mask;
} B3gsGtView;
size_t b3gs_gt_workspace_bytes(int32_t nviews, const B3gsGtView* views, int32_t H, int32_t W);
int b3gs_prepare_gt_batch(int32_t nviews, const B3gsGtView* views, int32_t H, int32_t W, int32_t white_background,
                          float dtu_threshold, void* workspace, b3gs_stream_t stream);

size_t b3gs_cloud_workspace_bytes(int64_t n);
int b3gs_triangulate_matches(int32_t N, const float* proj_ref, const float* proj_src, const float* intrinsic,
                             const float* w2c_ref, const float* w2c_src, const float* kp_ref, const float* kp_src,
                             const uint8_t* image, int32_t W, int32_t H, float reproj_threshold, float* points,
                             uint8_t* colors, int32_t* count, void* workspace, b3gs_stream_t stream);
int b3gs_background_sheet(const uint8_t* image, int32_t W, int32_t H, const float* inv_intrinsic_t, const float* c2w,
                          float depth, float* points, uint8_t* colors, int32_t* count, void* workspace,
                          b3gs_stream_t stream);
#define B3GS_CLOUD_MAX_VIEWS 16
typedef struct B3gsCloudGrow {
  int32_t W, H, n_views;
  int32_t ref, src;
  int32_t n_seeds, n_samples;
  int32_t n_start;
  int32_t h_patch_size;
  int32_t init;
  float fx, fy, cx, cy, alpha, ssim_threshold;
  const uint8_t* images;
  const float* w2c;
  const float* window;
  const int32_t* seed_idx;
  const float* noise;
  float* points;
  float* colors;
// ... 194 lines not shown
```

Before: 481.7 iters/s.

## Fuse visibility pre-scan into blend backward and split accumulate into post and chain kernels

Moves the per-Gaussian visibility and staging scan out of the accumulate kernel into a separate prescan. The prescan can run inside the blend-backward launch when planned ahead, and the accumulate path becomes a post kernel working only on listed entries plus the chain kernel. The aim is to cut the full P-wide radii/stage read pass and to overlap it with blend backward work. In exchange it adds new API entry points, planning state in Python, atomicOr-based touched-row writes, and a dependency on scratch rows being valid only for listed Gaussians.

```diff
diff --git a/binocular3dgs_amd/_lib.py b/binocular3dgs_amd/_lib.py
--- a/binocular3dgs_amd/_lib.py
+++ b/binocular3dgs_amd/_lib.py
@@ -149,6 +149,7 @@
            "b3gs_adam_step", "b3gs_forward_raw_batch", "b3gs_loss_workspace_floats", "b3gs_binocular_loss",
            "b3gs_densify_classify", "b3gs_densify_scatter", "b3gs_knn_workspace_bytes", "b3gs_knn_mean_dist2",
            "b3gs_backward_raw_accumulate_range", "b3gs_binocular_loss_batch",
+           "b3gs_blend_backward_prescan", "b3gs_backward_raw_accumulate_prescanned",
            "b3gs_lossfn_workspace_floats", "b3gs_l1_loss_forward", "b3gs_l1_loss_backward", "b3gs_inverse_warp_forward",
            "b3gs_inverse_warp_backward", "b3gs_smooth_loss_forward", "b3gs_smooth_loss_backward", "b3gs_ssim_forward",
            "b3gs_ssim_backward", "b3gs_opacity_decay", "b3gs_add_densification_stats", "b3gs_adam_step_at", "b3gs_debug_activations",
@@ -229,6 +230,12 @@
                                                      C.POINTER(B3gsRawGrads), C.c_int32, C.POINTER(B3gsDensifyStats),
                                                      C.c_int32, C.c_int32, C.c_void_p]
     L.b3gs_backward_raw_accumulate_range.restype = C.c_int
+    L.b3gs_blend_backward_prescan.argtypes = [C.c_int32, C.POINTER(B3gsBlendView), C.POINTER(B3gsFusedView),
+                                              C.POINTER(B3gsRawParams), C.POINTER(B3gsRawGrads), C.c_int32,
+                                              C.POINTER(B3gsDensifyStats), C.c_int32, C.c_void_p]
+    L.b3gs_blend_backward_prescan.restype = C.c_int
+    L.b3gs_backward_raw_accumulate_prescanned.argtypes = L.b3gs_backward_raw_accumulate.argtypes
+    L.b3gs_backward_raw_accumulate_prescanned.restype = C.c_int
     L.b3gs_forward_raw_batch.argtypes = [C.c_int32, C.POINTER(B3gsForwardView), C.POINTER(B3gsRawParams), C.c_int,
                                          C.c_void_p]
     L.b3gs_forward_raw_batch.restype = C.c_int
diff --git a/binocular3dgs_amd/csrc/api.hip b/binocular3dgs_amd/csrc/api.hip
--- a/binocular3dgs_amd/csrc/api.hip
+++ b/binocular3dgs_amd/csrc/api.hip
@@ -1,4 +1,5 @@
 #include "b3gs_internal.h"
+#include "prescan.h"
 
 #include <cstdio>
 #include <cstdlib>
@@ -573,11 +574,8 @@
   return B3GS_OK;
 }
 
-int b3gs_blend_backward_batch(int32_t nviews, const B3gsBlendView* views, b3gs_stream_t stream) {
-  int rc = batch_views_ok(nviews, views);
-  if (rc) return rc;
-  hipStream_t s = (hipStream_t)stream;
-  BlendBatch batch;
+static int blend_backward_batch(int32_t nviews, const B3gsBlendView* views, BlendBatch* out) {
+  BlendBatch& batch = *out;
   batch.n = nviews;
   batch.order = nullptr;
   batch.order_buf = nullptr;
@@ -596,6 +594,15 @@
                                      bv.scratch + 6, bv.scratch + 9, bv.scratch, B3GS_SCRATCH_ROW, B3GS_SCRATCH_ROW,
                                      B3GS_SCRATCH_ROW, B3GS_SCRATCH_ROW);
   }
+  return B3GS_OK;
+}
+
+int b3gs_blend_backward_batch(int32_t nviews, const B3gsBlendView* views, b3gs_stream_t stream) {
+  int rc = batch_views_ok(nviews, views);
+  if (rc) return rc;
+  hipStream_t s = (hipStream_t)stream;
+  BlendBatch batch;
+  if ((rc = blend_backward_batch(nviews, views, &batch))) return rc;
   StageTimer tm(s);
   tm.mark(-1);
   b3gs_launch_blend_backward(batch, s);
@@ -611,15 +618,16 @@
   return b3gs_backward_raw_accumulate_range(nviews, views, params, grads, overwrite, stats, 0, P, stream);
 }
 
-int b3gs_backward_raw_accumulate_range(int32_t nviews, const B3gsFusedView* views, const B3gsRawParams* params,
-                                       const B3gsRawGrads* grads, int32_t overwrite, const B3gsDensifyStats* stats,
-                                       int32_t first, int32_t count, b3gs_stream_t stream) {
+static int accumulate_args(int32_t nviews, const B3gsFusedView* views, const B3gsRawParams* params, const B3gsRawGrads* grads,
+                           int32_t overwrite, const B3gsDensifyStats* stats, int32_t first, int32_t count, PrescanArgs* pa,
+                           bool* skip) {
+  *skip = false;
   if (nviews <= 0 || nviews > B3GS_MAX_FUSED_VIEWS || !views || !params || !grads)
     return fail(B3GS_ERR_ARG, "%s", "bad view count / NULL argument (at most 8 views per call)");
   const B3gsScene* v0 = views[0].view;
   int rc = check_raw(v0, params);
   if (rc) return rc;
-  if (v0->P == 0 || count == 0) return B3GS_OK;
+  if (v0->P == 0 || count == 0) { *skip = true; return B3GS_OK; }
   if (first < 0 || count < 0 || (int64_t)first + count > v0->P) return fail(B3GS_ERR_ARG, "%s", "bad Gaussian range");
   if (grads->touched_rows && overwrite && (first & 63))
     return fail(B3GS_ERR_ARG, "%s", "sparse-row gradients (touched_rows) need a range that starts at a multiple of 64");
@@ -643,10 +651,64 @@
   }
   if (stats && (!stats->xyz_gradient_accum || !stats->denom || !stats->max_radii2D))
     return fail(B3GS_ERR_ARG, "%s", "densify stats need all three arrays");
-  hipStream_t s = (hipStream_t)stream;
-  StageTimer tm(s);
-  tm.mark(-1);
-  b3gs_launch_accumulate_views(*v0, *params, nviews, refs, *grads, overwrite, stats, first, count, list, counts, s);
+  *pa = b3gs_prescan_args(*v0, nviews, refs, *grads, overwrite, stats, first, count, list, counts);
+  return B3GS_OK;
+}
+
+int b3gs_backward_raw_accumulate_range(int32_t nviews, const B3gsFusedView* views, const B3gsRawParams* params,
+                                       const B3gsRawGrads* grads, int32_t overwrite, const B3gsDensifyStats* stats,
+                                       int32_t first, int32_t count, b3gs_stream_t stream) {
+  PrescanArgs pa;
+  bool skip;
+  int rc = accumulate_args(nviews, views, params, grads, overwrite, stats, first, count, &pa, &skip);
+  if (rc || skip) return rc;
+  hipStream_t s = (hipStream_t)stream;
+  StageTimer tm(s);
+  tm.mark(-1);
+  b3gs_launch_prescan(pa, s);
+  b3gs_launch_chain(*views[0].view, *params, pa, s);
+  tm.mark(4);
+  HIP_TRY(hipGetLastError());
+  return B3GS_OK;
+}
+
+int b3gs_blend_backward_prescan(int32_t nviews, const B3gsBlendView* views, const B3gsFusedView* fused,
+                                const B3gsRawParams* params, const B3gsRawGrads* grads, int32_t overwrite,
+                                const B3gsDensifyStats* stats, int32_t inside, b3gs_stream_t stream) {
+  int rc = batch_views_ok(nviews, views);
+  if (rc) return rc;
+  PrescanArgs pa;
+  bool skip;
+  const int32_t P = (fused && fused[0].view) ? fused[0].view->P : 0;
+  if ((rc = accumulate_args(nviews, fused, params, grads, overwrite, stats, 0, P, &pa, &skip))) return rc;
+  for (int k = 0; k < nviews; k++)
+    if (fused[k].view->P != views[k].view->P || fused[k].geometry != views[k].geometry || fused[k].scratch != views[k].scratch)
+      return fail(B3GS_ERR_ARG, "%s", "the two view tables of b3gs_blend_backward_prescan must describe the same views");
+  hipStream_t s = (hipStream_t)stream;
+  BlendBatch batch;
+  if ((rc = blend_backward_batch(nviews, views, &batch))) return rc;
+  static const bool no_staged = getenv("B3GS_NO_STAGED") != nullptr;
+  StageTimer tm(s);
+  tm.mark(-1);
+  const bool ran = b3gs_launch_blend_backward_prescan(batch, (inside && !skip && !no_staged) ? &pa : nullptr, s);
+  if (!ran && !skip) b3gs_launch_prescan(pa, s);
+  tm.mark(3);
+  HIP_TRY(hipGetLastError());
+  return B3GS_OK;
+}
+
+int b3gs_backward_raw_accumulate_prescanned(int32_t nviews, const B3gsFusedView* views, const B3gsRawParams* params,
+                                            const B3gsRawGrads* grads, int32_t overwrite, const B3gsDensifyStats* stats,
+                                            b3gs_stream_t stream) {
+  PrescanArgs pa;
+  bool skip;
+  const int32_t P = (nviews > 0 && views && views[0].view) ? views[0].view->P : 0;
+  int rc = accumulate_args(nviews, views, params, grads, overwrite, stats, 0, P, &pa, &skip);
+  if (rc || skip) return rc;
+  hipStream_t s = (hipStream_t)stream;
+  StageTimer tm(s);
+  tm.mark(-1);
+  b3gs_launch_chain(*views[0].view, *params, pa, s);
   tm.mark(4);
   HIP_TRY(hipGetLastError());
   return B3GS_OK;
diff --git a/binocular3dgs_amd/csrc/preprocess.hip b/binocular3dgs_amd/csrc/preprocess.hip
--- a/binocular3dgs_amd/csrc/preprocess.hip
+++ b/binocular3dgs_amd/csrc/preprocess.hip
@@ -1,4 +1,7 @@
 #include "b3gs_internal.h"
+#include "prescan.h"
+#include <cstdlib>
+#include <cstring>
 
 namespace {
 
@@ -713,104 +716,61 @@
   }
 }
 
-struct MultiViews {
-  int n;
-  B3gsViewRef v[B3GS_MAX_FUSED_VIEWS];
-};
-
 #ifndef B3GS_ACC_WAVES
 #define B3GS_ACC_WAVES 3
 #endif
-template <int ACC_PER_THREAD>
-__global__ void __launch_bounds__(256, ACC_PER_THREAD >= 4 ? 4 : 8)
-    accumulate_scan_kernel(B3gsScene base, MultiViews mv, B3gsRawGrads rg, int overwrite, int first, int count,
-                           B3gsDensifyStats ds, uint32_t* __restrict__ g_list, uint32_t* __restrict__ g_count) {
-  constexpr int ACC_BLOCK = 256 * ACC_PER_THREAD;
-  __shared__ uint32_t s_list[ACC_BLOCK];
+template <int BLOCK>
+__global__ void __launch_bounds__(256) prescan_kernel(PrescanArgs pa) {
   __shared__ uint32_t s_count;
   if (threadIdx.x == 0) s_count = 0;
   __syncthreads();
-  const int blk_first = first + (int)blockIdx.x * ACC_BLOCK;
-  const int end = first + count;
+  const unsigned lane = threadIdx.x & 63u, w = threadIdx.x >> 6;
+  const int blk_first = pa.first + (int)blockIdx.x * BLOCK;
+  prescan_wave<(BLOCK >= 512 ? 2 : 1), true>(pa, blk_first, pa.list + (size_t)blockIdx.x * BLOCK, (int)w * (BLOCK / 4),
+                                             (int)(w + 1) * (BLOCK / 4), &s_count, lane);
+  __syncthreads();
+  if (threadIdx.x == 0) pa.counts[blockIdx.x] = s_count;
+}
+
+template <int ACC_PER_THREAD>
+__global__ void __launch_bounds__(256) accumulate_post_kernel(PrescanArgs pa) {
+  constexpr int ACC_BLOCK = 256 * ACC_PER_THREAD;
+  const MultiViews& mv = pa.mv;
+  const B3gsRawGrads& rg = pa.rg;
+  const B3gsDensifyStats& ds = pa.ds;
+  const int overwrite = pa.overwrite, nrest = pa.nrest;
+  const uint32_t nblk = gridDim.x / (uint32_t)ACC_PER_THREAD;
+  const uint32_t blk = blockIdx.x % nblk, part = blockIdx.x / nblk;
+  const int blk_first = pa.first + (int)blk * ACC_BLOCK;
+  uint32_t* __restrict__ s_list = pa.list + (size_t)blk * ACC_BLOCK;
+  const uint32_t e = part * 256u + threadIdx.x;
+  if (part * 256u >= pa.counts[blk]) return;
+  const uint32_t n_list = pa.counts[blk];
   const unsigned lane = threadIdx.x & 63u;
-  const unsigned long long lt = lane == 0 ? 0ull : (~0ull >> (64 - lane));
-  const int nrest = 3 * (base.M - 1);
-  const bool skip_stats = ds.skip_if_nonzero && *ds.skip_if_nonzero != 0;
-  unsigned long long epochs = 0ull;
-#pragma unroll
-  for (int v = 0; v < B3GS_MAX_FUSED_VIEWS; v++)
-    if (v < mv.n && mv.v[v].staged) epochs |= (unsigned long long)(*mv.v[v].epoch & 0xFFu) << (8 * v);
-
-  uint32_t vis_j[ACC_PER_THREAD], stg_j[ACC_PER_THREAD];
-  int rad_j[ACC_PER_THREAD];
-  float cnt_j[ACC_PER_THREAD], acc_j[ACC_PER_THREAD], den_j[ACC_PER_THREAD], mxr_j[ACC_PER_THREAD];
-  const bool do_stats = ds.denom && !skip_stats;
-#pragma unroll
-  for (int j = 0; j < ACC_PER_THREAD; j++) {
-    const int i = blk_first + j * 256 + (int)threadIdx.x;
-    const bool valid = i < end;
-    const int ic = valid ? i : end - 1;
-    uint32_t vis = 0u, stg = 0u;
-    int st_rad = 0;
-    float st_cnt = 0.f;
-#pragma unroll
-    for (int v = 0; v < B3GS_MAX_FUSED_VIEWS; v++) {
-      if (v < mv.n) {
+  const uint32_t ent = e < n_list ? s_list[e] : 0u;
+  const int i = blk_first + (int)(ent & 0xFFFFu);
+  const size_t i3 = 3 * (size_t)i;
+  uint32_t mask = 0u;
+    {
+      const uint32_t marked = ent >> 16;
+      float st_norm = 0.f;
+      bool st_any = false;
+#pragma unroll 1
+      for (int v = 0; v < mv.n; v++) {
+        if (!((marked >> v) & 1u)) continue;
         const B3gsViewRef& vr = mv.v[v];
-        const int rad = vr.radii[ic];
-        const uint8_t ep = (uint8_t)(epochs >> (8 * v));
-        const uint8_t mk = vr.staged ? vr.staged[ic] : ep;
-        if (rad > 0) {
-          vis |= 1u << v;
-          if (vr.densify_stats) {
-            st_cnt += 1.0f;
-            st_rad = max(st_rad, rad);
-          }
-        }
-        if (mk == ep) stg |= 1u << v;
-      }
-    }
-    vis_j[j] = valid ? vis : 0u, stg_j[j] = stg, rad_j[j] = st_rad, cnt_j[j] = valid ? st_cnt : 0.f;
-    acc_j[j] = do_stats ? ds.xyz_gradient_accum[ic] : 0.f;
-    den_j[j] = do_stats ? ds.denom[ic] : 0.f;
-    mxr_j[j] = do_stats ? ds.max_radii2D[ic] : 0.f;
-  }
-#pragma unroll
-  for (int j = 0; j < ACC_PER_THREAD; j++) {
-    const int li = j * 256 + (int)threadIdx.x;
-    const int i = blk_first + li;
-    uint32_t mask = 0;
-    if (i < end) {
-      const size_t i3 = 3 * (size_t)i;
-      float st_norm = 0.f;
-      const float st_cnt = cnt_j[j];
-      const int st_rad = rad_j[j];
-      const uint32_t vis = vis_j[j], stg = stg_j[j];
-      for (int v = 0; v < mv.n; v++) {
-        const B3gsViewRef& vr = mv.v[v];
-        float* m2d = vr.dL_dmeans2D;
-        if (!((vis >> v) & 1u)) {
-          if (m2d) { m2d[i3] = 0.f; m2d[i3 + 1] = 0.f; m2d[i3 + 2] = 0.f; }
-          continue;
-        }
-        float2 r0 = make_float2(0.f, 0.f), r1 = r0, r2 = r0, r3 = r0, r4 = r0;
-        if ((stg >> v) & 1u) {
-          const float2* row = reinterpret_cast<const float2*>(vr.scratch) + 5 * (size_t)i;
-          r0 = row[0], r1 = row[1], r2 = row[2], r3 = row[3], r4 = row[4];
-        }
+        const float2* row = reinterpret_cast<const float2*>(vr.scratch) + 5 * (size_t)i;
+        const float2 r0 = row[0], r1 = row[1], r2 = row[2], r3 = row[3], r4 = row[4];
         const uint32_t any = ((__float_as_uint(r0.x) | __float_as_uint(r0.y)) | (__float_as_uint(r1.x) | __float_as_uint(r1.y))) |
                              ((__float_as_uint(r2.x) | __float_as_uint(r2.y)) | (__float_as_uint(r3.x) | __float_as_uint(r3.y))) |
                              (__float_as_uint(r4.x) | __float_as_uint(r4.y));
         if (any) mask |= 1u << v;
+        float* m2d = vr.dL_dmeans2D;
         if (m2d) { m2d[i3] = r2.x; m2d[i3 + 1] = r2.y; m2d[i3 + 2] = 0.f; }
-        if (vr.densify_stats) st_norm += sqrtf(r2.x * r2.x + r2.y * r2.y);
-      }
-      if (do_stats && st_cnt > 0.f) {
-        ds.xyz_gradient_accum[i] = acc_j[j] + st_norm;
-        ds.denom[i] = den_j[j] + st_cnt;
-        ds.max_radii2D[i] = fmaxf(mxr_j[j], (float)st_rad);
-      }
-      if (mask == 0u && overwrite && !rg.touched_rows) {
+        if (vr.densify_stats) { st_norm += sqrtf(r2.x * r2.x + r2.y * r2.y); st_any = true; }
+      }
+      if (st_any && ds.denom && !(ds.skip_if_nonzero && *ds.skip_if_nonzero != 0)) ds.xyz_gradient_accum[i] += st_norm;
+      if (marked != 0u && mask == 0u && overwrite && !rg.touched_rows) {
         rg.xyz[i3] = 0.f; rg.xyz[i3 + 1] = 0.f; rg.xyz[i3 + 2] = 0.f;
         rg.scaling[i3] = 0.f; rg.scaling[i3 + 1] = 0.f; rg.scaling[i3 + 2] = 0.f;
         reinterpret_cast<float4*>(rg.rotation)[i] = make_float4(0.f, 0.f, 0.f, 0.f);
@@ -819,22 +779,20 @@
         float* rest = rg.features_rest + (size_t)nrest * i;
         for (int k = 0; k < nrest; k++) rest[k] = 0.f;
       }
-    }
-    const unsigned long long b = __ballot(mask != 0u);
-    if (overwrite && rg.touched_rows && lane == 0 && blk_first + j * 256 + (int)(threadIdx.x & ~63u) < end)
-      rg.touched_rows[(size_t)(blk_first + j * 256 + (int)(threadIdx.x & ~63u)) >> 6] = b;
-    if (b) {
-      const int leader = __builtin_ctzll(b);
-      uint32_t at = 0;
-      if ((int)lane == leader) at = atomicAdd(&s_count, (uint32_t)__builtin_popcountll(b));
-      at = (uint32_t)__shfl((int)at, leader, 64);
-      if (mask != 0u) s_list[at + (uint32_t)__builtin_popcountll(b & lt)] = (uint32_t)li | (mask << 16);
-    }
-  }
-  __syncthreads();
-  const uint32_t n_list = s_count;
-  for (uint32_t e = threadIdx.x; e < n_list; e += 256) g_list[(size_t)blockIdx.x * ACC_BLOCK + e] = s_list[e];
-  if (threadIdx.x == 0) g_count[blockIdx.x] = n_list;
+      if (overwrite && rg.touched_rows) {
+        const uint32_t wd = (uint32_t)i >> 6;
+        unsigned long long bits = mask ? 1ull << ((uint32_t)i & 63u) : 0ull;
+#pragma unroll
+        for (int d = 1; d < 64; d <<= 1) {
+          const uint32_t ow = (uint32_t)__shfl_up((int)wd, d, 64);
+          const uint32_t lo = (uint32_t)__shfl_up((int)(uint32_t)bits, d, 64), hi = (uint32_t)__shfl_up((int)(uint32_t)(bits >> 32), d, 64);
+          if (lane >= (unsigned)d && ow == wd) bits |= (unsigned long long)lo | ((unsigned long long)hi << 32);
+        }
+        const uint32_t nw = (uint32_t)__shfl_down((int)wd, 1, 64);
+        if (bits && (lane == 63u || nw != wd)) atomicOr(reinterpret_cast<unsigned long long*>(rg.touched_rows) + wd, bits);
+      }
+    }
+  if (e < n_list) s_list[e] = (ent & 0xFFFFu) | (mask << 16);
 }
 
 template <int REG>
@@ -851,9 +809,13 @@
 constexpr int CH_ROW = 25;
 template <int ACC_PER_THREAD>
 __global__ void __launch_bounds__(256, B3GS_ACC_WAVES)
-    accumulate_chain_kernel(B3gsScene base, B3gsRawParams raw, MultiViews mv, B3gsRawGrads rg, int overwrite, int first,
-                            const uint32_t* __restrict__ g_list, const uint32_t* __restrict__ g_count) {
+    accumulate_chain_kernel(B3gsScene base, B3gsRawParams raw, PrescanArgs pa) {
   constexpr int ACC_BLOCK = 256 * ACC_PER_THREAD;
+  const MultiViews& mv = pa.mv;
+  const B3gsRawGrads& rg = pa.rg;
+  const int overwrite = pa.overwrite, first = pa.first;
+  const uint32_t* __restrict__ g_list = pa.list;
+  const uint32_t* __restrict__ g_count = pa.counts;
   __shared__ float s_acc[CH_GROUP][CH_ROW];
   __shared__ uint8_t s_idx[B3GS_MAX_FUSED_VIEWS][CH_GROUP];
   __shared__ uint32_t s_wcnt[B3GS_MAX_FUSED_VIEWS][4];
@@ -876,9 +838,9 @@
   for (uint32_t e0 = part * (uint32_t)CH_GROUP; e0 < n_list; e0 += CH_GROUP) {
     const uint32_t e = e0 + threadIdx.x;
     const uint32_t ent = e < n_list ? s_list[e] : 0u;
-    const uint32_t mask = ent >> 16;
     const int i = blk_first + (int)(ent & 0xFFFFu);
     const size_t i3 = 3 * (size_t)i;
+    const uint32_t mask = ent >> 16;
 #pragma unroll
     for (int k = 0; k < 23; k++) s_acc[threadIdx.x][k] = 0.f;
     if (mask != 0u && overwrite && base.M > 4) {
@@ -1036,29 +998,56 @@
                        dL_dopacity, dL_dmeans3D, dL_dcov3D, dL_dsh, dL_dscales, dL_drotations, none, m2d_out);
 }
 
+int b3gs_acc_block(int count) {
+  static const int force = getenv("B3GS_ACC_PER_THREAD") ? atoi(getenv("B3GS_ACC_PER_THREAD")) : 0;
+  if (force == 2) return 512;
+  return (force ? force >= 4 : count >= (1 << 18) + (1 << 17)) ? 1024 : 256;
+}
+
+PrescanArgs b3gs_prescan_args(const B3gsScene& base, int nviews, const B3gsViewRef* views, const B3gsRawGrads& rg, int overwrite,
+                              const B3gsDensifyStats* stats, int first, int count, uint32_t* list, uint32_t* counts) {
+  PrescanArgs pa;
+  memset(&pa, 0, sizeof(pa));
+  pa.mv.n = nviews;
+  for (int v = 0; v < nviews; v++) pa.mv.v[v] = views[v];
+  pa.rg = rg;
+  pa.ds = stats ? *stats : B3gsDensifyStats{nullptr, nullptr, nullptr, nullptr};
+  pa.overwrite = overwrite, pa.first = first, pa.count = count, pa.nrest = 3 * (base.M - 1);
+  pa.block = b3gs_acc_block(count);
+  pa.list = list, pa.counts = counts;
+  return pa;
+}
+
+void b3gs_launch_prescan(const PrescanArgs& pa, hipStream_t s) {
+  if (pa.mv.n <= 0 || pa.count <= 0) return;
+  const dim3 grid((pa.count + pa.block - 1) / pa.block);
+  if (pa.block == 512) hipLaunchKernelGGL(prescan_kernel<512>, grid, dim3(256), 0, s, pa);
+  else if (pa.block == 1024) hipLaunchKernelGGL(prescan_kernel<1024>, grid, dim3(256), 0, s, pa);
+  else hipLaunchKernelGGL(prescan_kernel<256>, grid, dim3(256), 0, s, pa);
+}
+
+void b3gs_launch_chain(const B3gsScene& base, const B3gsRawParams& raw, const PrescanArgs& pa, hipStream_t s) {
+  if (base.P <= 0 || pa.mv.n <= 0 || pa.count <= 0) return;
+  const unsigned nblk = (unsigned)((pa.count + pa.block - 1) / pa.block);
+  if (pa.block == 512) {
+    hipLaunchKernelGGL(accumulate_post_kernel<2>, dim3(nblk * 2), dim3(256), 0, s, pa);
+    hipLaunchKernelGGL(accumulate_chain_kernel<2>, dim3(nblk * 2), dim3(256), 0, s, base, raw, pa);
+  } else if (pa.block == 1024) {
+    hipLaunchKernelGGL(accumulate_post_kernel<4>, dim3(nblk * 4), dim3(256), 0, s, pa);
+    hipLaunchKernelGGL(accumulate_chain_kernel<4>, dim3(nblk * 4), dim3(256), 0, s, base, raw, pa);
+  } else {
+    hipLaunchKernelGGL(accumulate_post_kernel<1>, dim3(nblk), dim3(256), 0, s, pa);
+    hipLaunchKernelGGL(accumulate_chain_kernel<1>, dim3(nblk), dim3(256), 0, s, base, raw, pa);
+  }
+}
+
 void b3gs_launch_accumulate_views(const B3gsScene& base, const B3gsRawParams& raw, int nviews, const B3gsViewRef* views,
                                   const B3gsRawGrads& rg, int overwrite, const B3gsDensifyStats* stats, int first, int count,
                                   uint32_t* list, uint32_t* counts, hipStream_t s) {
   if (base.P <= 0 || nviews <= 0 || count <= 0) return;
-  MultiViews mv;
-  mv.n = nviews;
-  for (int v = 0; v < nviews; v++) mv.v[v] = views[v];
-  const B3gsDensifyStats ds = stats ? *stats : B3gsDensifyStats{nullptr, nullptr, nullptr, nullptr};
-  static const int force = getenv("B3GS_ACC_PER_THREAD") ? atoi(getenv("B3GS_ACC_PER_THREAD")) : 0;
-  const bool big = force ? force >= 4 : count >= (1 << 18) + (1 << 17);
-  if (force == 2) {
-    const dim3 grid((count + 511) / 512);
-    hipLaunchKernelGGL(accumulate_scan_kernel<2>, grid, dim3(256), 0, s, base, mv, rg, overwrite, first, count, ds, list, counts);
-    hipLaunchKernelGGL(accumulate_chain_kernel<2>, dim3(grid.x * 2), dim3(256), 0, s, base, raw, mv, rg, overwrite, first, list, counts);
-  } else if (big) {
-    const dim3 grid((count + 1023) / 1024);
-    hipLaunchKernelGGL(accumulate_scan_kernel<4>, grid, dim3(256), 0, s, base, mv, rg, overwrite, first, count, ds, list, counts);
-    hipLaunchKernelGGL(accumulate_chain_kernel<4>, dim3(grid.x * 4), dim3(256), 0, s, base, raw, mv, rg, overwrite, first, list, counts);
-  } else {
-    const dim3 grid((count + 255) / 256);
-    hipLaunchKernelGGL(accumulate_scan_kernel<1>, grid, dim3(256), 0, s, base, mv, rg, overwrite, first, count, ds, list, counts);
-    hipLaunchKernelGGL(accumulate_chain_kernel<1>, grid, dim3(256), 0, s, base, raw, mv, rg, overwrite, first, list, counts);
-  }
+  const PrescanArgs pa = b3gs_prescan_args(base, nviews, views, rg, overwrite, stats, first, count, list, counts);
+  b3gs_launch_prescan(pa, s);
+  b3gs_launch_chain(base, raw, pa, s);
 }
 
 void b3gs_launch_mark_visible(int32_t P, const float* means3D, const float* viewmatrix, uint8_t* present,
diff --git a/binocular3dgs_amd/csrc/prescan.h b/binocular3dgs_amd/csrc/prescan.h
--- /dev/null
+++ b/binocular3dgs_amd/csrc/prescan.h
@@ -0,0 +1,131 @@
+#pragma once
+#include "b3gs_internal.h"
+
+struct MultiViews {
+  int n;
+  B3gsViewRef v[B3GS_MAX_FUSED_VIEWS];
+};
+
+struct PrescanArgs {
+  MultiViews mv;
+  B3gsRawGrads rg;
+  B3gsDensifyStats ds;
+  int32_t overwrite, first, count, nrest;
+  int32_t block;
+  uint32_t blend_blocks;
+  uint32_t* list;
+  uint32_t* counts;
+};
+
+#ifdef __HIPCC__
+template <int J, bool SHARED>
+__device__ __forceinline__ uint32_t prescan_wave(const PrescanArgs& pa, int blk_first, uint32_t* __restrict__ blk_list,
+                                                 int li0, int li1, uint32_t* s_count, unsigned lane) {
+  const MultiViews& mv = pa.mv;
+  const B3gsDensifyStats& ds = pa.ds;
+  const B3gsRawGrads& rg = pa.rg;
+  const int end = pa.first + pa.count;
+  const unsigned long long lt = lane == 0 ? 0ull : (~0ull >> (64 - lane));
+  const bool skip_stats = ds.skip_if_nonzero && *ds.skip_if_nonzero != 0;
+  const bool do_stats = ds.denom && !skip_stats;
+  const bool bitmap = pa.overwrite && rg.touched_rows;
+  unsigned long long epochs = 0ull;
+#pragma unroll
+  for (int v = 0; v < B3GS_MAX_FUSED_VIEWS; v++)
+    if (v < mv.n && mv.v[v].staged) epochs |= (unsigned long long)(*mv.v[v].epoch & 0xFFu) << (8 * v);
+  uint32_t run = 0;
+#pragma unroll 1
+  for (int base = li0; base < li1; base += 64 * J) {
+    uint32_t mrk_j[J];
+    int rad_j[J];
+    float cnt_j[J], den_j[J], mxr_j[J];
+    bool valid_j[J];
+#pragma unroll
+    for (int j = 0; j < J; j++) {
+      const int li = base + j * 64 + (int)lane;
+      const int i = blk_first + li;
+      const bool valid = li < li1 && i < end;
+      const int ic = valid ? i : end - 1;
+      uint32_t vis = 0u, stg = 0u;
+      int st_rad = 0;
+      float st_cnt = 0.f;
+#pragma unroll
+      for (int v = 0; v < B3GS_MAX_FUSED_VIEWS; v++) {
+        if (v < mv.n) {
+          const B3gsViewRef& vr = mv.v[v];
+          const int rad = vr.radii[ic];
+          const uint8_t ep = (uint8_t)(epochs >> (8 * v));
+          const uint8_t mk = vr.staged ? vr.staged[ic] : ep;
+          if (rad > 0) {
+            vis |= 1u << v;
+            if (vr.densify_stats) {
+              st_cnt += 1.0f;
+              st_rad = max(st_rad, rad);
+            }
+          }
+          if (mk == ep) stg |= 1u << v;
+        }
+      }
+      valid_j[j] = valid, mrk_j[j] = valid ? (vis & stg) : 0u, rad_j[j] = st_rad, cnt_j[j] = valid ? st_cnt : 0.f;
+      den_j[j] = do_stats ? ds.denom[ic] : 0.f;
+      mxr_j[j] = do_stats ? ds.max_radii2D[ic] : 0.f;
+    }
+#pragma unroll
+    for (int j = 0; j < J; j++) {
+      const int li = base + j * 64 + (int)lane;
+      const int i = blk_first + li;
+      const uint32_t marked = mrk_j[j];
+      if (valid_j[j]) {
+        const size_t i3 = 3 * (size_t)i;
+#pragma unroll
+        for (int v = 0; v < B3GS_MAX_FUSED_VIEWS; v++)
+          if (v < mv.n) {
+            float* m2d = mv.v[v].dL_dmeans2D;
+            if (m2d && !((marked >> v) & 1u)) { m2d[i3] = 0.f; m2d[i3 + 1] = 0.f; m2d[i3 + 2] = 0.f; }
+          }
+        if (do_stats && cnt_j[j] > 0.f) {
+          ds.denom[i] = den_j[j] + cnt_j[j];
+          ds.max_radii2D[i] = fmaxf(mxr_j[j], (float)rad_j[j]);
+        }
+        if (marked == 0u && pa.overwrite && !rg.touched_rows) {
+          rg.xyz[i3] = 0.f; rg.xyz[i3 + 1] = 0.f; rg.xyz[i3 + 2] = 0.f;
+          rg.scaling[i3] = 0.f; rg.scaling[i3 + 1] = 0.f; rg.scaling[i3 + 2] = 0.f;
+          reinterpret_cast<float4*>(rg.rotation)[i] = make_float4(0.f, 0.f, 0.f, 0.f);
+          rg.opacity[i] = 0.f;
+          rg.features_dc[i3] = 0.f; rg.features_dc[i3 + 1] = 0.f; rg.features_dc[i3 + 2] = 0.f;
+          float* rest = rg.features_rest + (size_t)pa.nrest * i;
+          for (int k = 0; k < pa.nrest; k++) rest[k] = 0.f;
+        }
+      }
+      const unsigned long long b = __ballot(marked != 0u);
+      const int i_word = blk_first + base + j * 64;
+      if (bitmap && lane == 0 && base + j * 64 < li1 && i_word < end) rg.touched_rows[(size_t)i_word >> 6] = 0ull;
+      if (b) {
+        uint32_t at = run;
+        if (SHARED) {
+          const int leader = __builtin_ctzll(b);
+          if ((int)lane == leader) at = atomicAdd(s_count, (uint32_t)__builtin_popcountll(b));
+          at = (uint32_t)__shfl((int)at, leader, 64);
+        } else {
+          run += (uint32_t)__builtin_popcountll(b);
+        }
+        if (marked != 0u) blk_list[at + (uint32_t)__builtin_popcountll(b & lt)] = (uint32_t)li | (marked << 16);
+      }
+    }
+  }
+  return run;
+}
+
+__device__ __forceinline__ void prescan_block_wave(const PrescanArgs& pa, uint32_t blk, unsigned lane) {
+  const int blk_first = pa.first + (int)blk * pa.block;
+  const uint32_t n = prescan_wave<2, false>(pa, blk_first, pa.list + (size_t)blk * (size_t)pa.block, 0, pa.block, nullptr, lane);
+  if (lane == 0) pa.counts[blk] = n;
+}
+#endif
+
+int b3gs_acc_block(int count);
+PrescanArgs b3gs_prescan_args(const B3gsScene& base, int nviews, const B3gsViewRef* views, const B3gsRawGrads& rg, int overwrite,
+                              const B3gsDensifyStats* stats, int first, int count, uint32_t* list, uint32_t* counts);
+void b3gs_launch_prescan(const PrescanArgs& pa, hipStream_t s);
+void b3gs_launch_chain(const B3gsScene& base, const B3gsRawParams& raw, const PrescanArgs& pa, hipStream_t s);
+bool b3gs_launch_blend_backward_prescan(BlendBatch batch, const PrescanArgs* pre, hipStream_t s);
diff --git a/binocular3dgs_amd/csrc/render.hip b/binocular3dgs_amd/csrc/render.hip
--- a/binocular3dgs_amd/csrc/render.hip
+++ b/binocular3dgs_amd/csrc/render.hip
@@ -1,4 +1,5 @@
 #include "b3gs_internal.h"
+#include "prescan.h"
 #include <cstdlib>
 #include <cstring>
 
@@ -612,9 +613,15 @@
   float4 A[SC], B[SC], C[SC];
   float red[10 * RED_STRIDE];
 };
-template <bool TRACE, int SC, bool REGS, bool ROWS>
+template <bool TRACE, int SC, bool REGS, bool ROWS, bool PRE = false>
 __global__ void __launch_bounds__(64, REGS ? B3GS_BWD_QWAVES : B3GS_BWD_WAVES)
-    render_bwd_kernel(BlendBatch batch, unsigned long long* __restrict__ trace) {
+    render_bwd_kernel(BlendBatch batch, unsigned long long* __restrict__ trace, PrescanArgs pre) {
+  if (PRE) {
+    if (blockIdx.x >= pre.blend_blocks) {
+      prescan_block_wave(pre, blockIdx.x - pre.blend_blocks, threadIdx.x);
+      return;
+    }
+  }
   __shared__ WaveSharedBwd<REGS ? 1 : SC> sh;
   const unsigned long long t_start = TRACE ? __builtin_readcyclecounter() : 0ull;
   const unsigned long long r_start = TRACE ? __builtin_amdgcn_s_memrealtime() : 0ull;
@@ -917,13 +924,15 @@
 }
 }
 
-void b3gs_launch_blend_backward(BlendBatch batch, hipStream_t s) {
+void b3gs_launch_blend_backward(BlendBatch batch, hipStream_t s) { (void)b3gs_launch_blend_backward_prescan(batch, nullptr, s); }
+
+bool b3gs_launch_blend_backward_prescan(BlendBatch batch, const PrescanArgs* pre, hipStream_t s) {
   int total = 0;
   for (int k = 0; k < batch.n; k++) {
     batch.v[k].block_base = total;
     total += blocks_of(batch.v[k]);
   }
-  if (total <= 0) return;
+  if (total <= 0) return false;
   static const bool lpt = getenv("B3GS_NO_LPT") == nullptr;
   uint32_t* order = batch.order_buf;
   batch.order = nullptr;
@@ -948,16 +957,25 @@
              v.dL_dmeans2D == v.dL_dcov3D + 4 && v.dL_dcolors == v.dL_dcov3D + 6 && v.dL_dopacity == v.dL_dcov3D + 9 &&
              (uint64_t)v.cov_stride * 4u * (uint64_t)(v.idx_mask == 0xFFFFFFFFu ? 0x7FFFFFFFu : v.idx_mask) < 0xFFFFFFFFull;
     }
-    if (trace) hipLaunchKernelGGL((render_bwd_kernel<true, 64, true, false>), dim3(total * 4), dim3(64), 0, s, batch, trace);
-    else if (wave_lds) hipLaunchKernelGGL((render_bwd_kernel<false, 64, false, false>), dim3(total * 4), dim3(64), 0, s, batch, trace);
-    else if (rows) hipLaunchKernelGGL((render_bwd_kernel<false, 64, true, true>), dim3(total * 4), dim3(64), 0, s, batch, trace);
-    else hipLaunchKernelGGL((render_bwd_kernel<false, 64, true, false>), dim3(total * 4), dim3(64), 0, s, batch, trace);
-    return;
+    PrescanArgs pa;
+    if (pre) pa = *pre;
+    else memset(&pa, 0, sizeof(pa));
+    if (trace) hipLaunchKernelGGL((render_bwd_kernel<true, 64, true, false>), dim3(total * 4), dim3(64), 0, s, batch, trace, pa);
+    else if (wave_lds) hipLaunchKernelGGL((render_bwd_kernel<false, 64, false, false>), dim3(total * 4), dim3(64), 0, s, batch, trace, pa);
+    else if (rows && pre && pre->mv.n > 0 && pre->count > 0) {
+      pa.blend_blocks = (uint32_t)total * 4u;
+      const uint32_t nblk = (uint32_t)((pa.count + pa.block - 1) / pa.block);
+      hipLaunchKernelGGL((render_bwd_kernel<false, 64, true, true, true>), dim3(pa.blend_blocks + nblk), dim3(64), 0, s, batch, trace, pa);
+      return true;
+    } else if (rows) hipLaunchKernelGGL((render_bwd_kernel<false, 64, true, true>), dim3(total * 4), dim3(64), 0, s, batch, trace, pa);
+    else hipLaunchKernelGGL((render_bwd_kernel<false, 64, true, false>), dim3(total * 4), dim3(64), 0, s, batch, trace, pa);
+    return false;
   }
   if (trace) hipLaunchKernelGGL((render_bwd_tile_kernel<64, true>), dim3(total), dim3(256), 0, s, batch, trace);
   else if (bwd_chunk == 256) hipLaunchKernelGGL((render_bwd_tile_kernel<256, false>), dim3(total), dim3(256), 0, s, batch, trace);
   else if (bwd_chunk == 128) hipLaunchKernelGGL((render_bwd_tile_kernel<128, false>), dim3(total), dim3(256), 0, s, batch, trace);
   else hipLaunchKernelGGL((render_bwd_tile_kernel<64, false>), dim3(total), dim3(256), 0, s, batch, trace);
+  return false;
 }
 
 BlendView b3gs_blend_view(const B3gsScene& sc, const GeomView& g, const BinView& b, const ImgView& im) {
diff --git a/binocular3dgs_amd/fused.py b/binocular3dgs_amd/fused.py
--- a/binocular3dgs_amd/fused.py
+++ b/binocular3dgs_amd/fused.py
@@ -89,6 +89,9 @@
         self.depth_key_bits = 27
         self.slots: List[_Slot] = [self._new_slot(torch.cuda.Stream(self.dev), k) for k in range(num_slots)]
         self._deferred = None
+        self.prescan_inside = True
+        self._prescan_plan = None
+        self._prescanned = None
         self._params = _lib.B3gsRawParams()
         self._grads = _lib.B3gsRawGrads()
 
@@ -220,43 +223,70 @@
         L = _lib.lib()
         stream = torch.cuda.current_stream(self.dev)
         scenes = [self._scene(sp) for sp in specs]
+        pend = list(zip(specs, scenes))
+        plan = self._prescan_plan
+        if plan is not None and self._deferred == [] and self._prescanned is None and len(specs) <= MAX_BATCH:
+            arr, keep = self._blend_table(specs, scenes, grads)
+            favr, gr, stats = self._accumulate_args(pend, None, plan["touched_rows"], None)
+            rc = L.b3gs_blend_backward_prescan(len(arr), arr, favr, C.byref(self._bind_params()), C.byref(gr),
+                                               int(bool(plan["overwrite"])), None if stats is None else C.byref(stats),
+                                               int(bool(self.prescan_inside)), stream.cuda_stream)
+            _lib.check(rc, "b3gs_blend_backward_prescan")
+            del keep
+            self._prescanned = plan
+            self._deferred += pend
+            return
+        if self._prescanned is not None:
+            raise _lib.B3gsError("plan_prescan(): the section's first backward ran the pre-scan of ALL its views; render "
+                                 "every view of such a section in one render_batch() call")
         for c0 in range(0, len(specs), MAX_BATCH):
             arr, keep = self._blend_table(specs[c0:c0 + MAX_BATCH], scenes[c0:c0 + MAX_BATCH], grads[c0:c0 + MAX_BATCH])
             _lib.check(L.b3gs_blend_backward_batch(len(arr), arr, stream.cuda_stream), "b3gs_blend_backward_batch")
             del keep
-        pend = list(zip(specs, scenes))
         if self._deferred is not None:
             self._deferred += pend
         else:
             self._accumulate(pend, overwrite=False)
 
+    def _accumulate_args(self, chunk, grads, touched_rows, stats_target):
+        m = self.model
+        gr = grads if grads is not None else self._bind_grads()
+        if grads is None or touched_rows is not None:
+            gr.touched_rows = None if touched_rows is None else touched_rows.data_ptr()
+        stats = None
+        if getattr(m, "denom", None) is not None and m.denom.numel() == self.P:
+            ta, td, tr = stats_target if stats_target is not None else (m.xyz_gradient_accum, m.denom, m.max_radii2D)
+            stats = _lib.B3gsDensifyStats(ta.data_ptr(), td.data_ptr(), tr.data_ptr(), self.overflow_flag.data_ptr())
+        arr = (_lib.B3gsFusedView * len(chunk))()
+        for k, (sp, sc) in enumerate(chunk):
+            sl = self.slots[sp["slot"]]
+            arr[k].view = C.pointer(sc)
+            arr[k].radii, arr[k].geometry = sl.radii.data_ptr(), sl.geom.data_ptr()
+            arr[k].scratch = sl.scratch.data_ptr()
+            arr[k].dL_dmeans2D = None if sl.means2D_grad is None else sl.means2D_grad.data_ptr()
+            arr[k].densify_stats = int(bool(sp["densify_stats"]) and stats is not None)
+        return arr, gr, stats
+
     def _accumulate(self, pend, overwrite: bool, grads=None, first: int = 0, count: Optional[int] = None,
-                    touched_rows: Optional[torch.Tensor] = None, stats_target=None):
-        L, m = _lib.lib(), self.model
-        gr = grads if grads is not None else self._bind_grads()
+                    touched_rows: Optional[torch.Tensor] = None, stats_target=None, prescanned: bool = False):
+        L = _lib.lib()
         if touched_rows is not None:
             if not overwrite or len(pend) > MAX_BATCH:
                 raise _lib.B3gsError("sparse gradient rows need overwrite mode and at most 8 views (one accumulate call)")
             assert touched_rows.dtype == torch.int64 and touched_rows.numel() >= (self.P + 63) // 64
-        if grads is None or touched_rows is not None:
-            gr.touched_rows = None if touched_rows is None else touched_rows.data_ptr()
         count = self.P - first if count is None else count
-        stats = None
-        if getattr(m, "denom", None) is not None and m.denom.numel() == self.P:
-            ta, td, tr = stats_target if stats_target is not None else (m.xyz_gradient_accum, m.denom, m.max_radii2D)
-            stats = _lib.B3gsDensifyStats(ta.data_ptr(), td.data_ptr(), tr.data_ptr(), self.overflow_flag.data_ptr())
         stream = torch.cuda.current_stream(self.dev).cuda_stream
+        if prescanned:
+            assert len(pend) <= MAX_BATCH and first == 0 and count == self.P and grads is None and stats_target is None
+            arr, gr, stats = self._accumulate_args(pend, None, touched_rows, None)
+            rc = L.b3gs_backward_raw_accumulate_prescanned(len(arr), arr, C.byref(self._bind_params()), C.byref(gr),
+                                                           int(bool(overwrite)), None if stats is None else C.byref(stats),
+                                                           stream)
+            _lib.check(rc, "b3gs_backward_raw_accumulate_prescanned")
+            return
         for c0 in range(0, len(pend), MAX_BATCH):
-            chunk = pend[c0:c0 + MAX_BATCH]
-            arr = (_lib.B3gsFusedView * len(chunk))()
-            for k, (sp, sc) in enumerate(chunk):
-                sl = self.slots[sp["slot"]]
-                arr[k].view = C.pointer(sc)
-                arr[k].radii, arr[k].geometry = sl.radii.data_ptr(), sl.geom.data_ptr()
-                arr[k].scratch = sl.scratch.data_ptr()
-                arr[k].dL_dmeans2D = None if sl.means2D_grad is None else sl.means2D_grad.data_ptr()
-                arr[k].densify_stats = int(bool(sp["densify_stats"]) and stats is not None)
-            rc = L.b3gs_backward_raw_accumulate_range(len(chunk), arr, C.byref(self._bind_params()), C.byref(gr),
+            arr, gr, stats = self._accumulate_args(pend[c0:c0 + MAX_BATCH], grads, touched_rows, stats_target)
+            rc = L.b3gs_backward_raw_accumulate_range(len(arr), arr, C.byref(self._bind_params()), C.byref(gr),
                                                       int(bool(overwrite) and c0 == 0),
                                                       None if stats is None else C.byref(stats), first, count, stream)
             _lib.check(rc, "b3gs_backward_raw_accumulate_range")
@@ -284,9 +314,17 @@
 
     def begin_deferred(self):
         self._deferred = []
+        self._prescan_plan = self._prescanned = None
+
+    def plan_prescan(self, overwrite: bool = True, touched_rows: Optional[torch.Tensor] = None):
+        assert self._deferred is not None, "plan_prescan() belongs inside begin_deferred() ... finish_deferred()"
+        self._prescan_plan = {"overwrite": bool(overwrite), "touched_rows": touched_rows}
 
     def take_deferred(self):
+        if self._prescanned is not None:
+            raise _lib.B3gsError("take_deferred(): this section's backward already ran the pre-scan (plan_prescan)")
         pend, self._deferred = self._deferred, None
+        self._prescan_plan = None
         return pend
 
     def accumulate_range(self, pend, grads, first: int, count: int, overwrite: bool = True, stats_target=None):
@@ -303,6 +341,7 @@
 
     def finish_deferred(self, overwrite: bool = True, touched_rows: Optional[torch.Tensor] = None):
         pend, self._deferred = self._deferred, None
+        pre, self._prescanned, self._prescan_plan = self._prescanned, None, None
         if not pend:
             if overwrite:
                 for p in self.model.parameters():
@@ -311,7 +350,9 @@
                 if touched_rows is not None:
                     touched_rows.fill_(-1)
             return
-        self._accumulate(pend, overwrite, touched_rows=touched_rows)
+        if pre is not None and (pre["overwrite"] != bool(overwrite) or pre["touched_rows"] is not touched_rows):
+            raise _lib.B3gsError("finish_deferred(): arguments differ from the ones announced with plan_prescan()")
+        self._accumulate(pend, overwrite, touched_rows=touched_rows, prescanned=pre is not None)
 
     def resize(self):
         self.P = self.model.get_xyz.shape[0]
diff --git a/binocular3dgs_amd/step.py b/binocular3dgs_amd/step.py
--- a/binocular3dgs_amd/step.py
+++ b/binocular3dgs_amd/step.py
@@ -597,14 +597,18 @@
                     grads.append(g)
         else:
             outs, grads = self._loss_pixel_grads(pkgs, loss_fn, batch_loss_fn)
+        finish_here = self.fused is not None and not self._chain_rule_after_agreement()
+        if finish_here:
+            self._row_mask = self._sparse_rows()
+            if len(self.views) <= 8:
+                self.fused.plan_prescan(overwrite=True, touched_rows=self._row_mask)
         if outs:
             torch.autograd.backward(outs, grads)
         if self.fused is None:
             self._update_densify_stats(pkgs)
         if self.fused is not None:
-            if not self._chain_rule_after_agreement():
+            if finish_here:
                 self._pending_views = None
-                self._row_mask = self._sparse_rows()
                 self.fused.finish_deferred(overwrite=True, touched_rows=self._row_mask)
             else:
                 self._pending_views = self.fused.take_deferred()
diff --git a/include/b3gs_raster.h b/include/b3gs_raster.h
--- a/include/b3gs_raster.h
+++ b/include/b3gs_raster.h
@@ -154,6 +154,13 @@
 int b3gs_backward_raw_accumulate_range(int32_t nviews, const B3gsFusedView* views, const B3gsRawParams* params,
                                        const B3gsRawGrads* grads, int32_t overwrite, const B3gsDensifyStats* stats,
                                        int32_t first, int32_t count, b3gs_stream_t stream);
+
+int b3gs_blend_backward_prescan(int32_t nviews, const B3gsBlendView* views, const B3gsFusedView* fused,
+                                const B3gsRawParams* params, const B3gsRawGrads* grads, int32_t overwrite,
+                                const B3gsDensifyStats* stats, int32_t inside, b3gs_stream_t stream);
+int b3gs_backward_raw_accumulate_prescanned(int32_t nviews, const B3gsFusedView* views, const B3gsRawParams* params,
+                                            const B3gsRawGrads* grads, int32_t overwrite, const B3gsDensifyStats* stats,
+                                            b3gs_stream_t stream);
 
 typedef struct B3gsAdamSegment {
   float* param;
```

Result: slower. 429.7 iters/s (-10.8%).
